# amcpherson/defuse

Hardware: AMD Instinct MI355X
Metric: split-read DP aligns/sec (higher is better)
Workload: dtype int16

## Files before the change

### defuse_amd/csrc/dsa_api.hip

```cpp
#include <hip/hip_runtime.h>
#include <fcntl.h>
#include <sys/file.h>
#include <unistd.h>
#include <hipcub/hipcub.hpp>

#include <algorithm>
#include <atomic>
#include <condition_variable>
#include <memory>
#include <mutex>
#include <thread>
#include <cstdio>
#include <cstdlib>
#include <cstring>
#include <string>
#include <chrono>
#include <vector>

#include "dsa_kernels.hpp"
#include "dsa_long.hpp"
#include "dsa_diag_host.hpp"
#include "hip_host.hpp"

using namespace dsa;

namespace {

template <typename T>
using DevBuf = hiphost::DeviceBuffer<T, hiphost::GrowSize>;
using hiphost::elapsed;
using hiphost::grid_of;

struct HostResult {
    Counters ctr;
    int64_t n_rec;
    PlanGlobals plan;
};

struct PipeLane {
    hipStream_t stream = nullptr;
    hipEvent_t ev[7] = {};
    hipStream_t aux = nullptr;
    hipEvent_t ev_fork = nullptr, ev_join = nullptr;
    HostResult* host = nullptr;
    int slice = -1;
    int64_t resident_upload = -1;
    int resident_slice = -1;
    bool emit_pending = false;
    bool emit_early = false;
    uint64_t emit_cap = 0;
    int emit_from = 5;
    uint64_t last_gtasks = 0;
    bool phase1_end_recorded = false;
    unsigned tier_hint = 0xFu;
    unsigned tiers_launched = 0;
    DevBuf<uint8_t> d_wg_tier;
    DevBuf<uint32_t> d_rowcodes, d_rowbytes, d_bnd, d_cmax, d_rmax, d_tmask;
    DevBuf<PairState> d_state;
    DevBuf<KeptRow> d_kept;
    DevBuf<int64_t> d_rec_count, d_rec_offset;
    DevBuf<ReplayTask> d_tasks;
    DevBuf<uint64_t> d_masks;
    DevBuf<uint2> d_gtasks;
    DevBuf<Counters> d_ctr;
    DevBuf<uint8_t> d_scan_tmp;
    DevBuf<int32_t> d_tstop;
#ifdef DSA_PRUNE_STATS
    DevBuf<unsigned long long> d_stats;
#endif
    void release()
    {
        d_wg_tier.release(); d_rowcodes.release(); d_rowbytes.release();
        d_bnd.release(); d_cmax.release(); d_rmax.release(); d_tmask.release(); d_state.release(); d_kept.release();
        d_rec_count.release(); d_rec_offset.release(); d_tasks.release(); d_masks.release(); d_gtasks.release();
        d_ctr.release(); d_scan_tmp.release(); d_tstop.release();
    }
};

struct LaneSet {
    int device = -1;
    hipStream_t own[2] = {};
    PipeLane lane[2];
    ~LaneSet()
    {
        if (device >= 0) (void)hipSetDevice(device);
        (void)hipDeviceSynchronize();
        for (PipeLane& L : lane) {
            L.release();
            for (auto& e : L.ev)
                if (e) (void)hipEventDestroy(e);
            if (L.ev_fork) (void)hipEventDestroy(L.ev_fork);
            if (L.ev_join) (void)hipEventDestroy(L.ev_join);
            if (L.aux) (void)hipStreamDestroy(L.aux);
            if (L.host) (void)hipHostFree(L.host);
        }
        for (hipStream_t st : own)
            if (st) (void)hipStreamDestroy(st);
    }
};

std::atomic<int64_t> g_upload_serial{0};

struct Slice {
    int64_t pair_begin = 0, pair_end = 0;
    Geom g{};
};

}

struct dsa_ctx {
    int device = -1;
    hipStream_t main_stream() const;
    hipStream_t user_stream = nullptr;
    std::string err;
    size_t scratch_budget = (size_t)16 << 30;
    unsigned plan_flags = 0;

    int64_t n_pairs = 0, ref_bytes_len = 0, read_bytes_len = 0;
    int32_t n_fusions = 0;
    DevBuf<uint8_t> d_ref, d_reads;
    DevBuf<dsa_fusion> d_fusions;
    int64_t upload_serial = 0;
    int nch_all = 1;
    DevBuf<uint32_t> d_refcodes;
    hipEvent_t ev_pack[2] = {};
    DevBuf<int32_t> d_orig;
    DevBuf<dsa_pair> d_pairs_in;
    DevBuf<dsa_pair> d_pairs;
    DevBuf<int32_t> d_min_score;
    DevBuf<PlanRun> plan_runs;
    DevBuf<uint32_t> plan_key, plan_key_sorted;
    DevBuf<int32_t> plan_fidx, plan_order, plan_bsum, plan_start, plan_rank;
    DevBuf<uint16_t> plan_bound;
    DevBuf<uint8_t> plan_flip, plan_sort_tmp;
    DevBuf<PlanGlobals> plan_glob;
    PlanParams plan_prm{};
    hipEvent_t ev_plan[2] = {};
    bool plan_timed = false;
    std::vector<Slice> slices;
    float last_plan_ms = 0.f;
    std::vector<int32_t> h_min_score;
    std::vector<LongDesc> h_long;
    std::vector<int32_t> h_long_fusions;
    std::vector<LongState> h_long_state;
    DevBuf<LongDesc> d_long;
    DevBuf<int32_t> d_long_fusions, d_long_work, d_long_rows;
    DevBuf<LongState> d_long_state;
    DevBuf<uint32_t> d_long_bits;
    int64_t long_cells = 0;
    int64_t long_blank_cells = 0;

    std::shared_ptr<LaneSet> lanes;
    DevBuf<dsa_record> d_records;
    int64_t n_records = 0;
    bool have_results = false;

    dsa_timing timing{};
    dsa_kernel_counts kcounts{};
};

hipStream_t dsa_ctx::main_stream() const { return lanes->lane[0].stream; }

namespace {

template <class... Args>
int fail(dsa_ctx* c, int code, const char* fmt, Args... args)
{
    std::string nowhere;
    return hiphost::fail(c ? c->err : nowhere, code, fmt, args...);
}

#define HIPC(call) HIPHOST_TRY(ctx->err, call)

int min_score_for(int lq)
{
    float f = (float)lq * (float)DSA_MATCH;
    return (int)((double)f * 0.90);
}

size_t slice_scratch_bytes(int64_t n_waves, int lq1, int nch)
{
    size_t rows = (size_t)n_waves * lq1 * WAVE * 4;
    return 3 * rows + rows / 4 + 2 * rows * (size_t)nch;
}

void make_slices(dsa_ctx* ctx, int64_t n_pairs, int lqmax)
{
    ctx->slices.clear();
    const int lq1 = (lqmax + 1 + 3) & ~3;
    const size_t per_wg = slice_scratch_bytes(WG_WAVES, lq1, ctx->nch_all);
    int64_t chunk = (int64_t)std::min<size_t>((size_t)1 << 40, ctx->scratch_budget / std::max<size_t>(per_wg, 1)) * WG_LANES;
    if (const char* e = getenv("DEFUSE_DSA_SPLIT_LARGE"))
        if (atoi(e) != 0 && chunk >= n_pairs && n_pairs >= ((int64_t)1 << 19)) chunk = ((n_pairs + 1) / 2 + WG_LANES - 1) / WG_LANES * WG_LANES;
    if (const char* e = getenv("DEFUSE_DSA_SLICE_PAIRS")) chunk = std::min<int64_t>(chunk, std::max<int64_t>(WG_LANES, atoll(e) / WG_LANES * WG_LANES));
    chunk = std::max<int64_t>(chunk, WG_LANES);
    for (int64_t b = 0; b < n_pairs; b += chunk) {
        Slice cur;
        cur.pair_begin = b;
        cur.pair_end = std::min(n_pairs, b + chunk);
        const int64_t n = cur.pair_end - cur.pair_begin;
        cur.g.n_waves = (int32_t)((n + WAVE - 1) / WAVE);
        cur.g.n_wgs = (int32_t)((n + WG_LANES - 1) / WG_LANES);
        cur.g.lq1 = lq1;
        cur.g.nch = ctx->nch_all;
        cur.g.lrp = ctx->nch_all * W;
        cur.g.n_fusions = ctx->n_fusions;
        cur.g.n_pairs = n;
        cur.g.orig = nullptr;
        ctx->slices.push_back(cur);
    }
}

int enqueue_plan(dsa_ctx* ctx)
{
    const int nf = ctx->n_fusions;
    const int64_t n_pairs = ctx->n_pairs;
    if (n_pairs == 0 || nf == 0 || ctx->slices.empty()) return DSA_OK;
    hipStream_t st = ctx->main_stream();
    const bool no_reorder = ctx->plan_flags & DSA_PLAN_NO_REORDER, no_rank = ctx->plan_flags & DSA_PLAN_NO_RANK,
               no_tighten = ctx->plan_flags & DSA_PLAN_NO_TIGHTEN, no_lpt = ctx->plan_flags & DSA_PLAN_NO_LPT;
    int64_t max_chunk = 0;
    for (const Slice& sl : ctx->slices) max_chunk = std::max(max_chunk, sl.pair_end - sl.pair_begin);
    const int nb = (nf + PLACE_BLOCK - 1) / PLACE_BLOCK;
    HIPC(ctx->plan_runs.reserve((size_t)nf));
    HIPC(ctx->plan_key.reserve((size_t)nf));
    HIPC(ctx->plan_key_sorted.reserve((size_t)nf));
    HIPC(ctx->plan_fidx.reserve((size_t)nf));
    HIPC(ctx->plan_order.reserve((size_t)nf));
    HIPC(ctx->plan_bsum.reserve((size_t)nb));
    HIPC(ctx->plan_start.reserve((size_t)nf));
    HIPC(ctx->plan_flip.reserve((size_t)nf));
    HIPC(ctx->plan_rank.reserve((size_t)max_chunk));
    HIPC(ctx->plan_bound.reserve((size_t)max_chunk));
    HIPC(ctx->plan_glob.reserve(ctx->slices.size()));
    HIPC(ctx->d_orig.reserve((size_t)n_pairs));
    HIPC(ctx->d_pairs.reserve((size_t)n_pairs + 1));
    size_t sort_tmp = 0;
    HIPC(hipcub::DeviceRadixSort::SortPairs(nullptr, sort_tmp, ctx->plan_key.p, ctx->plan_key_sorted.p, ctx->plan_fidx.p, ctx->plan_order.p, nf, 0, PLAN_KEY_BITS, st));
    HIPC(ctx->plan_sort_tmp.reserve(sort_tmp));
    const PlanParams prm = ctx->plan_prm;
    const size_t lds = plan_lds_bytes(prm.wc, prm.slots);
    HIPC(hipEventRecord(ctx->ev_plan[0], st));
    HIPC(hipMemsetAsync(ctx->plan_glob.p, 0, ctx->slices.size() * sizeof(PlanGlobals), st));
    for (size_t k = 0; k < ctx->slices.size(); ++k) {
        Slice& sl = ctx->slices[k];
        const int64_t n = sl.pair_end - sl.pair_begin;
        const dsa_pair* in = ctx->d_pairs_in.p + sl.pair_begin;
        sl.g.orig = ctx->d_orig.p + sl.pair_begin;
        PlanGlobals* glob = ctx->plan_glob.p + k;
        if (!no_reorder) {
            HIPC(hipMemsetAsync(ctx->plan_runs.p, 0, (size_t)nf * sizeof(PlanRun), st));
            hipLaunchKernelGGL(k_plan_runs, dim3(grid_of(n)), dim3(256), 0, st, in, n, ctx->plan_runs.p);
            PlanParams pp = prm;
            pp.use_rank = no_rank ? 0 : 1;
            pp.use_bound = no_tighten ? 0 : 1;
            pp.use_lpt = no_lpt ? 0 : 1;
            hipLaunchKernelGGL(k_plan_fusion, dim3((unsigned)nf), dim3(PLAN_THREADS), lds, st, ctx->d_ref.p, ctx->d_fusions.p, ctx->d_reads.p, in,
                               ctx->plan_runs.p, ctx->plan_key.p, ctx->plan_fidx.p, ctx->plan_rank.p, ctx->plan_bound.p, glob, pp);
            size_t tmp = ctx->plan_sort_tmp.cap;
            HIPC(hipcub::DeviceRadixSort::SortPairs(ctx->plan_sort_tmp.p, tmp, ctx->plan_key.p, ctx->plan_key_sorted.p, ctx->plan_fidx.p,
                                                    ctx->plan_order.p, nf, 0, PLAN_KEY_BITS, st));
            hipLaunchKernelGGL(k_plan_place_a, dim3((unsigned)nb), dim3(PLACE_BLOCK), 0, st, ctx->plan_order.p, ctx->plan_runs.p, nf, ctx->plan_bsum.p);
            hipLaunchKernelGGL(k_plan_place_b, dim3((unsigned)nb), dim3(PLACE_BLOCK), 0, st, ctx->plan_order.p, ctx->plan_runs.p, nf, ctx->plan_bsum.p,
                               ctx->plan_start.p, ctx->plan_flip.p);
        }
        hipLaunchKernelGGL(k_plan_permute, dim3(grid_of(n)), dim3(256), 0, st, in, n, ctx->d_fusions.p, ctx->plan_runs.p, ctx->plan_start.p,
                           ctx->plan_flip.p, ctx->plan_rank.p, ctx->plan_bound.p, glob, no_reorder ? 1 : 0, ctx->d_pairs.p + sl.pair_begin,
                           ctx->d_orig.p + sl.pair_begin);
    }
    HIPC(hipEventRecord(ctx->ev_plan[1], st));
    HIPC(hipGetLastError());
    ctx->plan_timed = true;
    for (PipeLane& L : ctx->lanes->lane) L.resident_upload = -1;
    return DSA_OK;
}

int exclusive_scan(dsa_ctx* ctx, PipeLane& L, const int64_t* in, int64_t* out, int64_t n)
{
    HIPC(hiphost::cub_run(L.d_scan_tmp, [&](void* t, size_t& tmp) {
        return hipcub::DeviceScan::ExclusiveSum(t, tmp, in, out, (int)n, L.stream);
    }));
    return DSA_OK;
}

int grow_records(dsa_ctx* ctx, size_t need)
{
    if (need <= ctx->d_records.cap) return DSA_OK;
    DevBuf<dsa_record> bigger;
    HIPC(bigger.reserve(need + need / 2 + 1024));
    HIPC(hipDeviceSynchronize());
    if (ctx->n_records)
        HIPC(hipMemcpy(bigger.p, ctx->d_records.p, ctx->n_records * sizeof(dsa_record), hipMemcpyDeviceToDevice));
    ctx->d_records.release();
    ctx->d_records.swap(bigger);
    return DSA_OK;
}

FinishBufs finish_bufs(PipeLane& L)
{
    FinishBufs fb;
    fb.state = L.d_state.p;
    fb.kept = L.d_kept.p;
    fb.tasks = L.d_tasks.p;
    fb.masks = L.d_masks.p;
    fb.gtasks = L.d_gtasks.p;
    fb.ctr = L.d_ctr.p;
    fb.kept_cap = L.d_kept.cap;
    fb.task_cap = L.d_tasks.cap;
    fb.mask_cap = L.d_masks.cap / 2;
    fb.gtask_cap = L.d_gtasks.cap;
    fb.tstop = L.d_tstop.p;
    fb.rec_count = L.d_rec_count.p;
    return fb;
}

unsigned listed_grid(const PipeLane& L, int64_t n_pairs)
{
    const uint64_t expect = L.last_gtasks ? L.last_gtasks : (uint64_t)n_pairs / 10 + 1;
    const uint64_t blocks = (expect + expect / 64 + EMIT_BLOCK - 1) / EMIT_BLOCK + 1;
    return (unsigned)std::min<uint64_t>(std::max<uint64_t>(blocks, 16), 16384);
}
void launch_emit(dsa_ctx* ctx, PipeLane& L, const Slice& s, size_t cap_left, bool record_start = true)
{
    const int64_t np = s.g.n_pairs;
    Geom g = s.g;
    g.tiers_launched = L.tiers_launched;
    const dsa_pair* pairs = ctx->d_pairs.p + s.pair_begin;
    dsa_record* out = ctx->d_records.p + ctx->n_records;
    L.emit_from = record_start ? 5 : 2;
    if (record_start) (void)hipEventRecord(L.ev[5], L.stream);
    (void)hipEventRecord(L.ev_fork, L.stream);
    (void)hipStreamWaitEvent(L.aux, L.ev_fork, 0);
    hipLaunchKernelGGL(k_emit_listed<true>, dim3(listed_grid(L, np)), dim3(EMIT_BLOCK), 0, L.aux, L.d_gtasks.p, (uint64_t)L.d_gtasks.cap, L.d_ctr.p,
                       pairs, ctx->d_fusions.p, L.d_state.p, L.d_kept.p, L.d_tasks.p, (uint64_t)L.d_tasks.cap, L.d_masks.p,
                       (uint64_t)(L.d_masks.cap / 2), (uint64_t)L.d_kept.cap, L.d_rec_count.p, (const int64_t*)L.d_rec_offset.p, out,
                       (uint64_t)cap_left, (int64_t)s.pair_begin, g);
    (void)hipEventRecord(L.ev_join, L.aux);
    hipLaunchKernelGGL(k_emit_counted, dim3((unsigned)((np + EMIT_BLOCK - 1) / EMIT_BLOCK)), dim3(EMIT_BLOCK), 0, L.stream, pairs, ctx->d_fusions.p,
                       L.d_state.p, L.d_kept.p, L.d_tasks.p, L.d_masks.p, (const int64_t*)L.d_rec_offset.p, out, (uint64_t)cap_left,
                       (int64_t)s.pair_begin, L.d_ctr.p, (uint64_t)L.d_kept.cap, (uint64_t)L.d_tasks.cap, (uint64_t)(L.d_masks.cap / 2),
                       (uint64_t)L.d_gtasks.cap, g);
    if (!ctx->h_long.empty())
        hipLaunchKernelGGL(k_long_emit<true>, dim3((unsigned)((ctx->h_long.size() + 63) / 64)), dim3(64), 0, L.stream, ctx->d_long.p, ctx->d_long_state.p,
                           (int)ctx->h_long.size(), ctx->d_long_work.p, ctx->d_long_bits.p, (int64_t)s.pair_begin, (int64_t)s.pair_end, L.d_rec_count.p,
                           (const int64_t*)L.d_rec_offset.p, out, (uint64_t)cap_left);
    (void)hipStreamWaitEvent(L.stream, L.ev_join, 0);
    (void)hipEventRecord(L.ev[6], L.stream);
}

int launch_compute(dsa_ctx* ctx, PipeLane& L, const Slice& s)
{
    Geom g = s.g;
#ifdef DSA_PRUNE_STATS
    HIPC(L.d_stats.reserve(16));
    HIPC(hipMemsetAsync(L.d_stats.p, 0, 16 * sizeof(unsigned long long), L.stream));
    g.stats = L.d_stats.p;
#endif
    hipStream_t st = L.stream;
    const int64_t np = g.n_pairs;
    const dsa_pair* pairs = ctx->d_pairs.p + s.pair_begin;
    const FinishBufs fb = finish_bufs(L);
    hipLaunchKernelGGL(k_reset_finish, dim3(1), dim3(64), 0, st, L.d_ctr.p, L.d_rec_count.p + np);
    HIPC(hipEventRecord(L.ev[1], st));
    const unsigned mask = L.tier_hint | 1u;
    L.tiers_launched = mask;
    g.tiers_launched = mask;
#define DSA_LAUNCH_FILL(TIER, WIDE)                                                                                                              \
    hipLaunchKernelGGL((k_fill_fast<TIER, WIDE>), dim3((unsigned)g.n_wgs), dim3(WG_LANES), 0, st, pairs, L.d_wg_tier.p, ctx->d_refcodes.p, \
                       ctx->d_reads.p, L.d_rowcodes.p, L.d_rowbytes.p, ctx->d_min_score.p, ctx->d_fusions.p, L.d_bnd.p, L.d_cmax.p, L.d_rmax.p, L.d_tmask.p, fb, g)
    const bool wide = g.nch > 8 && g.nch <= 16;
    if (wide) DSA_LAUNCH_FILL(0, true); else DSA_LAUNCH_FILL(0, false);
    if (mask & 2u) { if (wide) DSA_LAUNCH_FILL(1, true); else DSA_LAUNCH_FILL(1, false); }
    if (mask & 4u) { if (wide) DSA_LAUNCH_FILL(2, true); else DSA_LAUNCH_FILL(2, false); }
#undef DSA_LAUNCH_FILL
    if (mask & 8u)
        hipLaunchKernelGGL(k_fill_generic, dim3((unsigned)g.n_wgs), dim3(WG_LANES), 0, st, pairs, ctx->d_fusions.p, L.d_wg_tier.p, ctx->d_refcodes.p,
                           ctx->d_reads.p, L.d_rowcodes.p, ctx->d_min_score.p, L.d_bnd.p, L.d_cmax.p, L.d_rmax.p, L.d_tmask.p, fb, g);
    HIPC(hipEventRecord(L.ev[2], st));
    hipLaunchKernelGGL(k_replay, dim3(2048), dim3(REPLAY_BLOCK), 0, st, L.d_tasks.p, (uint64_t)L.d_tasks.cap, L.d_gtasks.p,
                       (uint64_t)L.d_gtasks.cap, L.d_ctr.p, L.d_state.p, L.d_kept.p, (uint64_t)L.d_kept.cap, pairs, ctx->d_fusions.p,
                       ctx->d_refcodes.p, L.d_rowcodes.p, L.d_bnd.p, L.d_tstop.p, L.d_masks.p, (uint64_t)(L.d_masks.cap / 2), g);
    hipLaunchKernelGGL(k_emit_listed<false>, dim3(listed_grid(L, np)), dim3(EMIT_BLOCK), 0, st, L.d_gtasks.p, (uint64_t)L.d_gtasks.cap, L.d_ctr.p,
                       pairs, ctx->d_fusions.p, L.d_state.p, L.d_kept.p, L.d_tasks.p, (uint64_t)L.d_tasks.cap, L.d_masks.p,
                       (uint64_t)(L.d_masks.cap / 2), (uint64_t)L.d_kept.cap, L.d_rec_count.p, (const int64_t*)nullptr, (dsa_record*)nullptr,
                       (uint64_t)0, (int64_t)s.pair_begin, g);
    if (!ctx->h_long.empty())
        hipLaunchKernelGGL(k_long_emit<false>, dim3((unsigned)((ctx->h_long.size() + 63) / 64)), dim3(64), 0, st, ctx->d_long.p, ctx->d_long_state.p,
                           (int)ctx->h_long.size(), ctx->d_long_work.p, ctx->d_long_bits.p, (int64_t)s.pair_begin, (int64_t)s.pair_end, L.d_rec_count.p,
                           (const int64_t*)nullptr, (dsa_record*)nullptr, (uint64_t)0);
    if (int rc = exclusive_scan(ctx, L, L.d_rec_count.p, L.d_rec_offset.p, np + 1)) return rc;
    hipLaunchKernelGGL(k_publish, dim3(1), dim3(64), 0, st, L.d_ctr.p, L.d_rec_offset.p + np, reinterpret_cast<const unsigned long long*>(ctx->plan_glob.p + (&s - ctx->slices.data())),
                       &L.host->ctr, &L.host->n_rec, reinterpret_cast<unsigned long long*>(&L.host->plan));
    L.emit_cap = 0;
    L.emit_early = false;
    L.phase1_end_recorded = false;
    if (ctx->n_records == 0 && &s == &ctx->slices.front() && ctx->d_records.cap > 0) {
        L.emit_cap = ctx->d_records.cap;
        L.emit_early = true;
        launch_emit(ctx, L, s, L.emit_cap, false);
    } else {
        HIPC(hipEventRecord(L.ev[3], st));
        L.phase1_end_recorded = true;
    }
    HIPC(hipGetLastError());
    return DSA_OK;
}

int phase1(dsa_ctx* ctx, PipeLane& L, int slice_idx)
{
    const Slice& s = ctx->slices[slice_idx];
    Geom g = s.g;
    hipStream_t st = L.stream;
    const int64_t np = g.n_pairs;
    if (g.lq1 > ((FAST_MAX_READ + 1 + 3) & ~3)) return fail(ctx, DSA_E_LIMIT, "internal: a long read reached the 16-bit kernels");
    const size_t n_rows = (size_t)g.n_waves * g.lq1 * WAVE;
    HIPC(L.d_wg_tier.reserve((size_t)g.n_wgs));
    HIPC(L.d_rowcodes.reserve(n_rows));
    HIPC(L.d_rowbytes.reserve(n_rows / 4));
    HIPC(L.d_bnd.reserve(n_rows * g.nch));
    HIPC(L.d_cmax.reserve(n_rows * g.nch));
    HIPC(L.d_rmax.reserve(n_rows));
    HIPC(L.d_tmask.reserve(n_rows));
    HIPC(L.d_tstop.reserve((size_t)g.n_waves * g.nch));
    HIPC(L.d_state.reserve(np));
    HIPC(L.d_rec_count.reserve(np + 1));
    HIPC(L.d_rec_offset.reserve(np + 1));
    HIPC(L.d_ctr.reserve(1));
    HIPC(L.d_kept.reserve((size_t)np * 2 + 1024));
    HIPC(L.d_tasks.reserve((size_t)np * 4 + 1024));
    HIPC(L.d_masks.reserve((size_t)np * 8 + 1024));
    HIPC(L.d_gtasks.reserve((size_t)np * 2 + 1024));
    if (int rc = launch_compute(ctx, L, s)) return rc;
    L.slice = slice_idx;
    return DSA_OK;
}

void account_emit(dsa_ctx* ctx, PipeLane& L)
{
    if (!L.emit_pending) return;
    (void)hipEventSynchronize(L.ev[6]);
    ctx->timing.finish_ms += elapsed(L.ev[L.emit_from], L.ev[6]);
    L.emit_pending = false;
}

int phase2(dsa_ctx* ctx, PipeLane& L)
{
    const Slice& s = ctx->slices[L.slice];
    account_emit(ctx, L);
    for (int attempt = 0;; ++attempt) {
        HIPC(hipStreamSynchronize(L.stream));
        HIPC(hipGetLastError());
        const Counters c = L.host->ctr;
        const bool tiers_ok = (c.need_tiers & ~L.tiers_launched) == 0;
        L.tier_hint = tiers_ok ? c.need_tiers : 0xFu;
        if (!tiers_ok) ctx->kcounts.slices_rerun += 1;
        if (tiers_ok && c.n_kept <= L.d_kept.cap && c.n_tasks <= L.d_tasks.cap && c.n_masks <= L.d_masks.cap / 2 && c.n_gtasks <= L.d_gtasks.cap) break;
        if (attempt >= 3) return fail(ctx, DSA_E_DEVICE, "finish stage did not converge");
        HIPC(L.d_kept.reserve(c.n_kept + 1024));
        HIPC(L.d_tasks.reserve(c.n_tasks + 1024));
        HIPC(L.d_masks.reserve(2 * c.n_masks + 1024));
// ... 113 lines not shown
    if (hiphost::check_device(device) || hipSetDevice(device) != hipSuccess) return DSA_E_DEVICE;
    dsa_ctx* ctx = new dsa_ctx();
    ctx->device = device;
    bool ok = true;
    for (const auto& sw : {std::pair<const char*, unsigned>{"DEFUSE_DSA_NO_REORDER", DSA_PLAN_NO_REORDER}, {"DEFUSE_DSA_NO_RANK", DSA_PLAN_NO_RANK},
                           {"DEFUSE_DSA_NO_TIGHTEN", DSA_PLAN_NO_TIGHTEN}, {"DEFUSE_DSA_NO_LPT", DSA_PLAN_NO_LPT}}) {
        const char* e = getenv(sw.first);
        if (e && atoi(e) != 0) ctx->plan_flags |= sw.second;
    }
    if (share) {
        ctx->lanes = share->lanes;
        ctx->scratch_budget = share->scratch_budget;
    } else {
        ctx->lanes = std::make_shared<LaneSet>();
        ctx->lanes->device = device;
        for (int l = 0; l < 2; ++l) {
            PipeLane& L = ctx->lanes->lane[l];
            ok = ok && hipStreamCreate(&ctx->lanes->own[l]) == hipSuccess;
            L.stream = ctx->lanes->own[l];
            for (auto& e : L.ev) ok = ok && hipEventCreate(&e) == hipSuccess;
            ok = ok && hipStreamCreateWithFlags(&L.aux, hipStreamNonBlocking) == hipSuccess;
            ok = ok && hipEventCreateWithFlags(&L.ev_fork, hipEventDisableTiming) == hipSuccess;
            ok = ok && hipEventCreateWithFlags(&L.ev_join, hipEventDisableTiming) == hipSuccess;
            ok = ok && hipHostMalloc((void**)&L.host, sizeof(HostResult)) == hipSuccess;
        }
    }
    for (auto& e : ctx->ev_pack) ok = ok && hipEventCreate(&e) == hipSuccess;
    for (auto& e : ctx->ev_plan) ok = ok && hipEventCreate(&e) == hipSuccess;
    if (!ok) {
        dsa_destroy(ctx);
        return DSA_E_DEVICE;
    }
    if (!share)
        if (const char* mb = getenv("DEFUSE_DSA_SCRATCH_MB")) {
            long v = atol(mb);
            if (v > 0) ctx->scratch_budget = (size_t)v << 20;
        }
    *out = ctx;
    return DSA_OK;
}

int dsa_create(dsa_ctx** out, int device) { return create_ctx(out, device, nullptr); }

void dsa_destroy(dsa_ctx* ctx)
{
    if (!ctx) return;
    (void)hipSetDevice(ctx->device);
    (void)hipDeviceSynchronize();
    ctx->d_ref.release(); ctx->d_reads.release(); ctx->d_fusions.release(); ctx->d_pairs.release(); ctx->d_orig.release(); ctx->d_pairs_in.release();
    ctx->d_min_score.release(); ctx->d_records.release(); ctx->d_refcodes.release();
    ctx->plan_runs.release(); ctx->plan_key.release(); ctx->plan_key_sorted.release(); ctx->plan_fidx.release(); ctx->plan_order.release();
    ctx->plan_bsum.release(); ctx->plan_start.release(); ctx->plan_rank.release(); ctx->plan_bound.release(); ctx->plan_flip.release();
    ctx->plan_sort_tmp.release(); ctx->plan_glob.release();
    ctx->d_long.release(); ctx->d_long_fusions.release(); ctx->d_long_work.release(); ctx->d_long_rows.release(); ctx->d_long_state.release();
    ctx->d_long_bits.release();
    for (auto& e : ctx->ev_pack)
        if (e) (void)hipEventDestroy(e);
    for (auto& e : ctx->ev_plan)
        if (e) (void)hipEventDestroy(e);
    ctx->lanes.reset();
    delete ctx;
}

int dsa_share_scratch(dsa_ctx* ctx, dsa_ctx* donor)
{
    if (!ctx || !donor || ctx == donor) return DSA_E_ARG;
    if (ctx->device != donor->device) return fail(ctx, DSA_E_ARG, "dsa_share_scratch: contexts on different devices");
    HIPC(hipSetDevice(ctx->device));
    HIPC(hipDeviceSynchronize());
    ctx->lanes = donor->lanes;
    ctx->scratch_budget = donor->scratch_budget;
    return DSA_OK;
}

int dsa_get_limits(const dsa_ctx*, dsa_limits* out)
{
    if (!out) return DSA_E_ARG;
    out->max_read_len = LONG_MAX_READ;
    out->max_ref_len = LONG_MAX_REF;
    out->tile_cols = W;
    return DSA_OK;
}

const char* dsa_last_error(const dsa_ctx* ctx) { return ctx ? ctx->err.c_str() : "no context"; }

int dsa_set_stream(dsa_ctx* ctx, void* hip_stream)
{
    if (!ctx) return DSA_E_ARG;
    ctx->user_stream = (hipStream_t)hip_stream;
    ctx->lanes->lane[0].stream = hip_stream ? (hipStream_t)hip_stream : ctx->lanes->own[0];
    return DSA_OK;
}

int dsa_synchronize(dsa_ctx* ctx)
{
    if (!ctx) return DSA_E_ARG;
    HIPC(hipStreamSynchronize(ctx->main_stream()));
    return DSA_OK;
}

}

namespace {

int upload_enqueue(dsa_ctx* ctx, hipStream_t st, const uint8_t* ref_bytes, int64_t ref_bytes_len, const dsa_fusion* fusions,
               int32_t n_fusions, const uint8_t* read_bytes, int64_t read_bytes_len, const dsa_pair* pairs,
               int64_t n_pairs)
{
    if (!ctx) return DSA_E_ARG;
    if (n_fusions < 0 || n_pairs < 0 || ref_bytes_len < 0 || read_bytes_len < 0)
        return fail(ctx, DSA_E_ARG, "negative size");
    if (n_pairs >= ((int64_t)1 << 31)) return fail(ctx, DSA_E_LIMIT, "more than 2^31-1 pairs in one batch");
    if ((n_fusions && !fusions) || (n_pairs && !pairs) || (ref_bytes_len && !ref_bytes) || (read_bytes_len && !read_bytes))
        return fail(ctx, DSA_E_ARG, "null pointer with non-zero size");
    ctx->h_long.clear();
    ctx->h_long_fusions.clear();
    ctx->long_cells = 0;
    ctx->long_blank_cells = 0;
    int nch_all = 1, maxwin = 0;
    for (int32_t f = 0; f < n_fusions; ++f) {
        const dsa_fusion& fu = fusions[f];
        if (fu.ref0_len < 0 || fu.ref1_len < 0 || fu.ref0_off < 0 || fu.ref1_off < 0 ||
            (int64_t)fu.ref0_off + fu.ref0_len > ref_bytes_len || (int64_t)fu.ref1_off + fu.ref1_len > ref_bytes_len)
            return fail(ctx, DSA_E_ARG, "fusion %d: reference window outside ref_bytes", f);
        if (fu.ref0_len > LONG_MAX_REF || fu.ref1_len > LONG_MAX_REF)
            return fail(ctx, DSA_E_LIMIT, "fusion %d: reference window longer than %d", f, LONG_MAX_REF);
        if (fu.ref0_len > FAST_MAX_REF || fu.ref1_len > FAST_MAX_REF) {
            ctx->h_long_fusions.push_back(f);
            continue;
        }
        nch_all = std::max<int>(nch_all, std::max(grid_of(fu.ref0_len, W), grid_of(fu.ref1_len, W)));
        maxwin = std::max(maxwin, std::max(fu.ref0_len, fu.ref1_len));
    }
    const bool any_long_fusion = !ctx->h_long_fusions.empty();
    int lqmax = 0;
    for (int64_t p = 0; p < n_pairs; ++p) {
        const dsa_pair& pr = pairs[p];
        if (pr.fusion_idx < 0 || pr.fusion_idx >= n_fusions) return fail(ctx, DSA_E_ARG, "pair %lld: bad fusion_idx", (long long)p);
        if (pr.read_len < 0 || pr.read_off < 0 || (int64_t)pr.read_off + pr.read_len > read_bytes_len)
            return fail(ctx, DSA_E_ARG, "pair %lld: read outside read_bytes", (long long)p);
        if (pr.read_len > LONG_MAX_READ) return fail(ctx, DSA_E_LIMIT, "pair %lld: read longer than %d", (long long)p, LONG_MAX_READ);
        if (pr.read_len > FAST_MAX_READ ||
            (any_long_fusion && (fusions[pr.fusion_idx].ref0_len > FAST_MAX_REF || fusions[pr.fusion_idx].ref1_len > FAST_MAX_REF))) {
            const dsa_fusion& fu = fusions[pr.fusion_idx];
            LongDesc d;
            d.pair_idx = (int32_t)p;
            d.read_off = pr.read_off;
            d.read_len = pr.read_len;
            d.ref0_off = fu.ref0_off;
            d.ref0_len = fu.ref0_len;
            d.ref1_off = fu.ref1_off;
            d.ref1_len = fu.ref1_len;
            d.fusion_id = fu.fusion_id;
            d.frag = pr.frag;
            d.read_end = pr.read_end;
            d.revcomp = pr.revcomp;
            d.min_score = min_score_for(pr.read_len);
            ctx->h_long.push_back(d);
            ctx->long_cells += (int64_t)(fu.ref0_len + 1 + fu.ref1_len + 1) * (pr.read_len + 1);
            ctx->long_blank_cells += (fu.ref0_len > FAST_MAX_REF || fu.ref1_len > FAST_MAX_REF) ? 2 : fu.ref0_len + 1 + fu.ref1_len + 1;
            continue;
        }
        lqmax = std::max(lqmax, (int)pr.read_len);
    }
    HIPC(hipSetDevice(ctx->device));
    ctx->have_results = false;
    ctx->n_records = 0;
    ctx->upload_serial = ++g_upload_serial;
    ctx->n_pairs = n_pairs;
    ctx->n_fusions = n_fusions;
    ctx->ref_bytes_len = ref_bytes_len;
    ctx->read_bytes_len = read_bytes_len;
    HIPC(ctx->d_ref.reserve((size_t)ref_bytes_len + 64));
    HIPC(ctx->d_reads.reserve((size_t)read_bytes_len + 64));
    HIPC(ctx->d_fusions.reserve((size_t)n_fusions + 1));
    HIPC(ctx->d_pairs_in.reserve((size_t)n_pairs + 1));
    ctx->nch_all = nch_all;
    HIPC(ctx->d_refcodes.reserve((size_t)n_fusions * nch_all * W + 1));
    if (ref_bytes_len) HIPC(hipMemcpyAsync(ctx->d_ref.p, ref_bytes, ref_bytes_len, hipMemcpyHostToDevice, st));
    if (read_bytes_len) HIPC(hipMemcpyAsync(ctx->d_reads.p, read_bytes, read_bytes_len, hipMemcpyHostToDevice, st));
    if (n_fusions) HIPC(hipMemcpyAsync(ctx->d_fusions.p, fusions, n_fusions * sizeof(dsa_fusion), hipMemcpyHostToDevice, st));
    if (n_pairs) HIPC(hipMemcpyAsync(ctx->d_pairs_in.p, pairs, n_pairs * sizeof(dsa_pair), hipMemcpyHostToDevice, st));
    if (!ctx->h_long.empty() || !ctx->h_long_fusions.empty()) {
        const int nl = (int)ctx->h_long.size(), nlf = (int)ctx->h_long_fusions.size();
        HIPC(ctx->d_long.reserve((size_t)nl + 1));
        HIPC(ctx->d_long_fusions.reserve((size_t)nlf + 1));
        if (nl) HIPC(hipMemcpyAsync(ctx->d_long.p, ctx->h_long.data(), (size_t)nl * sizeof(LongDesc), hipMemcpyHostToDevice, st));
        if (nlf) HIPC(hipMemcpyAsync(ctx->d_long_fusions.p, ctx->h_long_fusions.data(), (size_t)nlf * sizeof(int32_t), hipMemcpyHostToDevice, st));
        const int n = std::max(nl, nlf);
        hipLaunchKernelGGL(k_long_blank, dim3(grid_of(n)), dim3(256), 0, st, ctx->d_pairs_in.p, ctx->d_long.p, nl, ctx->d_fusions.p,
                           ctx->d_long_fusions.p, nlf);
    }
    std::vector<int32_t>& tab = ctx->h_min_score;
    tab.resize(lqmax + 1);
    for (int l = 0; l <= lqmax; ++l) tab[l] = min_score_for(l);
    HIPC(ctx->d_min_score.reserve(tab.size()));
    HIPC(hipMemcpyAsync(ctx->d_min_score.p, tab.data(), tab.size() * sizeof(int32_t), hipMemcpyHostToDevice, st));
    {
        const int mw = std::min(maxwin, PLAN_MAXWIN - 1);
        int slots = 256;
        while (slots < 2 * mw) slots <<= 1;
        ctx->plan_prm = PlanParams{};
        ctx->plan_prm.n_fusions = n_fusions;
        ctx->plan_prm.slots = slots;
        ctx->plan_prm.wc = (mw + 2 * PLAN_PAD + 47) / 16 + 1;
        ctx->plan_prm.tile_cols = W;
    }
    make_slices(ctx, n_pairs, lqmax);
    HIPC(hipGetLastError());
    return DSA_OK;
}


}

extern "C" {

int dsa_upload(dsa_ctx* ctx, const uint8_t* ref_bytes, int64_t ref_bytes_len, const dsa_fusion* fusions,
               int32_t n_fusions, const uint8_t* read_bytes, int64_t read_bytes_len, const dsa_pair* pairs,
               int64_t n_pairs)
{
    if (!ctx) return DSA_E_ARG;
    if (int rc = upload_enqueue(ctx, ctx->main_stream(), ref_bytes, ref_bytes_len, fusions, n_fusions, read_bytes, read_bytes_len, pairs, n_pairs)) return rc;
    if (int rc = enqueue_plan(ctx)) return rc;
    HIPC(hipStreamSynchronize(ctx->main_stream()));
    HIPC(hipGetLastError());
    return DSA_OK;
}

int dsa_plan(dsa_ctx* ctx)
{
    if (!ctx) return DSA_E_ARG;
    HIPC(hipSetDevice(ctx->device));
    ctx->have_results = false;
    return enqueue_plan(ctx);
}

}

namespace {

void reset_lanes(dsa_ctx* ctx)
{
    for (PipeLane& L : ctx->lanes->lane) {
        (void)hipStreamSynchronize(L.stream);
        (void)hipStreamSynchronize(L.aux);
        L.slice = -1;
        L.emit_pending = false;
        L.emit_early = false;
    }
    (void)hipGetLastError();
}

int run_long(dsa_ctx* ctx)
{
    const int nl = (int)ctx->h_long.size();
    if (nl == 0) return DSA_OK;
    hipStream_t st = ctx->lanes->lane[0].stream;
    std::vector<LongState>& hs = ctx->h_long_state;
    hs.assign((size_t)nl, LongState{});
    for (LongState& x : hs) x.max_score = -1;
    int64_t work = 0, rows_max = 0;
    for (int k = 0; k < nl; ++k) {
        const LongDesc& d = ctx->h_long[(size_t)k];
        hs[(size_t)k].work_off = work;
        work += long_work_words(d.read_len);
        rows_max = std::max(rows_max, long_rows_words(d.ref0_len, d.ref1_len));
    }
    const int grid = (int)std::max<int64_t>(1, std::min<int64_t>(std::min(nl, 512), ((int64_t)1 << 28) / std::max<int64_t>(rows_max, 1)));
    HIPC(ctx->d_long_work.reserve((size_t)work + 1));
    HIPC(ctx->d_long_rows.reserve((size_t)(rows_max * grid) + 1));
    HIPC(ctx->d_long_state.reserve((size_t)nl));
    HIPC(hipMemcpyAsync(ctx->d_long_state.p, hs.data(), (size_t)nl * sizeof(LongState), hipMemcpyHostToDevice, st));
    hipLaunchKernelGGL(k_long_rows, dim3((unsigned)grid), dim3(LONG_THREADS), 0, st, ctx->d_long.p, ctx->d_long_state.p, nl, ctx->d_ref.p, ctx->d_reads.p,
                       ctx->d_long_work.p, ctx->d_long_rows.p, rows_max);
    HIPC(hipMemcpyAsync(hs.data(), ctx->d_long_state.p, (size_t)nl * sizeof(LongState), hipMemcpyDeviceToHost, st));
    HIPC(hipStreamSynchronize(st));
    HIPC(hipGetLastError());
    int64_t bits = 0;
    for (int k = 0; k < nl; ++k) {
        const LongDesc& d = ctx->h_long[(size_t)k];
        ctx->kcounts.long_pairs += hs[(size_t)k].max_score >= 0 ? 1 : 0;
        hs[(size_t)k].bits_off = bits;
        bits += (int64_t)hs[(size_t)k].n_kept * (long_bitmap_words(d.ref0_len) + long_bitmap_words(d.ref1_len));
    }
    HIPC(ctx->d_long_bits.reserve((size_t)bits + 1));
    HIPC(hipMemcpyAsync(ctx->d_long_state.p, hs.data(), (size_t)nl * sizeof(LongState), hipMemcpyHostToDevice, st));
    hipLaunchKernelGGL(k_long_cols, dim3((unsigned)grid), dim3(LONG_THREADS), 0, st, ctx->d_long.p, ctx->d_long_state.p, nl, ctx->d_ref.p, ctx->d_reads.p,
                       ctx->d_long_work.p, ctx->d_long_rows.p, rows_max, ctx->d_long_bits.p);
// ... 368 lines not shown
```

### defuse_amd/csrc/dsa_diag.hpp

```cpp
#pragma once
#include <hip/hip_runtime.h>

namespace dsa {

#ifdef DSA_NO_PRUNE
constexpr bool DIAG_PRUNE = false;
#else
constexpr bool DIAG_PRUNE = true;
#endif
#ifdef DSA_NO_GAP_SKIP
constexpr bool DIAG_GAP_SKIP = false;
#else
constexpr bool DIAG_GAP_SKIP = true;
#endif
#ifdef DSA_NARROW
constexpr bool DIAG_NARROW = true;
#else
constexpr bool DIAG_NARROW = false;
#endif
#ifdef DSA_ABLATE_TAIL
constexpr bool DIAG_TAIL = false;
#else
constexpr bool DIAG_TAIL = true;
#endif
#ifdef DSA_ABLATE_REPLAY
constexpr bool DIAG_REPLAY = false;
#else
constexpr bool DIAG_REPLAY = true;
#endif

enum DiagSlot {
    DS_GROUPS_SKIPPED = 0, DS_GROUPS = 1, DS_UNUSED2 = 2, DS_WAVE_CYCLES = 3, DS_BARRIER = 4, DS_TABLES = 5, DS_TAIL = 6, DS_ROWMAX = 7,
    DS_COMBINE = 8, DS_REPLAY = 9, DS_GREPLAY_SETUP = 10, DS_GREPLAY_SWEEP = 11, DS_GREPLAY_WAVES = 12, DS_GREPLAY_STEPS = 13,
    DS_GAP_GROUPS = 14, DS_SLOWEST_LISTED = 15
};

#ifdef DSA_PRUNE_STATS
struct DiagClock {
    unsigned long long t;
    __device__ DiagClock() : t(__builtin_readcyclecounter()) {}
    __device__ unsigned long long lap()
    {
        const unsigned long long n = __builtin_readcyclecounter(), d = n - t;
        t = n;
        return d;
    }
};
#define DSA_STAT_ADD(g, slot, v) atomicAdd(&(g).stats[slot], (unsigned long long)(v))
#define DSA_STAT_MAX(g, slot, v) atomicMax(&(g).stats[slot], (unsigned long long)(v))
#else
struct DiagClock {
    __device__ unsigned long long lap() { return 0; }
};
#define DSA_STAT_ADD(g, slot, v) ((void)0)
#define DSA_STAT_MAX(g, slot, v) ((void)0)
#endif

}
```

### defuse_amd/csrc/dsa_diag_host.hpp

```cpp
#pragma once
#ifdef DSA_PRUNE_STATS
#include <cstdio>
#include <vector>

#include "dsa_kernels.hpp"

namespace dsa {

inline void diag_dump_slice(const unsigned long long* d_stats, const uint2* d_gtasks, size_t ng, const ReplayTask* d_tasks, size_t nt)
{
    std::vector<uint2> gt(ng);
    std::vector<ReplayTask> tk(nt);
    if (ng) (void)hipMemcpy(gt.data(), d_gtasks, ng * sizeof(uint2), hipMemcpyDeviceToHost);
    if (nt) (void)hipMemcpy(tk.data(), d_tasks, nt * sizeof(ReplayTask), hipMemcpyDeviceToHost);
    long hist[3][10] = {};
    for (size_t i = 0; i < ng; ++i) {
        const ReplayTask& t = tk[gt[i].x & ~GTASK_OWNER];
        const int kind = t.chunk0 != NO_CHUNK && t.chunk1 != NO_CHUNK ? 2 : t.chunk0 != NO_CHUNK ? 0 : 1;
        hist[kind][std::min(9, (t.last_row & TASK_ROW) / 8)]++;
    }
    for (int k = 0; k < 3; ++k) {
        fprintf(stderr, "[stats] left-over replay tasks, %s, by last row / 8:", k == 0 ? "M1 side only" : k == 1 ? "M2 side only" : "both sides");
        for (int b = 0; b < 10; ++b) fprintf(stderr, " %ld", hist[k][b]);
        fprintf(stderr, "\n");
    }
    unsigned long long h[16];
    (void)hipMemcpy(h, d_stats, sizeof h, hipMemcpyDeviceToHost);
    const double wc = h[DS_WAVE_CYCLES] ? (double)h[DS_WAVE_CYCLES] : 1.0;
    fprintf(stderr,
            "[stats] fill: row groups not swept %llu of %llu (of which skipped between live parts %llu); wave cycles %.4g: tile barriers %.1f %%, "
            "table builds %.1f %%, tail %.1f %% (row maxima %.1f, combine %.1f, replay %.1f), sweeps %.1f %%\n",
            h[DS_GROUPS_SKIPPED], h[DS_GROUPS], h[DS_GAP_GROUPS], wc, 100.0 * h[DS_BARRIER] / wc, 100.0 * h[DS_TABLES] / wc, 100.0 * h[DS_TAIL] / wc,
            100.0 * h[DS_ROWMAX] / wc, 100.0 * h[DS_COMBINE] / wc, 100.0 * h[DS_REPLAY] / wc,
            100.0 * (wc - h[DS_BARRIER] - h[DS_TABLES] - h[DS_TAIL]) / wc);
    fprintf(stderr, "[stats] left-over replay: %llu waves, set-up %llu, sweep %llu cycles, %llu steps (lane 0); slowest lane of the listed count: %llu cycles, "
            "%llu kept rows, %llu tasks\n", h[DS_GREPLAY_WAVES], h[DS_GREPLAY_SETUP], h[DS_GREPLAY_SWEEP], h[DS_GREPLAY_STEPS], h[DS_SLOWEST_LISTED] >> 24,
            (h[DS_SLOWEST_LISTED] >> 8) & 0xFFFF, h[DS_SLOWEST_LISTED] & 0xFF);
}

inline void diag_dump_plan()
{
    unsigned long long h[8] = {}, zero[8] = {};
    (void)hipMemcpyFromSymbol(h, HIP_SYMBOL(g_plan_phase), sizeof h);
    (void)hipMemcpyToSymbol(HIP_SYMBOL(g_plan_phase), zero, sizeof zero);
    double tot = 0;
    for (int k = 0; k < 6; ++k) tot += (double)h[k];
    if (tot == 0) return;
    const char* names[6] = {"prologue + first read", "windows packed", "11-mers hashed", "diagonals + vote", "bounds + keys", "ranks"};
    fprintf(stderr, "[stats] k_plan_fusion wave cycles %.4g:", tot);
    for (int k = 0; k < 6; ++k) fprintf(stderr, " %s %.1f %%", names[k], 100.0 * h[k] / tot);
    fprintf(stderr, "\n");
}

}
#endif
```

### defuse_amd/csrc/dsa_kernels.hpp

```cpp
#pragma once
#include <hip/hip_runtime.h>
#include <stdint.h>

#include "../../include/defuse_dsa.h"
#include "dsa_diag.hpp"

namespace dsa {

constexpr int W = 64;
constexpr int WAVE = 64;
constexpr int WG_WAVES = 4;
constexpr int WG_LANES = WG_WAVES * WAVE;
constexpr uint32_t REF_PAD16 = 0x00AAu;
constexpr uint32_t ROW_PAD16 = 0x0055u;

constexpr int NCLS = 5;
constexpr int NCOMBO = NCLS * NCLS;
constexpr int TROW = W + 4;
#ifndef FILL_PF
#define FILL_PF 2
#endif
constexpr int GMAX = 4;
constexpr int TGROUP = NCOMBO * TROW;
constexpr int GSPLIT = 20;
constexpr int GSPLIT2 = 40;
constexpr int TROW_S = TROW / 2;
constexpr int TGROUP_SPLIT = 2 * NCLS * TROW_S;
static_assert(GSPLIT * TGROUP_SPLIT <= GMAX * TGROUP, "split tables must fit the LDS of the combined ones");
static_assert((TROW_S % 2) == 0, "split table rows are read with ds_read_b64");

__device__ __forceinline__ uint4 split_terms(const uint32_t* tb, uint32_t k1, uint32_t k2, int q)
{
    const uint2 L = reinterpret_cast<const uint2*>(tb + k1 * TROW_S)[q];
    const uint2 H = reinterpret_cast<const uint2*>(tb + (NCLS + k2) * TROW_S)[q];
    return make_uint4(__builtin_amdgcn_perm(H.x, L.x, 0x05040100u), __builtin_amdgcn_perm(H.x, L.x, 0x07060302u),
                      __builtin_amdgcn_perm(H.y, L.y, 0x05040100u), __builtin_amdgcn_perm(H.y, L.y, 0x07060302u));
}
constexpr uint32_t BIAS16 = 0x0400u;
constexpr uint32_t BIAS2 = 0x04000400u;
constexpr uint32_t TWO2 = 0x00020002u;
constexpr uint32_t FOUR2 = 0x00040004u;
constexpr uint32_t SIX2 = 0x00060006u;
__host__ __device__ constexpr uint32_t drift2(int i) { return (uint32_t)(2 * i) * 0x00010001u; }

typedef unsigned short v2u __attribute__((ext_vector_type(2)));
typedef _Float16 v2h __attribute__((ext_vector_type(2)));

__device__ __forceinline__ uint32_t max2(uint32_t a, uint32_t b)
{
    return __builtin_bit_cast(uint32_t, __builtin_elementwise_maximum(__builtin_bit_cast(v2h, a), __builtin_bit_cast(v2h, b)));
}
__device__ __forceinline__ uint32_t pk_max_u16(uint32_t a, uint32_t b)
{
    return __builtin_bit_cast(uint32_t, __builtin_elementwise_max(__builtin_bit_cast(v2u, a), __builtin_bit_cast(v2u, b)));
}
__device__ __forceinline__ uint32_t max3(uint32_t a, uint32_t b, uint32_t c)
{
    return __builtin_bit_cast(uint32_t,
                              __builtin_elementwise_maximum(
                                  __builtin_elementwise_maximum(__builtin_bit_cast(v2h, a), __builtin_bit_cast(v2h, b)),
                                  __builtin_bit_cast(v2h, c)));
}
__device__ __forceinline__ uint32_t min3u(uint32_t x)
{
    const v2u three = {3, 3};
    return __builtin_bit_cast(uint32_t, __builtin_elementwise_min(__builtin_bit_cast(v2u, x), three));
}

__device__ __forceinline__ int pair_bound(const dsa_pair& pr) { return (int)pr.pad_[0] | ((int)pr.pad_[1] << 8); }

struct WaveInfo {
    int32_t lq_max;
    int32_t nch_max;
};

constexpr uint8_t TIER_GENERIC = 3;

struct WgGroupsLds {
    int32_t wave_starts[WG_WAVES];
    int32_t group_f[GSPLIT2];
};
struct WgView {
    int32_t n_groups;
    int32_t f4[GMAX];
    const int32_t* list;
};
__device__ __forceinline__ int group_fusion(const WgView& v, int k)
{
    if (v.n_groups > GMAX) return v.list[k];
    int f = v.f4[0];
#pragma unroll
    for (int j = 1; j < GMAX; ++j)
        if (k == j) f = v.f4[j];
    return f;
}
__device__ __forceinline__ WgView wg_groups(WgGroupsLds* gl, int f, int f_prev_of_wave_lane0, int& my_group)
{
    const int tid = threadIdx.x, lane = tid & 63, wv = tid >> 6;
    int fprev = __shfl_up(f, 1, 64);
    if (lane == 0) fprev = f_prev_of_wave_lane0;
    const bool start = tid == 0 || f != fprev;
    const unsigned long long m = __builtin_amdgcn_ballot_w64(start);
    if (lane == 0) gl->wave_starts[wv] = __builtin_popcountll(m);
    __syncthreads();
    int base = 0, total = 0;
#pragma unroll
    for (int k = 0; k < WG_WAVES; ++k) {
        const int c = gl->wave_starts[k];
        if (k < wv) base += c;
        total += c;
    }
    my_group = base + __builtin_popcountll(m & ((2ull << lane) - 1ull)) - 1;
    if (start && my_group < GSPLIT2) gl->group_f[my_group] = f;
    __syncthreads();
    WgView v;
    v.n_groups = total <= GSPLIT2 ? total : 0;
    v.list = gl->group_f;
#pragma unroll
    for (int k = 0; k < GMAX; ++k) v.f4[k] = k < total ? gl->group_f[k] : 0;
    return v;
}

struct Geom {
    int32_t n_waves;
    int32_t n_wgs;
    int32_t lq1;
    int32_t nch;
    int32_t lrp;
    int32_t n_fusions;
    int64_t n_pairs;
    const int32_t* orig;
    uint32_t tiers_launched;
#ifdef DSA_PRUNE_STATS
    unsigned long long* stats;
#endif
};

struct KeptRow {
    int16_t a;
    int16_t m1, m2;
    int16_t pad_;
};

constexpr uint8_t NO_CHUNK = 0xFF;
struct ReplayTask {
    uint32_t pair;
    uint32_t mask_begin;
    uint16_t last_row;
    uint8_t  chunk0;
    uint8_t  chunk1;
    int32_t fusion;
};
constexpr uint32_t GTASK_OWNER = 0x80000000u;
constexpr uint16_t TASK_FAST = 0x8000u;
constexpr uint16_t TASK_ONLY = 0x4000u;
constexpr uint16_t TASK_ROW = 0x3FFFu;

struct alignas(8) PairState {
    uint32_t mask_begin;
    uint32_t kept_begin;
    uint32_t task_begin;
    uint16_t n_kept;
    uint8_t n_tasks;
    uint8_t flags;
    uint16_t tiles0, tiles1;
    uint8_t first0, first1;
    uint16_t pad_;
};
__device__ __forceinline__ int task_of_tile(uint32_t tiles, int first, int c)
{
    if (c == first) return 0;
    const uint32_t rest = first < 16 ? tiles & ~(1u << first) : tiles;
    return 1 + __builtin_popcount(rest & ((1u << c) - 1u));
}
static_assert(sizeof(PairState) == 24, "three 8-byte loads");
constexpr uint8_t STATE_COUNTED = 1;
constexpr uint8_t STATE_TILES = 2;

struct Counters {
    unsigned long long n_kept, n_tasks, n_masks, n_gtasks;
    unsigned need_tiers;
    unsigned pad_;
    unsigned fill_wgs[8];
};
constexpr int FILL_WGS_FAST = 0;
constexpr int FILL_WGS_GENERIC = 6;

__device__ __forceinline__ int cdiv_dev(int a, int b) { return (a + b - 1) / b; }

__host__ __device__ __forceinline__ int64_t rowidx(int j, int lane) { return ((int64_t)(j >> 2) * WAVE + lane) * 4 + (j & 3); }
constexpr uint32_t CODE_MASK = 0xFF00FF00u;
__device__ __forceinline__ int half_of(uint32_t v, int h) { return (int)((v >> (16 * h)) & 0xFFFFu) - (int)BIAS16; }

__global__ void k_pack_refs(const uint8_t* __restrict__ ref_bytes, const dsa_fusion* __restrict__ fusions,
                            uint32_t* __restrict__ refcodes, Geom g)
{
    int64_t t = (int64_t)blockIdx.x * blockDim.x + threadIdx.x;
    int64_t total = (int64_t)g.n_fusions * g.lrp;
    if (t >= total) return;
    const int i = (int)(t % g.lrp);
    const dsa_fusion f = fusions[t / g.lrp];
    uint32_t lo = REF_PAD16, hi = REF_PAD16;
    if (i < f.ref0_len) lo = (uint32_t)ref_bytes[(int64_t)f.ref0_off + i] << 8;
    if (i < f.ref1_len) hi = (uint32_t)ref_bytes[(int64_t)f.ref1_off + (f.ref1_len - 1 - i)] << 8;
    refcodes[t] = lo | (hi << 16);
}

__device__ __forceinline__ bool is_fast_base(uint32_t b)
{
    return b == 'A' || b == 'C' || b == 'G' || b == 'T' || b == 'N';
}

__device__ __forceinline__ uint32_t base_class(uint32_t byte)
{
    uint32_t k = (byte >> 1) & 7u;
    return k > 4u ? 4u : k;
}
__device__ __forceinline__ uint32_t table_row(uint32_t k1, uint32_t k2)
{
    if (k1 < 4u && k2 < 4u) return 4u * k1 + k2;
    return k1 == 4u ? 16u + k2 : 21u + k1;
}
__device__ __forceinline__ void table_row_classes(int t, int& k1, int& k2)
{
    if (t < 16) { k1 = t >> 2; k2 = t & 3; }
    else if (t < 21) { k1 = 4; k2 = t - 16; }
    else { k1 = t - 21; k2 = 4; }
}

template <bool SPLIT, class CodeFn>
__device__ __forceinline__ void build_tables(uint32_t* __restrict__ T, int n_groups, CodeFn&& code_of)
{
    for (int e = threadIdx.x; e < n_groups * W; e += WG_LANES) {
        const int i = e & (W - 1), gi = e >> 6;
        uint32_t q0, q1;
        code_of(gi, i, q0, q1);
        const uint32_t cls_byte[NCLS] = {'A', 'C', 'T', 'G', 'N'};
        uint32_t lo[NCLS], hi[NCLS];
#pragma unroll
        for (int k = 0; k < NCLS; ++k) {
            lo[k] = q0 == REF_PAD16 ? 0u : ((q0 >> 8) == cls_byte[k] ? 4u : 1u);
            hi[k] = (q1 == REF_PAD16 ? 0u : ((q1 >> 8) == cls_byte[k] ? 4u : 1u)) << 16;
        }
        const uint32_t drift = i > 0 ? TWO2 : 0u;
        if (SPLIT) {
            unsigned short* col = reinterpret_cast<unsigned short*>(T + gi * TGROUP_SPLIT) + i;
#pragma unroll
            for (int k = 0; k < NCLS; ++k) {
                col[k * TROW] = (unsigned short)(lo[k] + (drift & 0xFFFFu));
                col[(NCLS + k) * TROW] = (unsigned short)((hi[k] + (drift & 0xFFFF0000u)) >> 16);
            }
        } else {
            uint32_t* col = T + gi * TGROUP + i;
#pragma unroll
            for (int t = 0; t < NCOMBO; ++t) {
                int k1, k2;
                table_row_classes(t, k1, k2);
                col[t * TROW] = (lo[k1] | hi[k2]) + drift;
            }
        }
    }
}

template <int BYTE_KIND>
__device__ __forceinline__ bool pack_rows_wave(const uint8_t* __restrict__ read_bytes, const dsa_pair* __restrict__ pairs,
                                               uint32_t* __restrict__ rowcodes, uint32_t* __restrict__ row_bytes, const Geom& g, int w,
                                               int lane, int lq_wave)
{
    const int64_t p = (int64_t)w * WAVE + lane;
    const bool valid = p < g.n_pairs;
    dsa_pair pr{};
    if (valid) pr = pairs[p];
    uint4* out = reinterpret_cast<uint4*>(rowcodes + (int64_t)w * g.lq1 * WAVE) + lane;
    uint32_t* out1 = BYTE_KIND ? row_bytes + (int64_t)w * (g.lq1 >> 2) * WAVE + lane : nullptr;
    bool exotic = false;
    for (int gq = 0; gq <= (lq_wave >> 2); ++gq) {
        uint32_t code[4];
        uint32_t bytes = 0;
#pragma unroll
        for (int sidx = 0; sidx < 4; ++sidx) {
            const int j = 4 * gq + sidx;
            code[sidx] = ROW_PAD16 | (ROW_PAD16 << 16);
            if (valid && j >= 1 && j <= pr.read_len) {
                const uint32_t b0 = read_bytes[(int64_t)pr.read_off + (j - 1)];
                const uint32_t b1 = read_bytes[(int64_t)pr.read_off + (pr.read_len - j)];
                exotic |= !is_fast_base(b0);
                const uint32_t k1 = base_class(b0), k2 = base_class(b1);
                code[sidx] = (b0 << 8) | (b1 << 24) | table_row(k1, k2) | ((k1 | (k2 << 4)) << 16);
                if (BYTE_KIND) bytes |= (BYTE_KIND == 1 ? table_row(k1, k2) : (k1 | (k2 << 4))) << (8 * sidx);
            }
        }
        out[(int64_t)gq * WAVE] = make_uint4(code[0], code[1], code[2], code[3]);
        if (BYTE_KIND) out1[(int64_t)gq * WAVE] = bytes;
    }
    return exotic;
}

__device__ __forceinline__ void row_step(uint32_t (&X)[W], const uint32_t (&r)[W], uint32_t cj, uint32_t bprev,
                                         uint32_t bcur)
{
    cj &= CODE_MASK;
    constexpr int BLK = 16;
    uint32_t a = (bprev + FOUR2) - min3u(cj ^ r[0]);
    uint32_t up = bcur - TWO2;
#pragma unroll
    for (int b = 0; b < W; b += BLK) {
        uint32_t d[BLK];
#pragma unroll
        for (int k = 0; k < BLK; ++k)
            d[k] = b + k + 1 < W ? SIX2 - min3u(cj ^ r[b + k + 1]) : 0u;
#pragma unroll
        for (int k = 0; k < BLK; ++k) {
            const int i = b + k;
            const uint32_t a_next = X[i] + d[k];
            X[i] = max3(a, X[i], up);
            up = X[i];
            a = a_next;
        }
    }
}

template <bool MASKED>
__device__ __forceinline__ uint32_t tile_row_max(const uint32_t (&X)[W], int nv0, int nv1)
{
    uint32_t acc0 = BIAS2, acc1 = BIAS2;
#pragma unroll
    for (int i = 0; i < W; i += 4) {
        uint32_t x[4];
#pragma unroll
        for (int k = 0; k < 4; ++k) {
            x[k] = X[i + k] - drift2(i + k);
            if (MASKED) {
                if (i + k >= nv0) x[k] = (x[k] & 0xFFFF0000u) | BIAS16;
                if (i + k >= nv1) x[k] = (x[k] & 0x0000FFFFu) | (BIAS16 << 16);
            }
        }
        acc0 = max3(acc0, x[0], x[1]);
        acc1 = max3(acc1, x[2], x[3]);
    }
    return max2(acc0, acc1);
}

__device__ __forceinline__ unsigned long long wave_alloc(unsigned long long* counter, unsigned n)
{
    unsigned incl = n;
#pragma unroll
    for (int d = 1; d < 64; d <<= 1) {
        unsigned y = __shfl_up(incl, d, 64);
        if ((int)(threadIdx.x & 63) >= d) incl += y;
    }
    const unsigned total = __shfl(incl, 63, 64);
    unsigned long long base = 0;
    if ((threadIdx.x & 63) == 63 && total) base = atomicAdd(counter, (unsigned long long)total);
    base = __shfl(base, 63, 64);
    return base + (incl - n);
}

__device__ __forceinline__ int nth_set_bit(uint64_t m, int n)
{
    for (int k = 0; k < n && m; ++k) m &= m - 1;
    return m ? __builtin_ctzll(m) : -1;
}

constexpr int TMASK_TILES = 16;

struct FinishBufs {
    PairState* state;
    KeptRow* kept;
    ReplayTask* tasks;
    uint64_t* masks;
    uint2* gtasks;
    Counters* ctr;
    uint64_t kept_cap, task_cap, mask_cap, gtask_cap;
    int32_t* tstop;
    int64_t* rec_count;
};

__device__ __forceinline__ int load_tstop(const int32_t* p) { return __hip_atomic_load(p, __ATOMIC_RELAXED, __HIP_MEMORY_SCOPE_AGENT); }

struct LaneInfo {
    uint32_t kept_begin, mask_begin;
    uint16_t n_kept;
    uint16_t last_row;
    uint8_t  c0, c1;
    uint16_t key_group;
    uint16_t lq;
    uint8_t  nv0, nv1;
};
constexpr int KCACHE = 3;
struct FinishLds {
    int tile[GSPLIT2];
    int hist[258];
    unsigned short order[WG_LANES];
    LaneInfo info[WG_LANES];
    uint64_t kc[KCACHE * WG_LANES];
};

__device__ __forceinline__ void wave_alloc4(Counters* ctr, const unsigned (&n)[4], unsigned long long (&base)[4])
{
    unsigned incl[4] = {n[0], n[1], n[2], n[3]};
#pragma unroll
    for (int d = 1; d < 64; d <<= 1) {
#pragma unroll
        for (int q = 0; q < 4; ++q) {
            const unsigned y = __shfl_up(incl[q], d, 64);
            if ((int)(threadIdx.x & 63) >= d) incl[q] += y;
        }
    }
    unsigned long long* const counter[4] = {&ctr->n_kept, &ctr->n_tasks, &ctr->n_masks, &ctr->n_gtasks};
    unsigned long long b[4] = {0, 0, 0, 0};
    if ((threadIdx.x & 63) == 63) {
#pragma unroll
        for (int q = 0; q < 4; ++q)
            if (incl[q]) b[q] = atomicAdd(counter[q], (unsigned long long)incl[q]);
    }
#pragma unroll
    for (int q = 0; q < 4; ++q) base[q] = __shfl(b[q], 63, 64) + (incl[q] - n[q]);
}

template <bool HANDOFF>
__device__ __forceinline__ void combine_wg(
    const dsa_pair* __restrict__ pairs, const dsa_fusion* __restrict__ fusions, const uint32_t* __restrict__ cmax,
    const uint32_t* __restrict__ rmax, const uint32_t* __restrict__ tmask, const int32_t* __restrict__ min_score_tab,
    const WgView& wgi, int my_group, bool fast_wg, FinishLds* fl, const FinishBufs& fb, const Geom& g)
{
    PairState* __restrict__ state = fb.state;
    KeptRow* __restrict__ kept = fb.kept;
    ReplayTask* __restrict__ tasks = fb.tasks;
    uint2* __restrict__ gtasks = fb.gtasks;
    const uint64_t kept_cap = fb.kept_cap, task_cap = fb.task_cap, mask_cap = fb.mask_cap, gtask_cap = fb.gtask_cap;
    const int tid = threadIdx.x;
    const int64_t p = (int64_t)blockIdx.x * WG_LANES + tid;
    const bool active = p < g.n_pairs;
    const int64_t w = p >> 6;
    const int lane = (int)(p & 63);
    if (tid < GSPLIT2) fl->tile[tid] = -1;
    const uint32_t* rm = rmax + w * g.lq1 * WAVE;
    const uint4* rm4 = reinterpret_cast<const uint4*>(rm) + lane;
    const uint4* tm4 = reinterpret_cast<const uint4*>(tmask + w * g.lq1 * WAVE) + lane;
    auto accept = [](uint32_t word, int h, int n_chunks, int row) -> int {
        if (row == 0 || n_chunks == 0) return 0;
        const int v = half_of(word, h) - 2 * row;
        return v >= DSA_MIN_SPLIT ? v : 0;
    };
    auto rowmax = [&](int h, int n_chunks, int row) -> int { return accept(rm[rowidx(row, lane)], h, n_chunks, row); };
    auto pick = [](const uint4& v, int k) -> uint32_t { return k == 0 ? v.x : k == 1 ? v.y : k == 2 ? v.z : v.w; };
    int lq = 0, nc0 = 0, nc1 = 0, max_score = 0, n_kept = 0, fidx = -1, len0 = 0, len1 = 0;
    unsigned n_t0 = 0, n_t1 = 0;
    uint64_t tiles0 = 0, tiles1 = 0;
    bool small = true;
    int first_a = 0, last_a = 0;
    uint64_t kcr[KCACHE] = {};
    int n_cached = 0;
    if (active) {
        const dsa_pair pr = pairs[p];
        const dsa_fusion fu = fusions[pr.fusion_idx];
        fidx = pr.fusion_idx;
        lq = pr.read_len;
        len0 = fu.ref0_len;
        len1 = fu.ref1_len;
        nc0 = cdiv_dev(fu.ref0_len, W);
        nc1 = cdiv_dev(fu.ref1_len, W);
        small = nc0 <= 64 && nc1 <= 64;
        const int min_score = min_score_tab[lq];
        if (g.nch <= TMASK_TILES) {
            struct Step { uint4 x, yh, yl, tx, th, tl; };
            const int ng = lq >> 2;
            auto load = [&](int gq) -> Step {
                gq = gq < ng ? gq : ng;
                const int b_hi = lq - 4 * gq, b_lo = b_hi - 3;
                const int64_t ih = (int64_t)(b_hi >> 2) * WAVE, il = (int64_t)((b_lo > 0 ? b_lo : 0) >> 2) * WAVE;
                Step s;
                s.x = rm4[(int64_t)gq * WAVE];
                s.yh = rm4[ih];
                s.yl = rm4[il];
                s.tx = tm4[(int64_t)gq * WAVE];
                s.th = tm4[ih];
                s.tl = tm4[il];
                return s;
            };
            Step s0 = load(0), s1 = load(1);
            for (int gq = 0; gq <= ng; ++gq) {
                const Step cur = s0;
                s0 = s1;
                s1 = load(gq + 2);
                const int b_hi = lq - 4 * gq;
#pragma unroll
                for (int sidx = 0; sidx < 4; ++sidx) {
                    const int a = 4 * gq + sidx, b = lq - a;
                    if (b < 0) continue;
                    const bool in_hi = (b >> 2) == (b_hi >> 2);
                    const uint32_t yw = in_hi ? pick(cur.yh, b & 3) : pick(cur.yl, b & 3);
                    const int m1 = accept(pick(cur.x, sidx), 0, nc0, a), m2 = accept(yw, 1, nc1, b);
                    const int sc = m1 + m2;
                    if (sc < min_score || sc < max_score) continue;
                    if (sc > max_score) {
                        max_score = sc;
                        n_kept = 0;
                        tiles0 = tiles1 = 0;
                    }
                    if (m1 == 0 || m2 == 0) continue;
                    if (n_kept == 0) first_a = a;
                    last_a = a;
                    KeptRow kr;
                    kr.a = (int16_t)a;
                    kr.m1 = (int16_t)m1;
                    kr.m2 = (int16_t)m2;
                    kr.pad_ = 0;
#pragma unroll
                    for (int k = 0; k < KCACHE; ++k)
                        if (n_kept == k) kcr[k] = __builtin_bit_cast(uint64_t, kr);
                    ++n_kept;
                    tiles0 |= pick(cur.tx, sidx) & 0xFFFFu;
                    tiles1 |= (in_hi ? pick(cur.th, b & 3) : pick(cur.tl, b & 3)) >> 16;
                }
            }
            n_cached = n_kept < KCACHE ? n_kept : KCACHE;
        } else {
            auto for_each_split = [&](auto&& fn) {
                for (int gq = 0; 4 * gq <= lq; ++gq) {
                    const int b_hi = lq - 4 * gq, b_lo = b_hi - 3;
                    const uint4 x1 = rm4[(int64_t)gq * WAVE];
                    const uint4 y_hi = rm4[(int64_t)(b_hi >> 2) * WAVE];
                    const uint4 y_lo = rm4[(int64_t)((b_lo > 0 ? b_lo : 0) >> 2) * WAVE];
#pragma unroll
                    for (int sidx = 0; sidx < 4; ++sidx) {
                        const int a = 4 * gq + sidx, b = lq - a;
                        if (b >= 0) {
                            const uint32_t yw = (b >> 2) == (b_hi >> 2) ? pick(y_hi, b & 3) : pick(y_lo, b & 3);
                            fn(a, b, accept(pick(x1, sidx), 0, nc0, a), accept(yw, 1, nc1, b));
                        }
                    }
                }
            };
            for_each_split([&](int, int, int m1, int m2) {
                const int sc = m1 + m2;
                if (sc >= min_score && sc > max_score) max_score = sc;
            });
            if (max_score != 0) {
                first_a = lq;
                for_each_split([&](int a, int b, int m1, int m2) {
                    if (m1 + m2 != max_score || m1 == 0 || m2 == 0) return;
                    if (n_kept == 0) first_a = a;
                    last_a = a;
                    ++n_kept;
// ... 11 lines not shown
        }
        if (n_kept > 0) {
            n_t0 = small ? (unsigned)__builtin_popcountll(tiles0) : (unsigned)nc0;
            n_t1 = small ? (unsigned)__builtin_popcountll(tiles1) : (unsigned)nc1;
        }
    }
    unsigned n_tasks = n_t0 > n_t1 ? n_t0 : n_t1;
    const int gsel = my_group;
    int f0 = small ? nth_set_bit(tiles0, 0) : (n_t0 > 0 ? 0 : -1), f1 = small ? nth_set_bit(tiles1, 0) : (n_t1 > 0 ? 0 : -1);
    const bool eligible = n_tasks > 0 && small && fast_wg && gsel >= 0 && f0 >= 0 && f1 >= 0;
    const int key = eligible ? ((f0 << 8) | f1) : -1;
    constexpr int VOTE_TILES = 8;
    static_assert(GMAX * 2 * VOTE_TILES <= 2 * 258, "votes must fit the histogram words");
    const bool vote = g.nch <= VOTE_TILES && wgi.n_groups <= GMAX;
    if (vote)
        for (int e = tid; e < 258; e += WG_LANES) fl->hist[e] = 0;
    __syncthreads();
    if (eligible) {
        if (vote) {
            for (uint64_t r = tiles0; r; r &= r - 1) {
                const int slot = (gsel * 2 + 0) * VOTE_TILES + __builtin_ctzll(r);
                atomicAdd(&fl->hist[slot >> 1], 1 << (16 * (slot & 1)));
            }
            for (uint64_t r = tiles1; r; r &= r - 1) {
                const int slot = (gsel * 2 + 1) * VOTE_TILES + __builtin_ctzll(r);
                atomicAdd(&fl->hist[slot >> 1], 1 << (16 * (slot & 1)));
            }
        } else
            atomicCAS(&fl->tile[gsel], -1, key);
    }
    __syncthreads();
    if (vote && tid < GMAX) {
        int win[2] = {-1, -1};
        for (int h = 0; h < 2; ++h) {
            int best = 0;
            for (int c = 0; c < VOTE_TILES; ++c) {
                const int slot = (tid * 2 + h) * VOTE_TILES + c;
                const int n = (fl->hist[slot >> 1] >> (16 * (slot & 1))) & 0xFFFF;
                if (n > best) { best = n; win[h] = c; }
            }
        }
        if (win[0] >= 0 && win[1] >= 0) fl->tile[tid] = (win[0] << 8) | win[1];
    }
    if (vote) __syncthreads();
    bool fast = false;
    if (eligible) {
        const int agreed = fl->tile[gsel];
        if (vote) {
            const bool h0 = agreed >= 0 && ((tiles0 >> (agreed >> 8)) & 1ull), h1 = agreed >= 0 && ((tiles1 >> (agreed & 0xFF)) & 1ull);
            fast = h0 || h1;
            if (fast) {
                f0 = h0 ? agreed >> 8 : -1;
                f1 = h1 ? agreed & 0xFF : -1;
                const unsigned s0 = n_t0 + (h0 ? 0u : 1u), s1 = n_t1 + (h1 ? 0u : 1u);
                n_tasks = s0 > s1 ? s0 : s1;
            }
        } else
            fast = agreed == key;
    }
    const unsigned n_gen = n_tasks - (fast ? 1u : 0u);

    const int fold_a = first_a < lq - first_a ? first_a : lq - first_a;
    const unsigned want[4] = {(unsigned)n_kept, n_tasks, n_tasks * (unsigned)n_kept, n_gen};
    unsigned long long base[4];
    wave_alloc4(fb.ctr, want, base);
    const unsigned long long kb = base[0], tb = base[1], mb = base[2], gb = base[3];
    bool ok = active && n_kept > 0;
    if (ok && (kb + n_kept > kept_cap || tb + n_tasks > task_cap || mb + (unsigned long long)n_tasks * n_kept > mask_cap ||
               gb + n_gen > gtask_cap))
        ok = false;
    if (HANDOFF) {
        LaneInfo li;
        li.kept_begin = (uint32_t)kb;
        li.mask_begin = (uint32_t)mb;
        li.n_kept = (uint16_t)(ok ? n_kept : 0);
        const int c0 = f0 >= 0 ? f0 : (int)NO_CHUNK, c1 = f1 >= 0 ? f1 : (int)NO_CHUNK;
        const bool here = ok && fast;
        const int r0 = c0 != NO_CHUNK ? last_a : 0, r1 = c1 != NO_CHUNK ? lq - first_a : 0;
        li.last_row = here ? (uint16_t)((r0 > r1 ? r0 : r1) | TASK_FAST | (n_tasks == 1 ? TASK_ONLY : 0)) : (uint16_t)0;
        li.c0 = here ? (uint8_t)c0 : NO_CHUNK;
        li.c1 = here ? (uint8_t)c1 : NO_CHUNK;
        li.key_group = (uint16_t)((fold_a < 255 ? fold_a : 255) | ((gsel >= 0 ? gsel : 0) << 8));
        li.lq = (uint16_t)lq;
        const int v0 = len0 - c0 * W, v1 = len1 - c1 * W;
        li.nv0 = (uint8_t)(here && c0 != NO_CHUNK ? (v0 < W ? (v0 > 0 ? v0 : 0) : W) : 0);
        li.nv1 = (uint8_t)(here && c1 != NO_CHUNK ? (v1 < W ? (v1 > 0 ? v1 : 0) : W) : 0);
        fl->info[tid] = li;
    }
    if (!active) return;
    PairState st;
    st.mask_begin = (uint32_t)mb;
    st.kept_begin = (uint32_t)kb;
    st.task_begin = (uint32_t)tb;
    st.n_kept = (uint16_t)(ok ? n_kept : 0);
    st.n_tasks = (uint8_t)(n_tasks < 255u ? n_tasks : 255u);
    const bool tiles_fit = small && g.nch <= 16;
    st.flags = (uint8_t)(((!ok || (HANDOFF && fast && n_tasks == 1)) ? STATE_COUNTED : 0) | (tiles_fit ? STATE_TILES : 0));
    st.tiles0 = (uint16_t)(tiles_fit ? tiles0 : 0);
    st.tiles1 = (uint16_t)(tiles_fit ? tiles1 : 0);
    st.first0 = f0 >= 0 ? (uint8_t)f0 : NO_CHUNK;
    st.first1 = f1 >= 0 ? (uint8_t)f1 : NO_CHUNK;
    st.pad_ = 0;
    state[p] = st;
    if (!ok) {
        fb.rec_count[g.orig ? g.orig[p] : p] = 0;
        return;
    }
    int k = 0, a_next = first_a;
    for (; k < n_cached; ++k) {
        const KeptRow kr = __builtin_bit_cast(KeptRow, k == 0 ? kcr[0] : k == 1 ? kcr[1] : kcr[KCACHE - 1]);
        kept[kb + k] = kr;
        if (HANDOFF) fl->kc[k * WG_LANES + tid] = __builtin_bit_cast(uint64_t, kr);
        a_next = kr.a + 1;
    }
    for (int a = a_next; k < n_kept && a <= last_a; ++a) {
        const int m1 = rowmax(0, nc0, a), m2 = rowmax(1, nc1, lq - a);
        if (m1 + m2 != max_score || m1 == 0 || m2 == 0) continue;
        KeptRow kr;
        kr.a = (int16_t)a;
        kr.m1 = (int16_t)m1;
        kr.m2 = (int16_t)m2;
        kr.pad_ = 0;
        kept[kb + k] = kr;
        if (HANDOFF && k < KCACHE) fl->kc[k * WG_LANES + tid] = __builtin_bit_cast(uint64_t, kr);
        ++k;
    }
    unsigned gi = 0;
    const uint64_t rest0 = f0 >= 0 && small ? tiles0 & ~(1ull << f0) : tiles0, rest1 = f1 >= 0 && small ? tiles1 & ~(1ull << f1) : tiles1;
    for (unsigned t = 0; t < n_tasks; ++t) {
        const int c0 = small ? (t == 0 ? f0 : nth_set_bit(rest0, (int)t - 1)) : (t < n_t0 ? (int)t : -1);
        const int c1 = small ? (t == 0 ? f1 : nth_set_bit(rest1, (int)t - 1)) : (t < n_t1 ? (int)t : -1);
        ReplayTask rt;
        rt.pair = (uint32_t)p;
        rt.mask_begin = (uint32_t)(mb + (unsigned long long)t * n_kept);
        const int r0 = c0 >= 0 ? last_a : 0, r1 = c1 >= 0 ? lq - first_a : 0;
        rt.last_row = (uint16_t)(r0 > r1 ? r0 : r1);
        rt.chunk0 = c0 >= 0 ? (uint8_t)c0 : NO_CHUNK;
        rt.chunk1 = c1 >= 0 ? (uint8_t)c1 : NO_CHUNK;
        rt.fusion = fidx;
        if (t == 0 && fast)
            rt.last_row |= TASK_FAST;
        else {
            gtasks[gb + gi] = make_uint2((uint32_t)(tb + t) | (gi == 0 ? GTASK_OWNER : 0u), (uint32_t)p);
            ++gi;
        }
        tasks[tb + t] = rt;
    }
}

struct HitCursor {
    int k0, k1;
    int row0, row1;
    uint32_t t0, t1;
    uint64_t valid0, valid1;
};
__device__ __forceinline__ KeptRow kept_row(const KeptRow* __restrict__ kr, const uint64_t* kc, int k)
{
    if (kc != nullptr && k < KCACHE) return __builtin_bit_cast(KeptRow, kc[k * WG_LANES]);
    return kr[k];
}
__device__ __forceinline__ void cursor_next0(HitCursor& hc, const KeptRow* __restrict__ kr, const uint64_t* kc, int n_kept, bool has0)
{
    hc.row0 = -1;
    if (has0 && hc.k0 < n_kept) {
        const KeptRow r = kept_row(kr, kc, hc.k0);
        hc.row0 = r.a;
        hc.t0 = (uint32_t)(r.m1 + 2 * r.a) + BIAS16;
    }
}
__device__ __forceinline__ void cursor_next1(HitCursor& hc, const KeptRow* __restrict__ kr, const uint64_t* kc, int lq, bool has1)
{
    hc.row1 = -1;
    if (has1 && hc.k1 >= 0) {
        const KeptRow r = kept_row(kr, kc, hc.k1);
        hc.row1 = lq - r.a;
        hc.t1 = (uint32_t)(r.m2 + 2 * (lq - r.a)) + BIAS16;
    }
}
__device__ __forceinline__ HitCursor cursor_init(const KeptRow* __restrict__ kr, const uint64_t* kc, int n_kept, int lq,
                                                 bool has0, bool has1, int nv0, int nv1)
{
    HitCursor hc;
    hc.k0 = 0;
    hc.k1 = n_kept - 1;
    hc.t0 = hc.t1 = 0;
    hc.valid0 = nv0 >= W ? ~0ull : ((1ull << (nv0 > 0 ? nv0 : 0)) - 1ull);
    hc.valid1 = nv1 >= W ? ~0ull : ((1ull << (nv1 > 0 ? nv1 : 0)) - 1ull);
    cursor_next0(hc, kr, kc, n_kept, has0);
    cursor_next1(hc, kr, kc, lq, has1);
    return hc;
}

constexpr uint32_t NO_TARGET16 = 0x7F00u;
__device__ __forceinline__ void equal_columns(const uint32_t (&X)[W], uint32_t target2, uint64_t& m0, uint64_t& m1)
{
    uint32_t hit[W / 16];
    const uint32_t below = target2 - 0x00010001u;
#pragma unroll
    for (int q = 0; q < W / 16; ++q) {
        uint32_t acc = 0;
#pragma unroll
        for (int k = 15; k >= 0; --k) {
            const int i = 16 * q + k;
            const uint32_t c = below + drift2(i);
            typedef unsigned short us2 __attribute__((ext_vector_type(2)));
            const uint32_t y = __builtin_bit_cast(uint32_t, __builtin_elementwise_sub_sat(__builtin_bit_cast(us2, X[i]), __builtin_bit_cast(us2, c)));
            asm("v_lshl_or_b32 %0, %0, 1, %1" : "+v"(acc) : "v"(y));
        }
        hit[q] = acc;
    }
    const uint32_t lo_a = (hit[0] & 0xFFFFu) | (hit[1] << 16), lo_b = (hit[2] & 0xFFFFu) | (hit[3] << 16);
    const uint32_t hi_a = (hit[0] >> 16) | (hit[1] & 0xFFFF0000u), hi_b = (hit[2] >> 16) | (hit[3] & 0xFFFF0000u);
    m0 = (uint64_t)lo_a | ((uint64_t)lo_b << 32);
    m1 = (uint64_t)hi_a | ((uint64_t)hi_b << 32);
}

__device__ __forceinline__ void record_hits(const uint32_t (&X)[W], int j, int lq, const KeptRow* __restrict__ kr,
                                            const uint64_t* kc, int n_kept, bool has0, bool has1, HitCursor& hc,
                                            uint64_t* __restrict__ masks, uint32_t mask_begin)
{
    const bool hit0 = hc.row0 == j, hit1 = hc.row1 == j;
    if (!(hit0 || hit1)) return;
    uint64_t m0, m1;
    equal_columns(X, (hit0 ? hc.t0 : NO_TARGET16) | ((hit1 ? hc.t1 : NO_TARGET16) << 16), m0, m1);
    if (hit0) {
        masks[((uint64_t)mask_begin + hc.k0) * 2] = m0 & hc.valid0;
        ++hc.k0;
        cursor_next0(hc, kr, kc, n_kept, has0);
    }
    if (hit1) {
        masks[((uint64_t)mask_begin + hc.k1) * 2 + 1] = m1 & hc.valid1;
        --hc.k1;
        cursor_next1(hc, kr, kc, lq, has1);
    }
}

__device__ __forceinline__ int64_t count_one_tile_pair(const uint64_t* mk, int n_kept)
{
    int64_t n = 0;
    for (int k = 0; k < n_kept; ++k) {
        const uint64_t m0 = mk[2 * k], m1 = mk[2 * k + 1];
        if (k == 0) {
            n += (int64_t)__builtin_popcountll(m0) * __builtin_popcountll(m1);
            continue;
        }
        for (uint64_t r0 = m0; r0; r0 &= r0 - 1)
            for (uint64_t r1 = m1; r1; r1 &= r1 - 1) {
                const int i1 = __builtin_ctzll(r0), i2 = __builtin_ctzll(r1);
                bool dup = false;
                for (int k2 = 0; k2 < k && !dup; ++k2) dup = ((mk[2 * k2] >> i1) & 1ull) && ((mk[2 * k2 + 1] >> i2) & 1ull);
                n += dup ? 0 : 1;
            }
    }
    return n;
}

template <bool SPLIT>
__device__ __forceinline__ void replay_fast_wg(uint32_t* T, FinishLds* fl, const WgView& wgi, const FinishBufs& fb,
                                               const uint32_t* __restrict__ refcodes, const uint32_t* __restrict__ rowcodes,
                                               const uint32_t* __restrict__ bnd, const Geom& g)
{
    const KeptRow* __restrict__ kept = fb.kept;
    uint64_t* __restrict__ masks = fb.masks;
    bool any = false;
    for (int k = 0; k < wgi.n_groups; ++k) any |= fl->tile[k] >= 0;
    if (!any) return;
    build_tables<SPLIT>(T, wgi.n_groups, [&](int gi, int i, uint32_t& q0, uint32_t& q1) {
        const int key = fl->tile[gi];
        q0 = q1 = REF_PAD16;
        if (key >= 0) {
            const int c0 = key >> 8, c1 = key & 0xFF;
            const uint32_t* rc = refcodes + (int64_t)group_fusion(wgi, gi) * g.lrp;
            if (c0 != NO_CHUNK) q0 = rc[c0 * W + i] & 0xFFFFu;
            if (c1 != NO_CHUNK) q1 = rc[c1 * W + i] >> 16;
        }
    });
    for (int e = threadIdx.x; e < 258; e += WG_LANES) fl->hist[e] = 0;
    __syncthreads();
    int my_key = 256, my_rank = 0;
    {
        const LaneInfo mine = fl->info[threadIdx.x];
        if (mine.last_row & TASK_FAST) my_key = mine.key_group & 0xFF;
        my_rank = atomicAdd(&fl->hist[my_key], 1);
    }
    __syncthreads();
    if (threadIdx.x == 0) {
        int run = 0;
        for (int e = 0; e < 257; ++e) {
            const int n = fl->hist[e];
            fl->hist[e] = run;
            run += n;
        }
    }
    __syncthreads();
    fl->order[fl->hist[my_key] + my_rank] = (unsigned short)threadIdx.x;
    __syncthreads();

    const int src = fl->order[threadIdx.x];
    const LaneInfo li = fl->info[src];
    const int64_t p = (int64_t)blockIdx.x * WG_LANES + src;
    const int lane = (int)(p & 63);
    const int64_t w = p >> 6;
    const bool has = (li.last_row & TASK_FAST) != 0;
    const int R = has ? (li.last_row & TASK_ROW) : 0;
    int Rw = R;
#pragma unroll
    for (int d = 32; d >= 1; d >>= 1) Rw = max(Rw, __shfl_xor(Rw, d, 64));
    if (Rw == 0) return;
    const bool has0 = has && li.c0 != NO_CHUNK, has1 = has && li.c1 != NO_CHUNK;
    const int c0 = has0 ? li.c0 : 0, c1 = has1 ? li.c1 : 0;
    const uint32_t* tb = T + (li.key_group >> 8) * (SPLIT ? TGROUP_SPLIT : TGROUP);
    const int64_t wr = w < g.n_waves ? w : (int64_t)blockIdx.x * WG_WAVES;
    const uint4* rows4 = reinterpret_cast<const uint4*>(rowcodes + wr * g.lq1 * WAVE) + lane;
    const uint4* bi0 = reinterpret_cast<const uint4*>(bnd + (wr * g.nch + (c0 - 1)) * g.lq1 * WAVE) + lane;
    const uint4* bi1 = reinterpret_cast<const uint4*>(bnd + (wr * g.nch + (c1 - 1)) * g.lq1 * WAVE) + lane;
    const KeptRow* kr = kept + li.kept_begin;
    const uint64_t* kc = fl->kc + src;
    const int lq = li.lq;
    const int n_kept = has ? li.n_kept : 0;
    HitCursor hc = cursor_init(kr, kc, n_kept, lq, has0, has1, li.nv0, li.nv1);
    const int stop0 = c0 > 0 ? load_tstop(fb.tstop + wr * g.nch + (c0 - 1)) : 0;
    const int stop1 = c1 > 0 ? load_tstop(fb.tstop + wr * g.nch + (c1 - 1)) : 0;

    uint32_t X[W];
#pragma unroll
    for (int i = 0; i < W; ++i) X[i] = BIAS2 + drift2(i);
    const uint4 bias4 = make_uint4(BIAS2, BIAS2, BIAS2, BIAS2);
    uint32_t bprev = BIAS2;
    const int ngq = (Rw >> 2) + 1;
    auto boundary = [&](int gq) -> uint4 {
        const uint4 x0 = gq < stop0 ? bi0[(int64_t)gq * WAVE] : bias4;
        const uint4 x1 = gq < stop1 ? bi1[(int64_t)gq * WAVE] : bias4;
        return make_uint4((x0.x & 0xFFFFu) | (x1.x & 0xFFFF0000u), (x0.y & 0xFFFFu) | (x1.y & 0xFFFF0000u),
                          (x0.z & 0xFFFFu) | (x1.z & 0xFFFF0000u), (x0.w & 0xFFFFu) | (x1.w & 0xFFFF0000u));
    };
    uint4 rc_n = rows4[0];
    uint4 b_n = boundary(0);
    for (int gq = 0; gq < ngq; ++gq) {
        const uint4 rc = rc_n, b = b_n;
        const int gn = gq + 1 < ngq ? gq + 1 : gq;
        rc_n = rows4[(int64_t)gn * WAVE];
        b_n = boundary(gn);
        const uint32_t rcv[4] = {rc.x, rc.y, rc.z, rc.w}, bv[4] = {b.x, b.y, b.z, b.w};
#pragma unroll
        for (int sidx = 0; sidx < 4; ++sidx) {
            const int j = 4 * gq + sidx;
            const uint32_t bcur = bv[sidx];
            if (j >= 1 && j <= Rw) {
                const uint4* trow = reinterpret_cast<const uint4*>(tb + (rcv[sidx] & 0xFFu) * TROW);
                auto table4 = [&](int q) -> uint4 {
                    if (SPLIT) return split_terms(tb, (rcv[sidx] >> 16) & 0xFu, (rcv[sidx] >> 20) & 0xFu, q);
                    return trow[q];
                };
                uint4 v = table4(0);
                uint32_t a = bprev + v.x;
                uint32_t up = bcur - TWO2;
#pragma unroll
                for (int q = 0; q < W / 4; ++q) {
                    uint4 vn = v;
                    if (q + 1 < W / 4) vn = table4(q + 1);
                    uint32_t an;
                    an = X[4 * q + 0] + v.y;
                    X[4 * q + 0] = max3(a, X[4 * q + 0], up);
                    a = an;
                    an = X[4 * q + 1] + v.z;
                    X[4 * q + 1] = max3(a, X[4 * q + 1], X[4 * q + 0]);
                    a = an;
                    an = X[4 * q + 2] + v.w;
                    X[4 * q + 2] = max3(a, X[4 * q + 2], X[4 * q + 1]);
                    a = an;
                    an = X[4 * q + 3] + vn.x;
                    X[4 * q + 3] = max3(a, X[4 * q + 3], X[4 * q + 2]);
                    a = an;
                    up = X[4 * q + 3];
                    v = vn;
                }
                record_hits(X, j, lq, kr, kc, n_kept, has0, has1, hc, masks, li.mask_begin);
            }
            bprev = bcur;
        }
    }
    if (has && !has0)
        for (int k = 0; k < n_kept; ++k) masks[((uint64_t)li.mask_begin + k) * 2] = 0;
    if (has && !has1)
        for (int k = 0; k < n_kept; ++k) masks[((uint64_t)li.mask_begin + k) * 2 + 1] = 0;
    if (has && (li.last_row & TASK_ONLY) && p < g.n_pairs)
        fb.rec_count[g.orig ? g.orig[p] : p] = count_one_tile_pair(masks + (uint64_t)li.mask_begin * 2, n_kept);
}

template <bool MASKED>
__device__ __forceinline__ int sweep_tile_generic(const uint32_t (&r)[W], const uint4* __restrict__ rows4,
                                                  const uint4* __restrict__ bi4, uint4* __restrict__ cm4,
                                                  uint4* __restrict__ bo4, int lq, bool first, int nv0, int nv1,
                                                  int lq_lane, int slack, int l_in, int stop_prev, int& last_bnd)
{
    uint32_t X[W];
#pragma unroll
    for (int i = 0; i < W; ++i) X[i] = BIAS2 + drift2(i);
    const uint4 bias4 = make_uint4(BIAS2, BIAS2, BIAS2, BIAS2);
    uint32_t bprev = BIAS2;
    const int ngq = (lq >> 2) + 1;
    uint4 rc_n = rows4[0];
    uint4 b_n = first ? bias4 : bi4[0];
    last_bnd = 0;
    int gq = 0;
    for (; gq < ngq; ++gq) {
        const uint4 rc = rc_n, b = b_n;
        const int gn = gq + 1 < ngq ? gq + 1 : gq;
        rc_n = rows4[(int64_t)gn * WAVE];
        b_n = (!first && gn < stop_prev) ? bi4[(int64_t)gn * WAVE] : bias4;
        const uint32_t rcv[4] = {rc.x, rc.y, rc.z, rc.w}, bv[4] = {b.x, b.y, b.z, b.w};
        uint32_t cmv[4] = {BIAS2, BIAS2, BIAS2, BIAS2}, bov[4] = {BIAS2, BIAS2, BIAS2, BIAS2};
        bool alive = false;
#pragma unroll
        for (int sidx = 0; sidx < 4; ++sidx) {
            const int j = 4 * gq + sidx;
            if (j >= 1 && j <= lq) {
                row_step(X, r, rcv[sidx], bprev, bv[sidx]);
                cmv[sidx] = tile_row_max<MASKED>(X, nv0, nv1);
                bov[sidx] = X[W - 1] - drift2(W - 1);
                const int thr = 4 * j - slack + (int)BIAS16;
                const bool in_read = j <= lq_lane;
                alive |= in_read && ((int)(cmv[sidx] & 0xFFFFu) >= thr || (int)(cmv[sidx] >> 16) >= thr);
                if (in_read && ((int)(bov[sidx] & 0xFFFFu) >= thr || (int)(bov[sidx] >> 16) >= thr)) last_bnd = j;
            }
            bprev = bv[sidx];
        }
        cm4[(int64_t)gq * WAVE] = make_uint4(cmv[0], cmv[1], cmv[2], cmv[3]);
        bo4[(int64_t)gq * WAVE] = make_uint4(bov[0], bov[1], bov[2], bov[3]);
        if (DIAG_PRUNE && 4 * gq + 3 > l_in && __builtin_amdgcn_ballot_w64(alive) == 0) { ++gq; break; }
    }
    return gq;
}

__device__ __forceinline__ uint32_t eq_bits(uint32_t v, uint32_t m, int c)
{
    uint32_t differs;
    const uint32_t one2 = 0x00010001u;
    asm("v_pk_min_u16 %0, %1, %2" : "=v"(differs) : "v"(v ^ m), "v"(one2));
    return (differs ^ one2) << c;
}
struct TileStops { int v[8]; };
template <bool WIDE>
__device__ __forceinline__ void reduce_row_max(const uint32_t* __restrict__ cmax, uint32_t* __restrict__ rmax,
                                               uint32_t* __restrict__ tmask, const int32_t* tstop, const TileStops& stops,
                                               const Geom& g, int w, int lane, int nch_wave, int lq)
{
    const int ngq = (lq >> 2) + 1;
    const uint4 dead4 = make_uint4(BIAS2, BIAS2, BIAS2, BIAS2);
    uint4* out = reinterpret_cast<uint4*>(rmax + (int64_t)w * g.lq1 * WAVE) + lane;
    uint4* tout = reinterpret_cast<uint4*>(tmask + (int64_t)w * g.lq1 * WAVE) + lane;
    const uint4* src = reinterpret_cast<const uint4*>(cmax + (int64_t)w * g.nch * g.lq1 * WAVE) + lane;
    const int64_t cstride = (int64_t)(g.lq1 >> 2) * WAVE;
    constexpr int NC = 8;
    if (nch_wave <= NC) {
        for (int gq = 0; gq < ngq; ++gq) {
            uint4 v[NC];
#pragma unroll
            for (int c = 0; c < NC; ++c)
                v[c] = c < nch_wave ? (gq < stops.v[c] ? src[c * cstride + (int64_t)gq * WAVE] : dead4) : make_uint4(0, 0, 0, 0);
            uint4 m = make_uint4(BIAS2, BIAS2, BIAS2, BIAS2);
#pragma unroll
            for (int c = 0; c < NC; ++c)
                if (c < nch_wave) {
                    m.x = max2(m.x, v[c].x);
                    m.y = max2(m.y, v[c].y);
                    m.z = max2(m.z, v[c].z);
                    m.w = max2(m.w, v[c].w);
                }
            uint4 t = make_uint4(0, 0, 0, 0);
#pragma unroll
            for (int c = 0; c < NC; ++c)
                if (c < nch_wave) {
                    t.x |= eq_bits(v[c].x, m.x, c);
                    t.y |= eq_bits(v[c].y, m.y, c);
                    t.z |= eq_bits(v[c].z, m.z, c);
                    t.w |= eq_bits(v[c].w, m.w, c);
                }
            out[(int64_t)gq * WAVE] = m;
            tout[(int64_t)gq * WAVE] = t;
        }
        return;
    }
    if (WIDE && nch_wave <= 2 * NC) {
        int stop_hi[NC];
#pragma unroll
        for (int c = 0; c < NC; ++c) stop_hi[c] = NC + c < nch_wave ? load_tstop(tstop + (int64_t)w * g.nch + NC + c) : 0;
        for (int gq = 0; gq < ngq; ++gq) {
            uint4 v[NC], u[NC];
#pragma unroll
            for (int c = 0; c < NC; ++c) {
                v[c] = gq < stops.v[c] ? src[c * cstride + (int64_t)gq * WAVE] : dead4;
                u[c] = NC + c < nch_wave ? (gq < stop_hi[c] ? src[(NC + c) * cstride + (int64_t)gq * WAVE] : dead4) : make_uint4(0, 0, 0, 0);
            }
            uint4 m = make_uint4(BIAS2, BIAS2, BIAS2, BIAS2);
#pragma unroll
            for (int c = 0; c < NC; ++c) {
                m.x = max2(m.x, v[c].x); m.y = max2(m.y, v[c].y); m.z = max2(m.z, v[c].z); m.w = max2(m.w, v[c].w);
                if (NC + c < nch_wave) { m.x = max2(m.x, u[c].x); m.y = max2(m.y, u[c].y); m.z = max2(m.z, u[c].z); m.w = max2(m.w, u[c].w); }
            }
            uint4 t = make_uint4(0, 0, 0, 0);
#pragma unroll
            for (int c = 0; c < NC; ++c) {
                t.x |= eq_bits(v[c].x, m.x, c); t.y |= eq_bits(v[c].y, m.y, c); t.z |= eq_bits(v[c].z, m.z, c); t.w |= eq_bits(v[c].w, m.w, c);
                if (NC + c < nch_wave) {
                    t.x |= eq_bits(u[c].x, m.x, NC + c); t.y |= eq_bits(u[c].y, m.y, NC + c); t.z |= eq_bits(u[c].z, m.z, NC + c); t.w |= eq_bits(u[c].w, m.w, NC + c);
                }
            }
            out[(int64_t)gq * WAVE] = m;
            tout[(int64_t)gq * WAVE] = t;
        }
        return;
    }
    for (int gq = 0; gq < ngq; ++gq) {
        uint4 m = make_uint4(BIAS2, BIAS2, BIAS2, BIAS2);
        for (int c = 0; c < nch_wave; ++c) {
            const uint4 v = gq < load_tstop(tstop + (int64_t)w * g.nch + c) ? src[c * cstride + (int64_t)gq * WAVE] : dead4;
            m.x = max2(m.x, v.x);
            m.y = max2(m.y, v.y);
            m.z = max2(m.z, v.z);
            m.w = max2(m.w, v.w);
        }
        out[(int64_t)gq * WAVE] = m;
        if (nch_wave <= TMASK_TILES) {
            uint4 t = make_uint4(0, 0, 0, 0);
            for (int c = 0; c < nch_wave; ++c) {
                const uint4 v = gq < load_tstop(tstop + (int64_t)w * g.nch + c) ? src[c * cstride + (int64_t)gq * WAVE] : dead4;
                t.x |= eq_bits(v.x, m.x, c);
                t.y |= eq_bits(v.y, m.y, c);
                t.z |= eq_bits(v.z, m.z, c);
                t.w |= eq_bits(v.w, m.w, c);
            }
            tout[(int64_t)gq * WAVE] = t;
        }
    }
}

__global__ __launch_bounds__(WG_LANES) void k_fill_generic(const dsa_pair* __restrict__ pairs,
                                                           const dsa_fusion* __restrict__ fusions,
                                                           const uint8_t* __restrict__ wg_tier,
                                                           const uint32_t* __restrict__ refcodes,
                                                           const uint8_t* __restrict__ read_bytes,
                                                           uint32_t* __restrict__ rowcodes,
                                                           const int32_t* __restrict__ min_score_tab,
                                                           uint32_t* __restrict__ bnd, uint32_t* __restrict__ cmax,
                                                           uint32_t* __restrict__ rmax, uint32_t* __restrict__ tmask,
                                                           FinishBufs fb, Geom g)
{
    __shared__ FinishLds fl;
    if (wg_tier[blockIdx.x] != TIER_GENERIC) return;
    if (threadIdx.x == 0) atomicAdd(&fb.ctr->fill_wgs[FILL_WGS_GENERIC], 1u);
    const int w = __builtin_amdgcn_readfirstlane((int)(blockIdx.x * WG_WAVES + (threadIdx.x >> 6)));
    if (w < g.n_waves) {
        const int lane = threadIdx.x & 63;
        const int64_t p = min((int64_t)w * WAVE + lane, g.n_pairs - 1);
        const bool in_batch = (int64_t)w * WAVE + lane < g.n_pairs;
        const int f = pairs[p].fusion_idx;
        const dsa_fusion fu = fusions[f];
        auto wave_max = [](int v) {
#pragma unroll
            for (int d = 32; d >= 1; d >>= 1) v = max(v, __shfl_xor(v, d, 64));
            return v;
        };
        WaveInfo wi;
        wi.lq_max = wave_max(in_batch ? (int)pairs[p].read_len : 0);
        wi.nch_max = wave_max(in_batch ? max(cdiv_dev(fu.ref0_len, W), cdiv_dev(fu.ref1_len, W)) : 0);
        (void)pack_rows_wave<0>(read_bytes, pairs, rowcodes, nullptr, g, w, lane, wi.lq_max);
        const uint32_t* rc = refcodes + (int64_t)f * g.lrp;
        const uint4* rows4 = reinterpret_cast<const uint4*>(rowcodes + (int64_t)w * g.lq1 * WAVE) + lane;
        int lq_lane = 0, slack = 0;
        if (in_batch) {
            lq_lane = pairs[p].read_len;
            slack = 2 * lq_lane - max(min_score_tab[lq_lane], pair_bound(pairs[p]));
        }
        int l_in = wave_max(lq_lane > 0 ? min(slack >> 2, lq_lane) : 0);
        int stop_prev = 0;
        TileStops stops = {};

        for (int c = 0; c < wi.nch_max; ++c) {
            uint32_t r[W];
#pragma unroll
            for (int i = 0; i < W; ++i) r[i] = rc[c * W + i];
            const int nv0 = fu.ref0_len - c * W, nv1 = fu.ref1_len - c * W;
            uint4* cm4 = reinterpret_cast<uint4*>(cmax + ((int64_t)w * g.nch + c) * g.lq1 * WAVE) + lane;
            uint4* bo4 = reinterpret_cast<uint4*>(bnd + ((int64_t)w * g.nch + c) * g.lq1 * WAVE) + lane;
            const uint4* bi4 = reinterpret_cast<const uint4*>(bnd + ((int64_t)w * g.nch + (c - 1)) * g.lq1 * WAVE) + lane;
            int last_bnd, stop;
            if (__builtin_amdgcn_ballot_w64(nv0 < W || nv1 < W) == 0)
                stop = sweep_tile_generic<false>(r, rows4, bi4, cm4, bo4, wi.lq_max, c == 0, nv0, nv1, lq_lane, slack, l_in, stop_prev, last_bnd);
            else
                stop = sweep_tile_generic<true>(r, rows4, bi4, cm4, bo4, wi.lq_max, c == 0, nv0, nv1, lq_lane, slack, l_in, stop_prev, last_bnd);
            if (lane == 0) fb.tstop[(int64_t)w * g.nch + c] = stop;
            stop_prev = stop;
#pragma unroll
            for (int k = 0; k < 8; ++k)
                if (k == c) stops.v[k] = stop;
            l_in = wave_max(last_bnd);
        }
        __builtin_amdgcn_fence(__ATOMIC_RELEASE, "workgroup");
        reduce_row_max<false>(cmax, rmax, tmask, fb.tstop, stops, g, w, lane, wi.nch_max, wi.lq_max);
    }
    WgView wgi = {};
    wgi.list = nullptr;
    combine_wg<false>(pairs, fusions, cmax, rmax, tmask, min_score_tab, wgi, 0, false, &fl, fb, g);
}

template <int NW, bool SPLIT, bool LAST>
__device__ __forceinline__ int sweep_tile_fast(const uint32_t* __restrict__ tb, const uint32_t* __restrict__ rows1, const uint4* __restrict__ bi4,
                                               uint4* __restrict__ cm4, uint4* __restrict__ bo4, bool first_tile, int lq_max, int lq_lane,
                                               int slack, int l_in, int stop_prev, int& last_bnd, const Geom& g)
{
    static_assert(NW % 4 == 0 && NW / 4 > FILL_PF, "table reads in flight");
    (void)g;
    uint32_t X[NW];
#pragma unroll
    for (int i = 0; i < NW; ++i) X[i] = BIAS2 + drift2(i);
    const uint4 bias4 = make_uint4(BIAS2, BIAS2, BIAS2, BIAS2);
    uint32_t bprev = BIAS2;
    const int ngq = (lq_max >> 2) + 1;
    uint32_t rc_n = rows1[0];
    uint4 b_n = first_tile ? bias4 : bi4[0];
    last_bnd = 0;
    int gq = 0;
    int n_gap_groups = 0;
    for (; gq < ngq; ++gq) {
        const uint32_t rc = rc_n;
        const uint4 b = b_n;
        const int gn = gq + 1 < ngq ? gq + 1 : gq;
        rc_n = rows1[(int64_t)gn * WAVE];
        b_n = gn < stop_prev ? bi4[(int64_t)gn * WAVE] : bias4;
        const uint32_t bv[4] = {b.x, b.y, b.z, b.w};
        uint32_t cmv[4] = {BIAS2, BIAS2, BIAS2, BIAS2}, bov[4] = {BIAS2, BIAS2, BIAS2, BIAS2};
        uint32_t alive_bits = 0;
#pragma unroll
        for (int sidx = 0; sidx < 4; ++sidx) {
            const int j = 4 * gq + sidx;
            const uint32_t bcur = bv[sidx];
            if (j >= 1 && j <= lq_max) {
                if constexpr (SPLIT) {
                    const uint32_t k1 = (rc >> (8 * sidx)) & 0xFu, k2 = (rc >> (8 * sidx + 4)) & 0xFu;
                    uint4 v = split_terms(tb, k1, k2, 0);
                    uint32_t a = bprev + v.x;
                    uint32_t up = bcur - TWO2;
#pragma unroll
                    for (int q = 0; q < NW / 4; ++q) {
                        uint4 vn = v;
                        if (q + 1 < NW / 4) vn = split_terms(tb, k1, k2, q + 1);
                        uint32_t an;
                        an = X[4 * q + 0] + v.y;
                        X[4 * q + 0] = max3(a, X[4 * q + 0], up);
                        a = an;
                        an = X[4 * q + 1] + v.z;
                        X[4 * q + 1] = max3(a, X[4 * q + 1], X[4 * q + 0]);
                        a = an;
                        an = X[4 * q + 2] + v.w;
                        X[4 * q + 2] = max3(a, X[4 * q + 2], X[4 * q + 1]);
                        a = an;
                        an = X[4 * q + 3] + vn.x;
                        X[4 * q + 3] = max3(a, X[4 * q + 3], X[4 * q + 2]);
                        a = an;
                        up = X[4 * q + 3];
                        v = vn;
                    }
                } else {
                    const uint4* trow = reinterpret_cast<const uint4*>(tb + ((rc >> (8 * sidx)) & 0xFFu) * TROW);
                    uint4 vq[FILL_PF + 1];
#pragma unroll
                    for (int k = 0; k <= FILL_PF; ++k) vq[k] = trow[k];
                    uint32_t a = bprev + vq[0].x;
                    uint32_t up = bcur - TWO2;
#pragma unroll
                    for (int q = 0; q < NW / 4; ++q) {
                        const uint4 v = vq[0];
#pragma unroll
                        for (int k = 0; k < FILL_PF; ++k) vq[k] = vq[k + 1];
                        if (q + 1 + FILL_PF < NW / 4) vq[FILL_PF] = trow[q + 1 + FILL_PF];
                        const uint4 vn = vq[0];
                        uint32_t an;
                        an = X[4 * q + 0] + v.y;
                        X[4 * q + 0] = max3(a, X[4 * q + 0], up);
                        a = an;
                        an = X[4 * q + 1] + v.z;
                        X[4 * q + 1] = max3(a, X[4 * q + 1], X[4 * q + 0]);
                        a = an;
                        an = X[4 * q + 2] + v.w;
                        X[4 * q + 2] = max3(a, X[4 * q + 2], X[4 * q + 1]);
                        a = an;
                        an = X[4 * q + 3] + vn.x;
                        X[4 * q + 3] = max3(a, X[4 * q + 3], X[4 * q + 2]);
                        a = an;
                        up = X[4 * q + 3];
                    }
                }
                {
                    uint32_t acc0 = BIAS2, acc1 = BIAS2;
#pragma unroll
                    for (int i = 0; i < NW; i += 4) {
                        acc0 = max3(acc0, X[i] - drift2(i), X[i + 1] - drift2(i + 1));
                        acc1 = max3(acc1, X[i + 2] - drift2(i + 2), X[i + 3] - drift2(i + 3));
                    }
                    cmv[sidx] = max2(acc0, acc1);
                }
                const int t1 = max(4 * j - slack + (int)BIAS16 - 1, 0);
                const uint32_t tm2 = j <= lq_lane ? (uint32_t)t1 * 0x00010001u : 0xFFFFFFFFu;
                alive_bits |= pk_max_u16(cmv[sidx], tm2) ^ tm2;
                if (!LAST) {
                    bov[sidx] = X[NW - 1] - drift2(NW - 1);
                    if ((pk_max_u16(bov[sidx], tm2) ^ tm2) != 0u) last_bnd = j;
                }
            }
            bprev = bcur;
        }
        const bool alive = alive_bits != 0u;
        cm4[(int64_t)gq * WAVE] = make_uint4(cmv[0], cmv[1], cmv[2], cmv[3]);
        if (!LAST) bo4[(int64_t)gq * WAVE] = make_uint4(bov[0], bov[1], bov[2], bov[3]);
        if (DIAG_PRUNE && __builtin_amdgcn_ballot_w64(alive) == 0) {
            if (4 * gq + 3 > l_in) { ++gq; break; }
            if (DIAG_GAP_SKIP) {
                int g2 = gq + 1;
                bool resume = false;
                uint4 bb = b_n;
                uint32_t in_prev = bv[3];
                for (; g2 < ngq; ++g2) {
                    if (g2 > gq + 1) bb = g2 < stop_prev ? bi4[(int64_t)g2 * WAVE] : bias4;
                    const uint32_t bbv[5] = {in_prev, bb.x, bb.y, bb.z, bb.w};
                    uint32_t in_bits = 0;
#pragma unroll
                    for (int sidx = 0; sidx < 5; ++sidx) {
                        const int j = 4 * g2 + sidx - 1;
                        const int t1 = max(4 * j - slack + (int)BIAS16 - 1, 0);
                        const uint32_t tm2 = j <= lq_lane ? (uint32_t)t1 * 0x00010001u : 0xFFFFFFFFu;
                        in_bits |= pk_max_u16(bbv[sidx], tm2) ^ tm2;
                    }
                    if (__builtin_amdgcn_ballot_w64(in_bits != 0u) != 0) { resume = true; break; }
                    cm4[(int64_t)g2 * WAVE] = bias4;
                    if (!LAST) bo4[(int64_t)g2 * WAVE] = bias4;
                    in_prev = bb.w;
                    if (4 * g2 + 3 > l_in) { ++g2; break; }
                }
                n_gap_groups += g2 - (gq + 1);
                if (!resume) { gq = g2; break; }
#pragma unroll
                for (int i = 0; i < NW; ++i) X[i] = BIAS2 + drift2(i);
                bprev = in_prev;
                b_n = bb;
                rc_n = rows1[(int64_t)g2 * WAVE];
                gq = g2 - 1;
            }
        }
    }
    if ((threadIdx.x & 63) == 0) {
        DSA_STAT_ADD(g, DS_GAP_GROUPS, n_gap_groups);
        DSA_STAT_ADD(g, DS_GROUPS_SKIPPED, ngq - gq);
        DSA_STAT_ADD(g, DS_GROUPS, ngq);
    }
    return gq;
}

__host__ __device__ constexpr int tier_of(int n_groups) { return n_groups <= GMAX ? 0 : n_groups <= GSPLIT ? 1 : 2; }
#ifndef DSA_FAST_WGS
#define DSA_FAST_WGS 4
#endif
template <int TIER, bool WIDE = false>
__global__ __launch_bounds__(WG_LANES, TIER == 2 ? 2 : DSA_FAST_WGS) void k_fill_fast(const dsa_pair* __restrict__ pairs,
                                                           uint8_t* __restrict__ wg_tier,
                                                           const uint32_t* __restrict__ refcodes,
                                                           const uint8_t* __restrict__ read_bytes,
                                                           uint32_t* __restrict__ rowcodes, uint32_t* __restrict__ row_bytes,
                                                           const int32_t* __restrict__ min_score_tab,
                                                           const dsa_fusion* __restrict__ fusions,
                                                           uint32_t* __restrict__ bnd, uint32_t* __restrict__ cmax,
                                                           uint32_t* __restrict__ rmax, uint32_t* __restrict__ tmask,
                                                           FinishBufs fb, Geom g)
{
    constexpr bool SPLIT = TIER > 0;
    __shared__ __attribute__((aligned(16))) uint32_t T[TIER == 2 ? GSPLIT2 * TGROUP_SPLIT : GMAX * TGROUP];
    __shared__ int s_nch, s_exotic;
    __shared__ FinishLds fl;
    __shared__ WgGroupsLds gl;
    if (TIER != 0 && wg_tier[blockIdx.x] != TIER) return;
    const int w = __builtin_amdgcn_readfirstlane((int)(blockIdx.x * WG_WAVES + (threadIdx.x >> 6)));
    const bool live = w < g.n_waves;
    const int lane = threadIdx.x & 63;
    const int64_t p = (int64_t)w * WAVE + lane;
    const bool in_batch = p < g.n_pairs;
    const dsa_pair pr = pairs[min(p, g.n_pairs - 1)];
    const int f = pr.fusion_idx;
    int my_group;
    const WgView wgi = wg_groups(&gl, f, (lane == 0 && threadIdx.x != 0) ? pairs[min(p - 1, g.n_pairs - 1)].fusion_idx : -1, my_group);
    if (TIER == 0) {
        const int tier = wgi.n_groups == 0 ? (int)TIER_GENERIC : tier_of(wgi.n_groups);
        if (threadIdx.x == 0) {
            wg_tier[blockIdx.x] = (uint8_t)tier;
            if (tier != 0) atomicOr(&fb.ctr->need_tiers, 1u << tier);
        }
        if (tier != 0) return;
    }
    int lq_lane = 0, slack = 0, tiles_lane = 0, tail_cols_lane = 0;
    if (in_batch) {
        const dsa_fusion fu = fusions[f];
        lq_lane = pr.read_len;
        slack = 2 * lq_lane - max(min_score_tab[lq_lane], pair_bound(pr));
        tiles_lane = max(cdiv_dev(fu.ref0_len, W), cdiv_dev(fu.ref1_len, W));
        tail_cols_lane = max(fu.ref0_len, fu.ref1_len) - (tiles_lane - 1) * W;
    }
    auto wave_max = [](int v) {
#pragma unroll
        for (int d = 32; d >= 1; d >>= 1) v = max(v, __shfl_xor(v, d, 64));
        return v;
    };
    WaveInfo wi;
    wi.lq_max = wave_max(lq_lane);
    wi.nch_max = wave_max(tiles_lane);
    int l_in = wave_max(lq_lane > 0 ? min(slack >> 2, lq_lane) : 0);
    const bool exotic = live && pack_rows_wave<SPLIT ? 2 : 1>(read_bytes, pairs, rowcodes, row_bytes, g, w, lane, wi.lq_max);
    if (threadIdx.x == 0) { s_nch = 0; s_exotic = 0; }
    __syncthreads();
    if (lane == 0 && live) atomicMax(&s_nch, wi.nch_max);
    if (__builtin_amdgcn_ballot_w64(exotic) != 0 && lane == 0) atomicOr(&s_exotic, 1);
    __syncthreads();
    if (s_exotic != 0) {
        if (threadIdx.x == 0) {
            wg_tier[blockIdx.x] = TIER_GENERIC;
            atomicOr(&fb.ctr->need_tiers, 1u << TIER_GENERIC);
        }
        return;
    }
    if (threadIdx.x == 0) atomicAdd(&fb.ctr->fill_wgs[FILL_WGS_FAST + 2 * TIER + (WIDE ? 1 : 0)], 1u);
    const int nch_wg = s_nch;

    const uint32_t* tb = T + my_group * (SPLIT ? TGROUP_SPLIT : TGROUP);
    const uint32_t* rows1 = row_bytes + (int64_t)w * (g.lq1 >> 2) * WAVE + lane;
    int stop_prev = 0;
    TileStops stops = {};

    const int tail_cols = wave_max(in_batch && tiles_lane == wi.nch_max ? tail_cols_lane : 0);
    DiagClock clk_all, clk;
    unsigned long long t_bar = 0, t_tab = 0;
    for (int c = 0; c < nch_wg; ++c) {
        clk.lap();
        __syncthreads();
        t_bar += clk.lap();
        build_tables<SPLIT>(T, wgi.n_groups, [&](int gi, int i, uint32_t& q0, uint32_t& q1) {
            const uint32_t code = refcodes[(int64_t)group_fusion(wgi, gi) * g.lrp + c * W + i];
            q0 = code & 0xFFFFu;
            q1 = code >> 16;
        });
        t_tab += clk.lap();
        __syncthreads();
        t_bar += clk.lap();
        if (!live || c >= wi.nch_max) continue;

        uint4* cm4 = reinterpret_cast<uint4*>(cmax + ((int64_t)w * g.nch + c) * g.lq1 * WAVE) + lane;
        uint4* bo4 = reinterpret_cast<uint4*>(bnd + ((int64_t)w * g.nch + c) * g.lq1 * WAVE) + lane;
        const uint4* bi4 = reinterpret_cast<const uint4*>(bnd + ((int64_t)w * g.nch + (c - 1)) * g.lq1 * WAVE) + lane;
        int last_bnd = 0, gq;
        if (c + 1 < wi.nch_max)
            gq = sweep_tile_fast<W, SPLIT, false>(tb, rows1, bi4, cm4, bo4, c == 0, wi.lq_max, lq_lane, slack, l_in, stop_prev, last_bnd, g);
        else if (!DIAG_NARROW || tail_cols > 16)
            gq = sweep_tile_fast<W, SPLIT, true>(tb, rows1, bi4, cm4, bo4, c == 0, wi.lq_max, lq_lane, slack, l_in, stop_prev, last_bnd, g);
        else
            gq = sweep_tile_fast<16, SPLIT, true>(tb, rows1, bi4, cm4, bo4, c == 0, wi.lq_max, lq_lane, slack, l_in, stop_prev, last_bnd, g);
        if (lane == 0) fb.tstop[(int64_t)w * g.nch + c] = gq;
        stop_prev = gq;
#pragma unroll
        for (int k = 0; k < 8; ++k)
            if (k == c) stops.v[k] = gq;
        l_in = wave_max(last_bnd);
    }
    clk.lap();
    unsigned long long t_rowmax = 0, t_combine = 0, t_replay = 0;
    if (DIAG_TAIL) {
        if (live) {
            __builtin_amdgcn_fence(__ATOMIC_RELEASE, "workgroup");
            reduce_row_max<WIDE>(cmax, rmax, tmask, fb.tstop, stops, g, w, lane, wi.nch_max, wi.lq_max);
        }
        t_rowmax = clk.lap();
        combine_wg<true>(pairs, fusions, cmax, rmax, tmask, min_score_tab, wgi, my_group, true, &fl, fb, g);
        t_combine = clk.lap();
        if (DIAG_REPLAY) replay_fast_wg<SPLIT>(T, &fl, wgi, fb, refcodes, rowcodes, bnd, g);
        t_replay = clk.lap();
    }
    if (lane == 0 && live) {
        DSA_STAT_ADD(g, DS_WAVE_CYCLES, clk_all.lap());
        DSA_STAT_ADD(g, DS_BARRIER, t_bar);
        DSA_STAT_ADD(g, DS_TABLES, t_tab);
        DSA_STAT_ADD(g, DS_TAIL, t_rowmax + t_combine + t_replay);
        DSA_STAT_ADD(g, DS_ROWMAX, t_rowmax);
        DSA_STAT_ADD(g, DS_COMBINE, t_combine);
        DSA_STAT_ADD(g, DS_REPLAY, t_replay);
    }
    (void)t_bar; (void)t_tab; (void)t_rowmax; (void)t_combine; (void)t_replay;
}

constexpr int REPLAY_BLOCK = 256;
constexpr int RQ = 4;
constexpr int RW = W / RQ;
constexpr int REPLAY_TASKS = REPLAY_BLOCK / RQ;

__device__ __forceinline__ void row_step_quarter(uint32_t (&X)[RW], const uint32_t (&r)[RW], uint32_t cj, uint32_t bprev, uint32_t bcur)
{
    cj &= CODE_MASK;
    uint32_t d[RW];
#pragma unroll
    for (int k = 0; k < RW; ++k) d[k] = k + 1 < RW ? SIX2 - min3u(cj ^ r[k + 1]) : 0u;
    uint32_t a = (bprev + FOUR2) - min3u(cj ^ r[0]);
    uint32_t up = bcur - TWO2;
#pragma unroll
    for (int i = 0; i < RW; ++i) {
        const uint32_t a_next = X[i] + d[i];
        X[i] = max3(a, X[i], up);
        up = X[i];
        a = a_next;
    }
}

__device__ __forceinline__ uint32_t equal_columns_quarter(const uint32_t (&X)[RW], uint32_t target2)
{
    static_assert(RW == 16, "one accumulator word");
    const uint32_t below = target2 - 0x00010001u;
    uint32_t acc = 0;
#pragma unroll
    for (int k = RW - 1; k >= 0; --k) {
        typedef unsigned short us2 __attribute__((ext_vector_type(2)));
        const uint32_t c = below + drift2(k);
        const uint32_t y = __builtin_bit_cast(uint32_t, __builtin_elementwise_sub_sat(__builtin_bit_cast(us2, X[k]), __builtin_bit_cast(us2, c)));
        asm("v_lshl_or_b32 %0, %0, 1, %1" : "+v"(acc) : "v"(y));
    }
    return acc;
}

__global__ __launch_bounds__(REPLAY_BLOCK, 5) void k_replay(const ReplayTask* __restrict__ tasks, uint64_t task_cap,
                                                   const uint2* __restrict__ gtasks, uint64_t gtask_cap,
                                                   const Counters* __restrict__ ctr,
                                                   const PairState* __restrict__ state,
                                                   const KeptRow* __restrict__ kept, uint64_t kept_cap,
                                                   const dsa_pair* __restrict__ pairs,
                                                   const dsa_fusion* __restrict__ fusions,
                                                   const uint32_t* __restrict__ refcodes,
                                                   const uint32_t* __restrict__ rowcodes,
                                                   const uint32_t* __restrict__ bnd, const int32_t* __restrict__ tstop,
                                                   uint64_t* __restrict__ masks, uint64_t mask_cap, Geom g)
{
    __shared__ int s_hist[258];
    __shared__ unsigned short s_order[REPLAY_TASKS];
    __shared__ ReplayTask s_task[REPLAY_TASKS];
    __shared__ uint64_t s_kc[KCACHE * REPLAY_BLOCK];
    static_assert(REPLAY_BLOCK == WG_LANES, "kept_row() strides the cache by WG_LANES");
    const unsigned long long n_g = ctr->n_gtasks;
    if (ctr->n_tasks > task_cap || ctr->n_masks > mask_cap || ctr->n_kept > kept_cap || n_g > gtask_cap) return;
    if (ctr->need_tiers & ~g.tiers_launched) return;
    const int q = threadIdx.x & (RQ - 1);
    const int slot = threadIdx.x / RQ;
    for (unsigned long long base = (unsigned long long)blockIdx.x * REPLAY_TASKS; base < n_g;
         base += (unsigned long long)gridDim.x * REPLAY_TASKS) {
        __syncthreads();
        for (int e = threadIdx.x; e < 258; e += REPLAY_BLOCK) s_hist[e] = 0;
        __syncthreads();
        int my_key = 256, my_rank = 0;
        if (threadIdx.x < REPLAY_TASKS) {
            if (base + threadIdx.x < n_g) {
                const ReplayTask mine = tasks[gtasks[base + threadIdx.x].x & ~GTASK_OWNER];
                s_task[threadIdx.x] = mine;
                my_key = min((int)(mine.last_row & TASK_ROW), 255);
            }
            my_rank = atomicAdd(&s_hist[my_key], 1);
        }
        __syncthreads();
        if (threadIdx.x == 0) {
            int run = 0;
            for (int e = 0; e < 257; ++e) {
                const int n = s_hist[e];
                s_hist[e] = run;
                run += n;
            }
        }
        __syncthreads();
        if (threadIdx.x < REPLAY_TASKS) s_order[s_hist[my_key] + my_rank] = (unsigned short)threadIdx.x;
        __syncthreads();
        const int src = s_order[slot];
        const bool valid = base + src < n_g;
        if (__builtin_amdgcn_ballot_w64(valid) == 0) continue;
        ReplayTask rt = s_task[valid ? src : s_order[0]];
        if (!valid) { rt.last_row = 0; rt.chunk0 = rt.chunk1 = NO_CHUNK; }
        DiagClock clk;
        const int64_t p = rt.pair;
        const int64_t w = p >> 6;
        const int lane = (int)(p & 63);
        const bool has0 = rt.chunk0 != NO_CHUNK, has1 = rt.chunk1 != NO_CHUNK;
        const int c0 = has0 ? rt.chunk0 : 0, c1 = has1 ? rt.chunk1 : 0;
        const uint32_t* rc = refcodes + (int64_t)rt.fusion * g.lrp;
        const dsa_fusion fu = fusions[rt.fusion];
        PairState st = state[p];
        if (!valid) st.n_kept = 0;
        const int lq = pairs[p].read_len;
        const uint32_t* rows = rowcodes + w * g.lq1 * WAVE;
        const uint32_t* bi0 = bnd + (w * g.nch + (c0 - 1)) * g.lq1 * WAVE;
        const uint32_t* bi1 = bnd + (w * g.nch + (c1 - 1)) * g.lq1 * WAVE;
        const KeptRow* kr = kept + st.kept_begin;

        uint32_t r[RW];
#pragma unroll
        for (int i = 0; i < RW; ++i) {
            const uint32_t lo = has0 ? (rc[c0 * W + q * RW + i] & 0xFFFFu) : REF_PAD16;
            const uint32_t hi = has1 ? (rc[c1 * W + q * RW + i] & 0xFFFF0000u) : (REF_PAD16 << 16);
            r[i] = lo | hi;
        }
        uint32_t X[RW];
#pragma unroll
        for (int i = 0; i < RW; ++i) X[i] = BIAS2 + drift2(i);
        const int R = rt.last_row & TASK_ROW;
        const int nv0 = has0 ? min(W, fu.ref0_len - c0 * W) : 0;
        const int nv1 = has1 ? min(W, fu.ref1_len - c1 * W) : 0;
        {
            const uint2* kr2 = reinterpret_cast<const uint2*>(kr);
            uint2 first[KCACHE];
#pragma unroll
            for (int k = 0; k < KCACHE; ++k) first[k] = kr2[k < (int)st.n_kept ? k : (st.n_kept ? (int)st.n_kept - 1 : 0)];
#pragma unroll
            for (int k = 0; k < KCACHE; ++k) s_kc[k * REPLAY_BLOCK + threadIdx.x] = ((uint64_t)first[k].y << 32) | first[k].x;
        }
        const uint64_t* kc = s_kc + threadIdx.x;
        HitCursor hc = cursor_init(kr, kc, st.n_kept, lq, has0, has1, nv0, nv1);
        const uint32_t my_valid0 = (uint32_t)(hc.valid0 >> (q * RW)) & 0xFFFFu, my_valid1 = (uint32_t)(hc.valid1 >> (q * RW)) & 0xFFFFu;
        const int stop0 = c0 > 0 ? tstop[w * g.nch + (c0 - 1)] : 0;
        const int stop1 = c1 > 0 ? tstop[w * g.nch + (c1 - 1)] : 0;
        auto plane_at = [&](int j) -> int64_t { return ((int64_t)(j >> 2) * WAVE + lane) * 4 + (j & 3); };
        auto row_code = [&](int j) -> uint32_t { return rows[plane_at(j < 0 ? 0 : j > R ? R : j)]; };
        auto boundary = [&](int j) -> uint32_t {
            const int jj = j < 0 ? 0 : j > R ? R : j;
            const uint32_t x0 = (jj >> 2) < stop0 ? bi0[plane_at(jj)] : BIAS2;
            const uint32_t x1 = (jj >> 2) < stop1 ? bi1[plane_at(jj)] : BIAS2;
            return (x0 & 0xFFFFu) | (x1 & 0xFFFF0000u);
        };
        int Rw = R;
#pragma unroll
        for (int d = 32; d >= 1; d >>= 1) Rw = max(Rw, __shfl_xor(Rw, d, 64));
        uint32_t rc_n = row_code(1 - q), rc_nn = row_code(2 - q);
        uint32_t b_n = q == 0 ? boundary(1) : BIAS2, b_nn = q == 0 ? boundary(2) : BIAS2;
        uint32_t bprev = BIAS2;
        uint32_t xlast = BIAS2;
        const unsigned long long t_setup = clk.lap();
        for (int t = 1; t <= Rw + RQ - 1; ++t) {
            const int j = t - q;
            const uint32_t cj = rc_n;
            const uint32_t from_left = __shfl_up(xlast, 1, RQ);
            const uint32_t bcur = q == 0 ? b_n : from_left;
            rc_n = rc_nn;
            b_n = b_nn;
            rc_nn = row_code(j + 2);
            if (q == 0) b_nn = boundary(j + 2);
            if (j >= 1 && j <= R) {
                row_step_quarter(X, r, cj, bprev, bcur);
                const bool hit0 = hc.row0 == j, hit1 = hc.row1 == j;
                if (hit0 || hit1) {
                    const uint32_t bits = equal_columns_quarter(X, (hit0 ? hc.t0 : NO_TARGET16) | ((hit1 ? hc.t1 : NO_TARGET16) << 16));
                    if (hit0) {
                        reinterpret_cast<unsigned short*>(masks + ((uint64_t)rt.mask_begin + hc.k0) * 2)[q] = (unsigned short)(bits & my_valid0);
                        ++hc.k0;
                        cursor_next0(hc, kr, kc, st.n_kept, has0);
                    }
                    if (hit1) {
                        reinterpret_cast<unsigned short*>(masks + ((uint64_t)rt.mask_begin + hc.k1) * 2 + 1)[q] = (unsigned short)((bits >> 16) & my_valid1);
                        --hc.k1;
                        cursor_next1(hc, kr, kc, lq, has1);
                    }
                }
                bprev = bcur;
                xlast = X[RW - 1] - drift2(RW - 1);
            }
        }
        if (valid && q == 0 && !has0)
            for (int k = 0; k < st.n_kept; ++k) masks[((uint64_t)rt.mask_begin + k) * 2] = 0;
        if (valid && q == 0 && !has1)
            for (int k = 0; k < st.n_kept; ++k) masks[((uint64_t)rt.mask_begin + k) * 2 + 1] = 0;
        if ((threadIdx.x & 63) == 0) {
            DSA_STAT_ADD(g, DS_GREPLAY_SETUP, t_setup);
            DSA_STAT_ADD(g, DS_GREPLAY_SWEEP, clk.lap());
            DSA_STAT_ADD(g, DS_GREPLAY_WAVES, 1);
            DSA_STAT_ADD(g, DS_GREPLAY_STEPS, Rw + RQ - 1);
        }
        (void)t_setup;
    }
}

__global__ void k_reset_finish(Counters* ctr, int64_t* rec_count_end)
{
    if (threadIdx.x == 0) {
        ctr->n_kept = ctr->n_tasks = ctr->n_masks = ctr->n_gtasks = 0;
        ctr->need_tiers = 0;
        for (int k = 0; k < 8; ++k) ctr->fill_wgs[k] = 0;
        *rec_count_end = 0;
    }
}

struct PlanGlobals;
__global__ void k_publish(const Counters* __restrict__ ctr, const int64_t* __restrict__ n_rec, const unsigned long long* __restrict__ plan,
                          Counters* host_ctr, int64_t* host_n_rec, unsigned long long* host_plan)
{
    if (threadIdx.x == 0) {
        *host_ctr = *ctr;
        *host_n_rec = *n_rec;
        host_plan[0] = plan[0];
        host_plan[1] = plan[1];
        __threadfence_system();
    }
}

__device__ __forceinline__ bool col_in(const ReplayTask* tasks, const uint64_t* masks, uint32_t tb, uint32_t te,
                                       int k, int h, int col )
{
    const int c = (col - 1) / W, bit = (col - 1) % W;
    for (uint32_t q = tb; q < te; ++q)
        if ((h ? tasks[q].chunk1 : tasks[q].chunk0) == c)
            return (masks[((uint64_t)tasks[q].mask_begin + k) * 2 + h] >> bit) & 1ull;
    return false;
}

constexpr int EMIT_BLOCK = 128;
constexpr int EMIT_SLOTS_COUNTED = 1, EMIT_SLOTS_LISTED = 16;
constexpr int EMIT_REG_ROWS = 4;
template <int SLOTS>
struct EmitLds {
    uint4 mask[SLOTS][EMIT_BLOCK];
    uint2 kept[SLOTS][EMIT_BLOCK];
};

template <bool WRITE, int SLOTS>
__device__ __forceinline__ int64_t emit_pair(EmitLds<SLOTS>* lds, int64_t p, int64_t o, const PairState& st, const dsa_pair* __restrict__ pairs,
                                             const dsa_fusion* __restrict__ fusions, const KeptRow* __restrict__ kept,
                                             const ReplayTask* __restrict__ tasks, const uint64_t* __restrict__ masks,
                                             const int64_t* __restrict__ rec_offset, dsa_record* __restrict__ out, uint64_t out_cap,
                                             int64_t pair_base)
{
    const int tid = threadIdx.x;
    int64_t n = 0;
    int64_t wr = 0;
    dsa_record rec = {};
    int ref1_len = 0;
    if (WRITE) {
        const dsa_pair pr = pairs[p];
        wr = rec_offset[o];
        const int64_t wr_end = rec_offset[o + 1];
        const dsa_fusion fu = fusions[pr.fusion_idx];
        if ((uint64_t)wr_end > out_cap) return 0;
        rec.fusion_id = fu.fusion_id;
        rec.frag = pr.frag;
        rec.read_end = pr.read_end;
        rec.revcomp = pr.revcomp;
        rec.read_second = pr.read_len;
        rec.pair_idx = (int32_t)(pair_base + o);
        ref1_len = fu.ref1_len;
    }
    auto put = [&](int i1, int i2, const KeptRow& kr) {
        if (WRITE) {
            dsa_record r = rec;
            r.ref_first = i1;
            r.ref_second = ref1_len - i2 - 1;
            r.read_first = kr.a;
            r.read_second = rec.read_second - kr.a;
            r.score = kr.m1 < kr.m2 ? kr.m1 : kr.m2;
            uint2* dst = reinterpret_cast<uint2*>(out + wr);
            const uint2* src = reinterpret_cast<const uint2*>(&r);
#pragma unroll
            for (int q = 0; q < 5; ++q) dst[q] = src[q];
        }
        ++wr;
        ++n;
    };
    const int K = st.n_kept, T = (int)st.n_tasks;
    const bool tiles = (st.flags & STATE_TILES) != 0;
    if (tiles && T == 1 && K <= EMIT_REG_ROWS) {
        const uint4* masks4 = reinterpret_cast<const uint4*>(masks) + st.mask_begin;
        const uint2* kept2 = reinterpret_cast<const uint2*>(kept) + st.kept_begin;
        uint4 m[EMIT_REG_ROWS];
        uint2 kr2[EMIT_REG_ROWS];
#pragma unroll
        for (int e = 0; e < 2; ++e) {
            m[e] = masks4[e < K ? e : K - 1];
            kr2[e] = kept2[e < K ? e : K - 1];
        }
#pragma unroll
        for (int e = 2; e < EMIT_REG_ROWS; ++e) {
            m[e] = m[1];
            kr2[e] = kr2[1];
        }
        if (K > 2) {
#pragma unroll
            for (int e = 2; e < EMIT_REG_ROWS; ++e) {
                m[e] = masks4[e < K ? e : K - 1];
                kr2[e] = kept2[e < K ? e : K - 1];
            }
        }
        const bool both = st.tiles0 != 0 && st.tiles1 != 0;
        const int base1 = __builtin_ctz(st.tiles0 | 0x10000u) * W + 1, base2 = __builtin_ctz(st.tiles1 | 0x10000u) * W + 1;
        auto lo64 = [](const uint4& v) -> uint64_t { return ((uint64_t)v.y << 32) | v.x; };
        auto hi64 = [](const uint4& v) -> uint64_t { return ((uint64_t)v.w << 32) | v.z; };
#pragma unroll
        for (int k = 0; k < EMIT_REG_ROWS; ++k) {
            if (both && k < K) {
                const KeptRow kr = __builtin_bit_cast(KeptRow, kr2[k]);
                for (uint64_t r1 = lo64(m[k]); r1; r1 &= r1 - 1) {
                    const int b1 = __builtin_ctzll(r1);
                    for (uint64_t r2 = hi64(m[k]); r2; r2 &= r2 - 1) {
                        const int b2 = __builtin_ctzll(r2);
                        bool dup = false;
#pragma unroll
                        for (int k2 = 0; k2 < k; ++k2) dup = dup || (((lo64(m[k2]) >> b1) & 1ull) && ((hi64(m[k2]) >> b2) & 1ull));
                        if (!dup) put(base1 + b1, base2 + b2, kr);
                    }
                }
            }
        }
    } else if (tiles) {
        const uint4* masks4 = reinterpret_cast<const uint4*>(masks) + st.mask_begin;
        const uint2* kept2 = reinterpret_cast<const uint2*>(kept) + st.kept_begin;
        const int slots = K * T;
        const bool staged = slots <= SLOTS;
        if (staged) {
#pragma unroll
            for (int e0 = 0, e1 = 2; e0 < SLOTS; e0 = e1, e1 *= 2) {
                if (e0 == 0 || slots > e0) {
#pragma unroll
                    for (int e = e0; e < e1 && e < SLOTS; ++e) {
                        lds->mask[e][tid] = masks4[e < slots ? e : slots - 1];
                        lds->kept[e][tid] = kept2[e < K ? e : K - 1];
                    }
                }
            }
        }
        auto mask_of = [&](int k, int t, int h) -> uint64_t {
            const uint4 v = staged ? lds->mask[t * K + k][tid] : masks4[t * K + k];
            return h ? ((uint64_t)v.w << 32) | v.z : ((uint64_t)v.y << 32) | v.x;
        };
        for (int k = 0; k < K; ++k) {
            const KeptRow kr = __builtin_bit_cast(KeptRow, staged ? lds->kept[k][tid] : kept2[k]);
            for (uint32_t w0 = st.tiles0; w0; w0 &= w0 - 1) {
                const int c0 = __builtin_ctz(w0), t1 = task_of_tile(st.tiles0, st.first0, c0);
                for (uint64_t r1 = mask_of(k, t1, 0); r1; r1 &= r1 - 1) {
                    const int b1 = __builtin_ctzll(r1);
                    for (uint32_t w1 = st.tiles1; w1; w1 &= w1 - 1) {
                        const int c1 = __builtin_ctz(w1), t2 = task_of_tile(st.tiles1, st.first1, c1);
                        for (uint64_t r2 = mask_of(k, t2, 1); r2; r2 &= r2 - 1) {
                            const int b2 = __builtin_ctzll(r2);
                            bool dup = false;
                            for (int k2 = 0; k2 < k && !dup; ++k2) dup = ((mask_of(k2, t1, 0) >> b1) & 1ull) && ((mask_of(k2, t2, 1) >> b2) & 1ull);
                            if (!dup) put(c0 * W + b1 + 1, c1 * W + b2 + 1, kr);
                        }
                    }
                }
            }
        }
    } else {
        const uint32_t tb = st.task_begin, te = tb + st.n_tasks;
        for (int k = 0; k < K; ++k) {
            const KeptRow kr = kept[st.kept_begin + k];
            for (uint32_t q1 = tb; q1 < te; ++q1) {
                if (tasks[q1].chunk0 == NO_CHUNK) continue;
                uint64_t m1 = masks[((uint64_t)tasks[q1].mask_begin + k) * 2];
                while (m1) {
                    const int i1 = tasks[q1].chunk0 * W + __builtin_ctzll(m1) + 1;
                    m1 &= m1 - 1;
                    for (uint32_t q2 = tb; q2 < te; ++q2) {
                        if (tasks[q2].chunk1 == NO_CHUNK) continue;
                        uint64_t m2 = masks[((uint64_t)tasks[q2].mask_begin + k) * 2 + 1];
                        while (m2) {
                            const int i2 = tasks[q2].chunk1 * W + __builtin_ctzll(m2) + 1;
                            m2 &= m2 - 1;
                            bool dup = false;
                            for (int k2 = 0; k2 < k && !dup; ++k2)
                                dup = col_in(tasks, masks, tb, te, k2, 0, i1) && col_in(tasks, masks, tb, te, k2, 1, i2);
                            if (!dup) put(i1, i2, kr);
                        }
                    }
                }
            }
        }
    }
    return n;
}

template <bool WRITE, int SLOTS>
__device__ __forceinline__ int64_t emit_pair_wave(EmitLds<SLOTS>* lds, int64_t p, int64_t o, uint32_t mask_begin, uint32_t kept_begin, int K, int T,
                                                  uint32_t tiles0, uint32_t tiles1, int first0, int first1, const dsa_pair* __restrict__ pairs,
                                                  const dsa_fusion* __restrict__ fusions, const KeptRow* __restrict__ kept,
                                                  const uint64_t* __restrict__ masks, const int64_t* __restrict__ rec_offset,
                                                  dsa_record* __restrict__ out, uint64_t out_cap, int64_t pair_base)
{
    const int lane = threadIdx.x & 63, wbase = threadIdx.x & ~63;
    auto slot_m = [&](int e) -> uint4& { return lds->mask[e >> 6][wbase + (e & 63)]; };
    auto slot_k = [&](int e) -> uint2& { return lds->kept[e >> 6][wbase + (e & 63)]; };
    const uint4* masks4 = reinterpret_cast<const uint4*>(masks) + mask_begin;
    const uint2* kept2 = reinterpret_cast<const uint2*>(kept) + kept_begin;
    __builtin_amdgcn_wave_barrier();
    for (int e = lane; e < K * T; e += 64) slot_m(e) = masks4[e];
    for (int e = lane; e < K; e += 64) slot_k(e) = kept2[e];
    __builtin_amdgcn_fence(__ATOMIC_RELEASE, "wavefront");
    __builtin_amdgcn_wave_barrier();
    __builtin_amdgcn_fence(__ATOMIC_ACQUIRE, "wavefront");
    auto mask_of = [&](int k, int t, int h) -> uint64_t {
        const uint4 v = slot_m(t * K + k);
        return h ? ((uint64_t)v.w << 32) | v.z : ((uint64_t)v.y << 32) | v.x;
    };
    int64_t wr = 0;
    dsa_record rec = {};
    int ref1_len = 0;
    if (WRITE) {
        wr = rec_offset[o];
        if ((uint64_t)rec_offset[o + 1] > out_cap) return 0;
        const dsa_pair pr = pairs[p];
        const dsa_fusion fu = fusions[pr.fusion_idx];
        rec.fusion_id = fu.fusion_id;
        rec.frag = pr.frag;
        rec.read_end = pr.read_end;
        rec.revcomp = pr.revcomp;
        rec.read_second = pr.read_len;
        rec.pair_idx = (int32_t)(pair_base + o);
        ref1_len = fu.ref1_len;
    }
    auto row = [&](int k, auto&& fn) {
        for (uint32_t w0 = tiles0; w0; w0 &= w0 - 1) {
            const int c0 = __builtin_ctz(w0), t1 = task_of_tile(tiles0, first0, c0);
            for (uint64_t r1 = mask_of(k, t1, 0); r1; r1 &= r1 - 1) {
                const int b1 = __builtin_ctzll(r1);
                for (uint32_t w1 = tiles1; w1; w1 &= w1 - 1) {
                    const int c1 = __builtin_ctz(w1), t2 = task_of_tile(tiles1, first1, c1);
                    for (uint64_t r2 = mask_of(k, t2, 1); r2; r2 &= r2 - 1) {
                        const int b2 = __builtin_ctzll(r2);
                        bool dup = false;
                        for (int k2 = 0; k2 < k && !dup; ++k2) dup = ((mask_of(k2, t1, 0) >> b1) & 1ull) && ((mask_of(k2, t2, 1) >> b2) & 1ull);
                        if (!dup) fn(c0 * W + b1 + 1, c1 * W + b2 + 1);
                    }
                }
            }
        }
    };
    int64_t total = 0;
    for (int k0 = 0; k0 < K; k0 += 64) {
        const int k = k0 + lane;
        int n_row = 0;
        if (k < K) row(k, [&](int, int) { ++n_row; });
        int incl = n_row;
#pragma unroll
        for (int d = 1; d < 64; d <<= 1) {
            const int y = __shfl_up(incl, d, 64);
            if (lane >= d) incl += y;
        }
        if (WRITE && k < K) {
            const KeptRow kr = __builtin_bit_cast(KeptRow, slot_k(k));
            int64_t at = wr + total + (incl - n_row);
            row(k, [&](int i1, int i2) {
                dsa_record r = rec;
                r.ref_first = i1;
                r.ref_second = ref1_len - i2 - 1;
                r.read_first = kr.a;
                r.read_second = rec.read_second - kr.a;
                r.score = kr.m1 < kr.m2 ? kr.m1 : kr.m2;
                uint2* dst = reinterpret_cast<uint2*>(out + at);
                const uint2* src = reinterpret_cast<const uint2*>(&r);
#pragma unroll
                for (int q = 0; q < 5; ++q) dst[q] = src[q];
                ++at;
            });
        }
        total += __shfl(incl, 63, 64);
    }
    __builtin_amdgcn_wave_barrier();
    return total;
}

template <int SLOTS>
__device__ __forceinline__ bool emit_is_heavy(const PairState& st)
{
    const int slots = (int)st.n_kept * (int)st.n_tasks;
    if (st.n_tasks == 1 && st.n_kept <= EMIT_REG_ROWS) return false;
    return (st.flags & STATE_TILES) != 0 && slots > SLOTS && slots <= 64 * SLOTS;
}

template <bool WRITE, int SLOTS>
__device__ __forceinline__ int64_t emit_heavy_of_wave(EmitLds<SLOTS>* lds, bool heavy, int64_t p, int64_t o, const PairState& st,
                                                      const dsa_pair* __restrict__ pairs, const dsa_fusion* __restrict__ fusions,
                                                      const KeptRow* __restrict__ kept, const uint64_t* __restrict__ masks,
                                                      const int64_t* __restrict__ rec_offset, dsa_record* __restrict__ out, uint64_t out_cap,
                                                      int64_t pair_base)
{
    int64_t mine = 0;
    uint64_t todo = __builtin_amdgcn_ballot_w64(heavy);
    while (todo) {
        const int src = __builtin_ctzll(todo);
        todo &= todo - 1;
        const int64_t sp = __shfl((int)p, src, 64), so = __shfl((int)o, src, 64);
        const uint32_t mb = (uint32_t)__shfl((int)st.mask_begin, src, 64), kb = (uint32_t)__shfl((int)st.kept_begin, src, 64);
        const int packed = __shfl((int)st.n_kept | ((int)st.n_tasks << 16), src, 64);
        const int tl = __shfl((int)st.tiles0 | ((int)st.tiles1 << 16), src, 64);
        const int firsts = __shfl((int)st.first0 | ((int)st.first1 << 8), src, 64);
        const int64_t n = emit_pair_wave<WRITE, SLOTS>(lds, sp, so, mb, kb, packed & 0xFFFF, (packed >> 16) & 0xFF, (uint32_t)tl & 0xFFFFu,
                                                        (uint32_t)tl >> 16, firsts & 0xFF, (firsts >> 8) & 0xFF, pairs, fusions, kept, masks, rec_offset, out, out_cap, pair_base);
        if ((int)(threadIdx.x & 63) == src) mine = n;
    }
    return mine;
}

__global__ __launch_bounds__(EMIT_BLOCK) void k_emit_counted(const dsa_pair* __restrict__ pairs, const dsa_fusion* __restrict__ fusions,
                       const PairState* __restrict__ state, const KeptRow* __restrict__ kept,
                       const ReplayTask* __restrict__ tasks, const uint64_t* __restrict__ masks,
                       const int64_t* __restrict__ rec_offset, dsa_record* __restrict__ out, uint64_t out_cap, int64_t pair_base,
                       const Counters* __restrict__ ctr, uint64_t kept_cap, uint64_t task_cap, uint64_t mask_cap, uint64_t gtask_cap, Geom g)
{
    __shared__ EmitLds<EMIT_SLOTS_COUNTED> lds;
    if (ctr->n_tasks > task_cap || ctr->n_masks > mask_cap || ctr->n_kept > kept_cap || ctr->n_gtasks > gtask_cap) return;
    if (ctr->need_tiers & ~g.tiers_launched) return;
    const int64_t p = (int64_t)blockIdx.x * EMIT_BLOCK + threadIdx.x;
    PairState st = {};
    int64_t o = 0;
    if (p < g.n_pairs) {
        st = state[p];
        o = g.orig ? g.orig[p] : p;
    }
    const bool mine = p < g.n_pairs && (st.flags & STATE_COUNTED) && st.n_kept != 0;
    if (mine) emit_pair<true, EMIT_SLOTS_COUNTED>(&lds, p, o, st, pairs, fusions, kept, tasks, masks, rec_offset, out, out_cap, pair_base);
}

template <bool WRITE>
__global__ __launch_bounds__(EMIT_BLOCK) void k_emit_listed(const uint2* __restrict__ gtasks, uint64_t gtask_cap, const Counters* __restrict__ ctr,
                       const dsa_pair* __restrict__ pairs, const dsa_fusion* __restrict__ fusions,
                       const PairState* __restrict__ state, const KeptRow* __restrict__ kept,
                       const ReplayTask* __restrict__ tasks, uint64_t task_cap, const uint64_t* __restrict__ masks, uint64_t mask_cap,
                       uint64_t kept_cap, int64_t* __restrict__ rec_count, const int64_t* __restrict__ rec_offset,
                       dsa_record* __restrict__ out, uint64_t out_cap, int64_t pair_base, Geom g)
{
    __shared__ EmitLds<EMIT_SLOTS_LISTED> lds;
    const unsigned long long n_g = ctr->n_gtasks;
    if (ctr->n_tasks > task_cap || ctr->n_masks > mask_cap || ctr->n_kept > kept_cap || n_g > gtask_cap) return;
    if (ctr->need_tiers & ~g.tiers_launched) return;
    const unsigned long long stride = (unsigned long long)gridDim.x * EMIT_BLOCK;
    for (unsigned long long e0 = 0; e0 < n_g; e0 += stride) {
        const unsigned long long e = e0 + (unsigned long long)threadIdx.x * gridDim.x + blockIdx.x;
        uint2 entry = make_uint2(0u, 0u);
        if (e < n_g) entry = gtasks[e];
        const bool mine = (entry.x & GTASK_OWNER) != 0;
        const int64_t p = entry.y;
        PairState st = {};
        if (mine) st = state[p];
        const int64_t o = mine ? (g.orig ? g.orig[p] : p) : 0;
        const bool heavy = mine && emit_is_heavy<EMIT_SLOTS_LISTED>(st);
        DiagClock clk;
        int64_t n = 0;
        if (mine && !heavy) n = emit_pair<WRITE, EMIT_SLOTS_LISTED>(&lds, p, o, st, pairs, fusions, kept, tasks, masks, rec_offset, out, out_cap, pair_base);
        const int64_t nh = emit_heavy_of_wave<WRITE, EMIT_SLOTS_LISTED>(&lds, heavy, p, o, st, pairs, fusions, kept, masks, rec_offset, out, out_cap, pair_base);
        if (!WRITE && mine) rec_count[o] = heavy ? nh : n;
        if (!WRITE && mine)
            DSA_STAT_MAX(g, DS_SLOWEST_LISTED, (clk.lap() << 24) | ((unsigned long long)st.n_kept << 8) | st.n_tasks);
    }
}

}

#include "dsa_plan.hpp"
```

### defuse_amd/dsa.py

```python
import ctypes
import os

import numpy as np

_HERE = os.path.dirname(os.path.abspath(__file__))
LIB_PATH = os.environ.get("DEFUSE_DSA_LIB") or os.path.join(_HERE, "libdefuse_dsa.so")

FUSION_DTYPE = np.dtype([("fusion_id", "<i4"), ("ref0_off", "<i4"), ("ref0_len", "<i4"),
                         ("ref1_off", "<i4"), ("ref1_len", "<i4")])
PAIR_DTYPE = np.dtype([("fusion_idx", "<i4"), ("read_off", "<i4"), ("read_len", "<i4"), ("frag", "<i4"),
                       ("read_end", "u1"), ("revcomp", "u1"), ("pad_", "u1", (2,))])
RECORD_DTYPE = np.dtype([(n, "<i4") for n in ("fusion_id", "frag", "read_end", "revcomp", "ref_first",
                                             "ref_second", "read_first", "read_second", "score", "pair_idx")])
assert FUSION_DTYPE.itemsize == 20 and PAIR_DTYPE.itemsize == 20 and RECORD_DTYPE.itemsize == 40

EXPORTS = ["dsa_create", "dsa_destroy", "dsa_get_limits", "dsa_last_error", "dsa_version", "dsa_build_flags", "dsa_device_count", "dsa_pick_device", "dsa_pick_device_among", "dsa_set_plan_options", "dsa_set_scratch_budget", "dsa_share_scratch", "dsa_align_batch",
           "dsa_upload", "dsa_plan", "dsa_run", "dsa_download", "dsa_copy_records_device", "dsa_get_timing", "dsa_get_kernel_counts", "dsa_set_stream", "dsa_synchronize",
           "dsa_stream_create", "dsa_stream_destroy", "dsa_stream_submit", "dsa_stream_collect", "dsa_stream_recollect", "dsa_stream_last_error",
           "dsa_host_alloc", "dsa_host_free", "dsa_host_register", "dsa_host_unregister"]

PLAN_NO_REORDER, PLAN_NO_RANK, PLAN_NO_TIGHTEN, PLAN_NO_LPT = 1, 2, 4, 8
DSA_E_CAPACITY = -1
DSA_E_ARG = -3
DSA_E_BUSY = -5


class Limits(ctypes.Structure):
    _fields_ = [("max_read_len", ctypes.c_int32), ("max_ref_len", ctypes.c_int32), ("tile_cols", ctypes.c_int32)]


class Timing(ctypes.Structure):
    _fields_ = [("pack_ms", ctypes.c_float), ("fill_ms", ctypes.c_float), ("finish_ms", ctypes.c_float),
                ("total_ms", ctypes.c_float), ("fill_launches", ctypes.c_int32), ("n_generic_tasks", ctypes.c_int32),
                ("cells", ctypes.c_int64), ("n_records", ctypes.c_int64), ("n_replay_tasks", ctypes.c_int64),
                ("plan_ms", ctypes.c_float), ("pad_", ctypes.c_float)]


class KernelCounts(ctypes.Structure):
    _fields_ = [("fast_wgs", ctypes.c_int64 * 3), ("fast_wide_wgs", ctypes.c_int64 * 3), ("generic_wgs", ctypes.c_int64),
                ("workgroups", ctypes.c_int64), ("slices", ctypes.c_int64), ("slices_rerun", ctypes.c_int64),
                ("long_pairs", ctypes.c_int64), ("generic_tasks", ctypes.c_int64)]


class DsaError(RuntimeError):
    def __init__(self, code, msg):
        super().__init__("dsa error %d: %s" % (code, msg))
        self.code = code


_lib = None


def load_library():
    global _lib
    if _lib is None:
        if not os.path.exists(LIB_PATH):
            raise RuntimeError("%s missing: run `python -m defuse_amd.build`" % LIB_PATH)
        lib = ctypes.CDLL(LIB_PATH)
        vp, i32, i64 = ctypes.c_void_p, ctypes.c_int32, ctypes.c_int64
        lib.dsa_create.argtypes = [ctypes.POINTER(vp), ctypes.c_int]
        lib.dsa_destroy.argtypes = [vp]
        lib.dsa_destroy.restype = None
        lib.dsa_get_limits.argtypes = [vp, ctypes.POINTER(Limits)]
        lib.dsa_last_error.argtypes = [vp]
        lib.dsa_last_error.restype = ctypes.c_char_p
        lib.dsa_version.restype = ctypes.c_char_p
        lib.dsa_build_flags.restype = ctypes.c_char_p
        batch = [vp, vp, i64, vp, i32, vp, i64, vp, i64]
        lib.dsa_align_batch.argtypes = batch + [vp, i64, ctypes.POINTER(i64)]
        lib.dsa_upload.argtypes = batch
        lib.dsa_plan.argtypes = [vp]
        lib.dsa_run.argtypes = [vp, ctypes.POINTER(i64)]
        lib.dsa_download.argtypes = [vp, vp, i64, ctypes.POINTER(i64)]
        lib.dsa_copy_records_device.argtypes = [vp, vp, i64, ctypes.POINTER(i64)]
        lib.dsa_get_timing.argtypes = [vp, ctypes.POINTER(Timing)]
        lib.dsa_get_kernel_counts.argtypes = [vp, ctypes.POINTER(KernelCounts)]
        lib.dsa_set_stream.argtypes = [vp, vp]
        lib.dsa_synchronize.argtypes = [vp]
        lib.dsa_set_scratch_budget.argtypes = [vp, i64]
        lib.dsa_set_plan_options.argtypes = [vp, ctypes.c_uint]
        lib.dsa_share_scratch.argtypes = [vp, vp]
        lib.dsa_pick_device_among.argtypes = [ctypes.c_int]
        lib.dsa_stream_create.argtypes = [ctypes.POINTER(vp), ctypes.c_int, ctypes.c_int]
        lib.dsa_stream_destroy.argtypes = [vp]
        lib.dsa_stream_destroy.restype = None
        lib.dsa_stream_submit.argtypes = [vp] + batch[1:] + [vp, i64]
        lib.dsa_stream_collect.argtypes = [vp, ctypes.POINTER(i64)]
        lib.dsa_stream_recollect.argtypes = [vp, vp, i64, ctypes.POINTER(i64)]
        lib.dsa_stream_last_error.argtypes = [vp]
        lib.dsa_stream_last_error.restype = ctypes.c_char_p
        lib.dsa_host_alloc.argtypes = [ctypes.c_size_t]
        lib.dsa_host_alloc.restype = vp
        lib.dsa_host_free.argtypes = [vp]
        lib.dsa_host_free.restype = None
        lib.dsa_host_register.argtypes = [vp, ctypes.c_size_t]
        lib.dsa_host_unregister.argtypes = [vp]
        _lib = lib
    return _lib


def _check_arrays(ref_bytes, fusions, read_bytes, pairs):
    ref_bytes = np.ascontiguousarray(ref_bytes, dtype=np.uint8)
    read_bytes = np.ascontiguousarray(read_bytes, dtype=np.uint8)
    fusions = np.ascontiguousarray(fusions, dtype=FUSION_DTYPE)
    pairs = np.ascontiguousarray(pairs, dtype=PAIR_DTYPE)
    return ref_bytes, fusions, read_bytes, pairs


class Context:

    def __init__(self, device=0):
        self.lib = load_library()
        self.h = ctypes.c_void_p()
        self.device = int(device)
        rc = self.lib.dsa_create(ctypes.byref(self.h), int(device))
        if rc != 0:
            raise DsaError(rc, "dsa_create failed (no HIP device %d?)" % device)
        self._keep = None

    def close(self):
        if self.h:
            self.lib.dsa_destroy(self.h)
            self.h = ctypes.c_void_p()

    def __del__(self):
        try:
            self.close()
        except Exception:
            pass

    def _err(self, rc):
        raise DsaError(rc, self.lib.dsa_last_error(self.h).decode())

    def limits(self):
        lim = Limits()
        self.lib.dsa_get_limits(self.h, ctypes.byref(lim))
        return lim

    def set_plan_options(self, flags):
        rc = self.lib.dsa_set_plan_options(self.h, int(flags))
        if rc != 0:
            self._err(rc)

    def set_scratch_budget(self, nbytes):
        rc = self.lib.dsa_set_scratch_budget(self.h, int(nbytes))
        if rc != 0:
            self._err(rc)

    def share_scratch(self, donor):
        rc = self.lib.dsa_share_scratch(self.h, donor.h)
        if rc != 0:
            self._err(rc)

    def set_stream(self, stream_ptr):
        self.lib.dsa_set_stream(self.h, ctypes.c_void_p(stream_ptr))

    def upload(self, ref_bytes, fusions, read_bytes, pairs):
        ref_bytes, fusions, read_bytes, pairs = _check_arrays(ref_bytes, fusions, read_bytes, pairs)
        rc = self.lib.dsa_upload(self.h, ref_bytes.ctypes.data, ref_bytes.size, fusions.ctypes.data, len(fusions),
                                 read_bytes.ctypes.data, read_bytes.size, pairs.ctypes.data, len(pairs))
        if rc != 0:
            self._err(rc)

    def plan(self):
        rc = self.lib.dsa_plan(self.h)
        if rc != 0:
            self._err(rc)

    def run(self):
        n = ctypes.c_int64(0)
        rc = self.lib.dsa_run(self.h, ctypes.byref(n))
        if rc != 0:
            self._err(rc)
        return n.value

    def download(self):
        n = ctypes.c_int64(0)
        rc = self.lib.dsa_download(self.h, None, 0, ctypes.byref(n))
        if rc not in (0, DSA_E_CAPACITY):
            self._err(rc)
        out = np.zeros(n.value, dtype=RECORD_DTYPE)
        if n.value:
            rc = self.lib.dsa_download(self.h, out.ctypes.data, n.value, ctypes.byref(n))
            if rc != 0:
                self._err(rc)
        return out

    def records_to_device(self, device_ptr, capacity):
        n = ctypes.c_int64(0)
        rc = self.lib.dsa_copy_records_device(self.h, ctypes.c_void_p(device_ptr), int(capacity), ctypes.byref(n))
        if rc != 0:
            self._err(rc)
        return n.value

    def timing(self):
        t = Timing()
        self.lib.dsa_get_timing(self.h, ctypes.byref(t))
        return t

    def kernel_counts(self):
        k = KernelCounts()
        rc = self.lib.dsa_get_kernel_counts(self.h, ctypes.byref(k))
        if rc != 0:
            self._err(rc)
        return dict(fast=list(k.fast_wgs), fast_wide=list(k.fast_wide_wgs), generic=k.generic_wgs, workgroups=k.workgroups,
                    slices=k.slices, slices_rerun=k.slices_rerun, long_pairs=k.long_pairs, generic_tasks=k.generic_tasks)

    def align_batch_into(self, ref_bytes, fusions, read_bytes, pairs, out):
        n = ctypes.c_int64(0)
        rc = self.lib.dsa_align_batch(self.h, ref_bytes.ctypes.data, ref_bytes.size, fusions.ctypes.data, len(fusions),
                                      read_bytes.ctypes.data, read_bytes.size, pairs.ctypes.data, len(pairs),
                                      out.ctypes.data, len(out), ctypes.byref(n))
        if rc != 0:
            self._err(rc)
        return n.value

    def align_batch(self, ref_bytes, fusions, read_bytes, pairs):
        ref_bytes, fusions, read_bytes, pairs = _check_arrays(ref_bytes, fusions, read_bytes, pairs)
        cap = max(1024, 2 * len(pairs))
        while True:
# ... 98 lines not shown
```

### include/defuse_dsa.h

```cpp
#ifndef DEFUSE_DSA_H_
#define DEFUSE_DSA_H_

#include <stddef.h>
#include <stdint.h>

#ifdef __cplusplus
extern "C" {
#endif

#define DSA_OK            0
#define DSA_E_CAPACITY  (-1)
#define DSA_E_DEVICE    (-2)
#define DSA_E_ARG       (-3)
#define DSA_E_LIMIT     (-4)
#define DSA_E_BUSY      (-5)

#define DSA_MATCH       2
#define DSA_MISMATCH  (-1)
#define DSA_GAP       (-2)
#define DSA_MIN_SPLIT   8

typedef struct dsa_ctx dsa_ctx;

typedef struct dsa_fusion {
    int32_t fusion_id;
    int32_t ref0_off, ref0_len;
    int32_t ref1_off, ref1_len;
} dsa_fusion;

typedef struct dsa_pair {
    int32_t fusion_idx;
    int32_t read_off, read_len;
    int32_t frag;
    uint8_t read_end;
    uint8_t revcomp;
    uint8_t pad_[2];
} dsa_pair;

typedef struct dsa_record {
    int32_t fusion_id, frag, read_end, revcomp;
    int32_t ref_first, ref_second;
    int32_t read_first, read_second;
    int32_t score;
    int32_t pair_idx;
} dsa_record;

typedef struct dsa_limits {
    int32_t max_read_len;
    int32_t max_ref_len;
    int32_t tile_cols;
} dsa_limits;

typedef struct dsa_timing {
    float   pack_ms;
    float   fill_ms;
    float   finish_ms;
    float   total_ms;
    int32_t fill_launches;
    int32_t n_generic_tasks;
    int64_t cells;
    int64_t n_records;
    int64_t n_replay_tasks;
    float   plan_ms;
    float   pad_;
} dsa_timing;

typedef struct dsa_kernel_counts {
    int64_t fast_wgs[3];
    int64_t fast_wide_wgs[3];
    int64_t generic_wgs;
    int64_t workgroups;
    int64_t slices;
    int64_t slices_rerun;
    int64_t long_pairs;
    int64_t generic_tasks;
} dsa_kernel_counts;

int  dsa_create(dsa_ctx** out, int device);
void dsa_destroy(dsa_ctx* ctx);
int  dsa_get_limits(const dsa_ctx* ctx, dsa_limits* out);
const char* dsa_last_error(const dsa_ctx* ctx);
const char* dsa_version(void);
const char* dsa_build_flags(void);
int dsa_device_count(void);
int dsa_pick_device(void);
int dsa_pick_device_among(int n_devices);
#define DSA_PLAN_NO_REORDER  1u
#define DSA_PLAN_NO_RANK     2u
#define DSA_PLAN_NO_TIGHTEN  4u
#define DSA_PLAN_NO_LPT      8u
int dsa_set_plan_options(dsa_ctx* ctx, unsigned flags);
int dsa_set_scratch_budget(dsa_ctx* ctx, int64_t bytes);
int dsa_share_scratch(dsa_ctx* ctx, dsa_ctx* donor);

int dsa_align_batch(dsa_ctx* ctx,
                    const uint8_t* ref_bytes, int64_t ref_bytes_len,
                    const dsa_fusion* fusions, int32_t n_fusions,
                    const uint8_t* read_bytes, int64_t read_bytes_len,
                    const dsa_pair* pairs, int64_t n_pairs,
                    dsa_record* out, int64_t out_cap, int64_t* out_n);

int dsa_upload(dsa_ctx* ctx,
               const uint8_t* ref_bytes, int64_t ref_bytes_len,
               const dsa_fusion* fusions, int32_t n_fusions,
               const uint8_t* read_bytes, int64_t read_bytes_len,
               const dsa_pair* pairs, int64_t n_pairs);
int dsa_plan(dsa_ctx* ctx);
int dsa_run(dsa_ctx* ctx, int64_t* out_n);
int dsa_download(dsa_ctx* ctx, dsa_record* out, int64_t out_cap, int64_t* out_n);
int dsa_copy_records_device(dsa_ctx* ctx, void* out_device, int64_t out_cap, int64_t* out_n);
int dsa_get_timing(const dsa_ctx* ctx, dsa_timing* out);
int dsa_get_kernel_counts(const dsa_ctx* ctx, dsa_kernel_counts* out);
int dsa_set_stream(dsa_ctx* ctx, void* hip_stream);
int dsa_synchronize(dsa_ctx* ctx);

typedef struct dsa_stream dsa_stream;
int  dsa_stream_create(dsa_stream** out, int device, int depth);
void dsa_stream_destroy(dsa_stream* s);
int  dsa_stream_submit(dsa_stream* s,
                       const uint8_t* ref_bytes, int64_t ref_bytes_len,
                       const dsa_fusion* fusions, int32_t n_fusions,
                       const uint8_t* read_bytes, int64_t read_bytes_len,
                       const dsa_pair* pairs, int64_t n_pairs,
                       dsa_record* out, int64_t out_cap);
int  dsa_stream_collect(dsa_stream* s, int64_t* out_n);
int  dsa_stream_recollect(dsa_stream* s, dsa_record* out, int64_t out_cap, int64_t* out_n);
const char* dsa_stream_last_error(const dsa_stream* s);
void* dsa_host_alloc(size_t bytes);
void  dsa_host_free(void* p);
int   dsa_host_register(void* p, size_t bytes);
int   dsa_host_unregister(void* p);

#ifdef __cplusplus
}
#endif
#endif
```

Baseline: 286.4 million.

## Pick DP tile width per batch to cut padded columns in fill kernels

Templates the fill, replay and combine kernels on tile width (64, 60 or 56 columns) and picks at upload the width that minimises padded reference columns for the longest window, without changing the tile-count class. Refcodes keep a 64-column stride, with the unused columns padded. Narrower tiles shrink the per-lane register row and skip wasted cells when windows land just above a multiple of 64. In exchange there are more kernel instantiations, which grows code size and compile time, and index maths in the emit and pack paths now depends on the width.

```diff
diff --git a/defuse_amd/csrc/dsa_api.hip b/defuse_amd/csrc/dsa_api.hip
--- a/defuse_amd/csrc/dsa_api.hip
+++ b/defuse_amd/csrc/dsa_api.hip
@@ -10,6 +10,8 @@
 #include <memory>
 #include <mutex>
 #include <thread>
+#include <type_traits>
+#include <utility>
 #include <cstdio>
 #include <cstdlib>
 #include <cstring>
@@ -121,6 +123,7 @@
     DevBuf<uint8_t> d_ref, d_reads;
     DevBuf<dsa_fusion> d_fusions;
     int64_t upload_serial = 0;
+    int wt = W;
     int nch_all = 1;
     DevBuf<uint32_t> d_refcodes;
     hipEvent_t ev_pack[2] = {};
@@ -178,6 +181,17 @@
     return (int)((double)f * 0.90);
 }
 
+template <class Fn, int... K>
+void for_each_tile_width_impl(Fn&& fn, std::integer_sequence<int, K...>)
+{
+    (fn(std::integral_constant<int, TILE_WIDTHS[K]>{}), ...);
+}
+template <class Fn>
+void for_each_tile_width(Fn&& fn)
+{
+    for_each_tile_width_impl(fn, std::make_integer_sequence<int, N_TILE_WIDTHS>{});
+}
+
 size_t slice_scratch_bytes(int64_t n_waves, int lq1, int nch)
 {
     size_t rows = (size_t)n_waves * lq1 * WAVE * 4;
@@ -204,6 +218,7 @@
         cur.g.lq1 = lq1;
         cur.g.nch = ctx->nch_all;
         cur.g.lrp = ctx->nch_all * W;
+        cur.g.wt = ctx->wt;
         cur.g.n_fusions = ctx->n_fusions;
         cur.g.n_pairs = n;
         cur.g.orig = nullptr;
@@ -352,8 +367,8 @@
 {
     Geom g = s.g;
 #ifdef DSA_PRUNE_STATS
-    HIPC(L.d_stats.reserve(16));
-    HIPC(hipMemsetAsync(L.d_stats.p, 0, 16 * sizeof(unsigned long long), L.stream));
+    HIPC(L.d_stats.reserve(DS_SLOTS));
+    HIPC(hipMemsetAsync(L.d_stats.p, 0, DS_SLOTS * sizeof(unsigned long long), L.stream));
     g.stats = L.d_stats.p;
 #endif
     hipStream_t st = L.stream;
@@ -365,17 +380,29 @@
     const unsigned mask = L.tier_hint | 1u;
     L.tiers_launched = mask;
     g.tiers_launched = mask;
-#define DSA_LAUNCH_FILL(TIER, WIDE)                                                                                                              \
-    hipLaunchKernelGGL((k_fill_fast<TIER, WIDE>), dim3((unsigned)g.n_wgs), dim3(WG_LANES), 0, st, pairs, L.d_wg_tier.p, ctx->d_refcodes.p, \
+    const bool wide = g.nch > 8 && g.nch <= 16;
+    bool launched = false;
+    auto launch_fills = [&](auto wt_c, auto wide_c) {
+        constexpr int WT = decltype(wt_c)::value;
+        constexpr bool WIDE = decltype(wide_c)::value;
+        if (g.wt != WT || wide != WIDE) return;
+        launched = true;
+#define DSA_LAUNCH_FILL(TIER)                                                                                                                    \
+    hipLaunchKernelGGL((k_fill_fast<TIER, WIDE, WT>), dim3((unsigned)g.n_wgs), dim3(WG_LANES), 0, st, pairs, L.d_wg_tier.p, ctx->d_refcodes.p, \
                        ctx->d_reads.p, L.d_rowcodes.p, L.d_rowbytes.p, ctx->d_min_score.p, ctx->d_fusions.p, L.d_bnd.p, L.d_cmax.p, L.d_rmax.p, L.d_tmask.p, fb, g)
-    const bool wide = g.nch > 8 && g.nch <= 16;
-    if (wide) DSA_LAUNCH_FILL(0, true); else DSA_LAUNCH_FILL(0, false);
-    if (mask & 2u) { if (wide) DSA_LAUNCH_FILL(1, true); else DSA_LAUNCH_FILL(1, false); }
-    if (mask & 4u) { if (wide) DSA_LAUNCH_FILL(2, true); else DSA_LAUNCH_FILL(2, false); }
+        DSA_LAUNCH_FILL(0);
+        if (mask & 2u) DSA_LAUNCH_FILL(1);
+        if (mask & 4u) DSA_LAUNCH_FILL(2);
 #undef DSA_LAUNCH_FILL
-    if (mask & 8u)
-        hipLaunchKernelGGL(k_fill_generic, dim3((unsigned)g.n_wgs), dim3(WG_LANES), 0, st, pairs, ctx->d_fusions.p, L.d_wg_tier.p, ctx->d_refcodes.p,
-                           ctx->d_reads.p, L.d_rowcodes.p, ctx->d_min_score.p, L.d_bnd.p, L.d_cmax.p, L.d_rmax.p, L.d_tmask.p, fb, g);
+        if (mask & 8u)
+            hipLaunchKernelGGL((k_fill_generic<WT>), dim3((unsigned)g.n_wgs), dim3(WG_LANES), 0, st, pairs, ctx->d_fusions.p, L.d_wg_tier.p, ctx->d_refcodes.p,
+                               ctx->d_reads.p, L.d_rowcodes.p, ctx->d_min_score.p, L.d_bnd.p, L.d_cmax.p, L.d_rmax.p, L.d_tmask.p, fb, g);
+    };
+    for_each_tile_width([&](auto wt_c) {
+        launch_fills(wt_c, std::false_type{});
+        launch_fills(wt_c, std::true_type{});
+    });
+    if (!launched) return fail(ctx, DSA_E_DEVICE, "internal: no fill kernel for tile width %d", g.wt);
     HIPC(hipEventRecord(L.ev[2], st));
     hipLaunchKernelGGL(k_replay, dim3(2048), dim3(REPLAY_BLOCK), 0, st, L.d_tasks.p, (uint64_t)L.d_tasks.cap, L.d_gtasks.p,
                        (uint64_t)L.d_gtasks.cap, L.d_ctr.p, L.d_state.p, L.d_kept.p, (uint64_t)L.d_kept.cap, pairs, ctx->d_fusions.p,
@@ -655,6 +682,10 @@
     return DSA_OK;
 }
 
+int dsa_tile_cols_for(int32_t max_window) { return pick_tile_width(max_window); }
+
+int dsa_tile_cols_in_use(const dsa_ctx* ctx) { return ctx ? ctx->wt : 0; }
+
 const char* dsa_last_error(const dsa_ctx* ctx) { return ctx ? ctx->err.c_str() : "no context"; }
 
 int dsa_set_stream(dsa_ctx* ctx, void* hip_stream)
@@ -690,7 +721,7 @@
     ctx->h_long_fusions.clear();
     ctx->long_cells = 0;
     ctx->long_blank_cells = 0;
-    int nch_all = 1, maxwin = 0;
+    int maxwin = 0;
     for (int32_t f = 0; f < n_fusions; ++f) {
         const dsa_fusion& fu = fusions[f];
         if (fu.ref0_len < 0 || fu.ref1_len < 0 || fu.ref0_off < 0 || fu.ref1_off < 0 ||
@@ -702,9 +733,14 @@
             ctx->h_long_fusions.push_back(f);
             continue;
         }
-        nch_all = std::max<int>(nch_all, std::max(grid_of(fu.ref0_len, W), grid_of(fu.ref1_len, W)));
         maxwin = std::max(maxwin, std::max(fu.ref0_len, fu.ref1_len));
     }
+    int wt = pick_tile_width(maxwin);
+    if (const char* e = getenv("DEFUSE_DSA_TILE_COLS")) {
+        if (!is_tile_width(atoi(e))) return fail(ctx, DSA_E_ARG, "DEFUSE_DSA_TILE_COLS=%s is not a built tile width", e);
+        wt = atoi(e);
+    }
+    const int nch_all = std::max(1, tiles_of(maxwin, wt));
     const bool any_long_fusion = !ctx->h_long_fusions.empty();
     int lqmax = 0;
     for (int64_t p = 0; p < n_pairs; ++p) {
@@ -748,6 +784,7 @@
     HIPC(ctx->d_reads.reserve((size_t)read_bytes_len + 64));
     HIPC(ctx->d_fusions.reserve((size_t)n_fusions + 1));
     HIPC(ctx->d_pairs_in.reserve((size_t)n_pairs + 1));
+    ctx->wt = wt;
     ctx->nch_all = nch_all;
     HIPC(ctx->d_refcodes.reserve((size_t)n_fusions * nch_all * W + 1));
     if (ref_bytes_len) HIPC(hipMemcpyAsync(ctx->d_ref.p, ref_bytes, ref_bytes_len, hipMemcpyHostToDevice, st));
@@ -777,7 +814,7 @@
         ctx->plan_prm.n_fusions = n_fusions;
         ctx->plan_prm.slots = slots;
         ctx->plan_prm.wc = (mw + 2 * PLAN_PAD + 47) / 16 + 1;
-        ctx->plan_prm.tile_cols = W;
+        ctx->plan_prm.tile_cols = wt;
     }
     make_slices(ctx, n_pairs, lqmax);
     HIPC(hipGetLastError());
diff --git a/defuse_amd/csrc/dsa_diag.hpp b/defuse_amd/csrc/dsa_diag.hpp
--- a/defuse_amd/csrc/dsa_diag.hpp
+++ b/defuse_amd/csrc/dsa_diag.hpp
@@ -13,11 +13,6 @@
 #else
 constexpr bool DIAG_GAP_SKIP = true;
 #endif
-#ifdef DSA_NARROW
-constexpr bool DIAG_NARROW = true;
-#else
-constexpr bool DIAG_NARROW = false;
-#endif
 #ifdef DSA_ABLATE_TAIL
 constexpr bool DIAG_TAIL = false;
 #else
@@ -32,7 +27,10 @@
 enum DiagSlot {
     DS_GROUPS_SKIPPED = 0, DS_GROUPS = 1, DS_UNUSED2 = 2, DS_WAVE_CYCLES = 3, DS_BARRIER = 4, DS_TABLES = 5, DS_TAIL = 6, DS_ROWMAX = 7,
     DS_COMBINE = 8, DS_REPLAY = 9, DS_GREPLAY_SETUP = 10, DS_GREPLAY_SWEEP = 11, DS_GREPLAY_WAVES = 12, DS_GREPLAY_STEPS = 13,
-    DS_GAP_GROUPS = 14, DS_SLOWEST_LISTED = 15
+    DS_GAP_GROUPS = 14, DS_SLOWEST_LISTED = 15,
+    DS_TILE_GROUPS = 16,
+    DS_TILE_CYCLES = 32,
+    DS_TILE_SLOTS = 16, DS_SLOTS = 48
 };
 
 #ifdef DSA_PRUNE_STATS
diff --git a/defuse_amd/csrc/dsa_diag_host.hpp b/defuse_amd/csrc/dsa_diag_host.hpp
--- a/defuse_amd/csrc/dsa_diag_host.hpp
+++ b/defuse_amd/csrc/dsa_diag_host.hpp
@@ -24,7 +24,7 @@
         for (int b = 0; b < 10; ++b) fprintf(stderr, " %ld", hist[k][b]);
         fprintf(stderr, "\n");
     }
-    unsigned long long h[16];
+    unsigned long long h[DS_SLOTS];
     (void)hipMemcpy(h, d_stats, sizeof h, hipMemcpyDeviceToHost);
     const double wc = h[DS_WAVE_CYCLES] ? (double)h[DS_WAVE_CYCLES] : 1.0;
     fprintf(stderr,
@@ -36,6 +36,13 @@
     fprintf(stderr, "[stats] left-over replay: %llu waves, set-up %llu, sweep %llu cycles, %llu steps (lane 0); slowest lane of the listed count: %llu cycles, "
             "%llu kept rows, %llu tasks\n", h[DS_GREPLAY_WAVES], h[DS_GREPLAY_SETUP], h[DS_GREPLAY_SWEEP], h[DS_GREPLAY_STEPS], h[DS_SLOWEST_LISTED] >> 24,
             (h[DS_SLOWEST_LISTED] >> 8) & 0xFFFF, h[DS_SLOWEST_LISTED] & 0xFF);
+    unsigned long long tg = 0, tc = 0;
+    for (int c = 0; c < DS_TILE_SLOTS; ++c) { tg += h[DS_TILE_GROUPS + c]; tc += h[DS_TILE_CYCLES + c]; }
+    fprintf(stderr, "[stats] fill sweeps by tile, swept row groups %% / sweep cycles %%:");
+    for (int c = 0; c < DS_TILE_SLOTS; ++c)
+        if (h[DS_TILE_GROUPS + c] || h[DS_TILE_CYCLES + c])
+            fprintf(stderr, " t%d %.1f / %.1f", c, 100.0 * h[DS_TILE_GROUPS + c] / (tg ? tg : 1), 100.0 * h[DS_TILE_CYCLES + c] / (tc ? tc : 1));
+    fprintf(stderr, " (swept row groups %llu, sweep cycles %.4g)\n", tg, (double)tc);
 }
 
 inline void diag_dump_plan()
diff --git a/defuse_amd/csrc/dsa_kernels.hpp b/defuse_amd/csrc/dsa_kernels.hpp
--- a/defuse_amd/csrc/dsa_kernels.hpp
+++ b/defuse_amd/csrc/dsa_kernels.hpp
@@ -4,10 +4,11 @@
 
 #include "../../include/defuse_dsa.h"
 #include "dsa_diag.hpp"
+#include "dsa_tile.hpp"
 
 namespace dsa {
 
-constexpr int W = 64;
+constexpr int W = TILE_W;
 constexpr int WAVE = 64;
 constexpr int WG_WAVES = 4;
 constexpr int WG_LANES = WG_WAVES * WAVE;
@@ -127,6 +128,7 @@
     int32_t lq1;
     int32_t nch;
     int32_t lrp;
+    int32_t wt;
     int32_t n_fusions;
     int64_t n_pairs;
     const int32_t* orig;
@@ -198,9 +200,14 @@
     int64_t t = (int64_t)blockIdx.x * blockDim.x + threadIdx.x;
     int64_t total = (int64_t)g.n_fusions * g.lrp;
     if (t >= total) return;
-    const int i = (int)(t % g.lrp);
+    const int s = (int)(t % g.lrp), k = s % W;
+    const int i = (s / W) * g.wt + k;
     const dsa_fusion f = fusions[t / g.lrp];
     uint32_t lo = REF_PAD16, hi = REF_PAD16;
+    if (k >= g.wt) {
+        refcodes[t] = lo | (hi << 16);
+        return;
+    }
     if (i < f.ref0_len) lo = (uint32_t)ref_bytes[(int64_t)f.ref0_off + i] << 8;
     if (i < f.ref1_len) hi = (uint32_t)ref_bytes[(int64_t)f.ref1_off + (f.ref1_len - 1 - i)] << 8;
     refcodes[t] = lo | (hi << 16);
@@ -228,11 +235,11 @@
     else { k1 = t - 21; k2 = 4; }
 }
 
-template <bool SPLIT, class CodeFn>
+template <bool SPLIT, int WT, class CodeFn>
 __device__ __forceinline__ void build_tables(uint32_t* __restrict__ T, int n_groups, CodeFn&& code_of)
 {
-    for (int e = threadIdx.x; e < n_groups * W; e += WG_LANES) {
-        const int i = e & (W - 1), gi = e >> 6;
+    for (int e = threadIdx.x; e < n_groups * WT; e += WG_LANES) {
+        const int i = e % WT, gi = e / WT;
         uint32_t q0, q1;
         code_of(gi, i, q0, q1);
         const uint32_t cls_byte[NCLS] = {'A', 'C', 'T', 'G', 'N'};
@@ -296,7 +303,8 @@
     return exotic;
 }
 
-__device__ __forceinline__ void row_step(uint32_t (&X)[W], const uint32_t (&r)[W], uint32_t cj, uint32_t bprev,
+template <int WT>
+__device__ __forceinline__ void row_step(uint32_t (&X)[WT], const uint32_t (&r)[WT], uint32_t cj, uint32_t bprev,
                                          uint32_t bcur)
 {
     cj &= CODE_MASK;
@@ -304,13 +312,13 @@
     uint32_t a = (bprev + FOUR2) - min3u(cj ^ r[0]);
     uint32_t up = bcur - TWO2;
 #pragma unroll
-    for (int b = 0; b < W; b += BLK) {
+    for (int b = 0; b < WT; b += BLK) {
         uint32_t d[BLK];
 #pragma unroll
         for (int k = 0; k < BLK; ++k)
-            d[k] = b + k + 1 < W ? SIX2 - min3u(cj ^ r[b + k + 1]) : 0u;
-#pragma unroll
-        for (int k = 0; k < BLK; ++k) {
+            d[k] = b + k + 1 < WT ? SIX2 - min3u(cj ^ r[b + k + 1]) : 0u;
+#pragma unroll
+        for (int k = 0; k < BLK && b + k < WT; ++k) {
             const int i = b + k;
             const uint32_t a_next = X[i] + d[k];
             X[i] = max3(a, X[i], up);
@@ -320,12 +328,13 @@
     }
 }
 
-template <bool MASKED>
-__device__ __forceinline__ uint32_t tile_row_max(const uint32_t (&X)[W], int nv0, int nv1)
+template <bool MASKED, int WT>
+__device__ __forceinline__ uint32_t tile_row_max(const uint32_t (&X)[WT], int nv0, int nv1)
 {
     uint32_t acc0 = BIAS2, acc1 = BIAS2;
-#pragma unroll
-    for (int i = 0; i < W; i += 4) {
+    static_assert(WT % 4 == 0, "four columns per step");
+#pragma unroll
+    for (int i = 0; i < WT; i += 4) {
         uint32_t x[4];
 #pragma unroll
         for (int k = 0; k < 4; ++k) {
@@ -418,7 +427,7 @@
     for (int q = 0; q < 4; ++q) base[q] = __shfl(b[q], 63, 64) + (incl[q] - n[q]);
 }
 
-template <bool HANDOFF>
+template <bool HANDOFF, int WT>
 __device__ __forceinline__ void combine_wg(
     const dsa_pair* __restrict__ pairs, const dsa_fusion* __restrict__ fusions, const uint32_t* __restrict__ cmax,
     const uint32_t* __restrict__ rmax, const uint32_t* __restrict__ tmask, const int32_t* __restrict__ min_score_tab,
@@ -459,8 +468,8 @@
         lq = pr.read_len;
         len0 = fu.ref0_len;
         len1 = fu.ref1_len;
-        nc0 = cdiv_dev(fu.ref0_len, W);
-        nc1 = cdiv_dev(fu.ref1_len, W);
+        nc0 = cdiv_dev(fu.ref0_len, WT);
+        nc1 = cdiv_dev(fu.ref1_len, WT);
         small = nc0 <= 64 && nc1 <= 64;
         const int min_score = min_score_tab[lq];
         if (g.nch <= TMASK_TILES) {
@@ -638,9 +647,9 @@
         li.c1 = here ? (uint8_t)c1 : NO_CHUNK;
         li.key_group = (uint16_t)((fold_a < 255 ? fold_a : 255) | ((gsel >= 0 ? gsel : 0) << 8));
         li.lq = (uint16_t)lq;
-        const int v0 = len0 - c0 * W, v1 = len1 - c1 * W;
-        li.nv0 = (uint8_t)(here && c0 != NO_CHUNK ? (v0 < W ? (v0 > 0 ? v0 : 0) : W) : 0);
-        li.nv1 = (uint8_t)(here && c1 != NO_CHUNK ? (v1 < W ? (v1 > 0 ? v1 : 0) : W) : 0);
+        const int v0 = len0 - c0 * WT, v1 = len1 - c1 * WT;
+        li.nv0 = (uint8_t)(here && c0 != NO_CHUNK ? (v0 < WT ? (v0 > 0 ? v0 : 0) : WT) : 0);
+        li.nv1 = (uint8_t)(here && c1 != NO_CHUNK ? (v1 < WT ? (v1 > 0 ? v1 : 0) : WT) : 0);
         fl->info[tid] = li;
     }
     if (!active) return;
@@ -748,7 +757,8 @@
 }
 
 constexpr uint32_t NO_TARGET16 = 0x7F00u;
-__device__ __forceinline__ void equal_columns(const uint32_t (&X)[W], uint32_t target2, uint64_t& m0, uint64_t& m1)
+template <int WT>
+__device__ __forceinline__ void equal_columns(const uint32_t (&X)[WT], uint32_t target2, uint64_t& m0, uint64_t& m1)
 {
     uint32_t hit[W / 16];
     const uint32_t below = target2 - 0x00010001u;
@@ -758,6 +768,7 @@
 #pragma unroll
         for (int k = 15; k >= 0; --k) {
             const int i = 16 * q + k;
+            if (i >= WT) continue;
             const uint32_t c = below + drift2(i);
             typedef unsigned short us2 __attribute__((ext_vector_type(2)));
             const uint32_t y = __builtin_bit_cast(uint32_t, __builtin_elementwise_sub_sat(__builtin_bit_cast(us2, X[i]), __builtin_bit_cast(us2, c)));
@@ -771,7 +782,8 @@
     m1 = (uint64_t)hi_a | ((uint64_t)hi_b << 32);
 }
 
-__device__ __forceinline__ void record_hits(const uint32_t (&X)[W], int j, int lq, const KeptRow* __restrict__ kr,
+template <int WT>
+__device__ __forceinline__ void record_hits(const uint32_t (&X)[WT], int j, int lq, const KeptRow* __restrict__ kr,
                                             const uint64_t* kc, int n_kept, bool has0, bool has1, HitCursor& hc,
                                             uint64_t* __restrict__ masks, uint32_t mask_begin)
 {
@@ -811,7 +823,7 @@
     return n;
 }
 
-template <bool SPLIT>
+template <bool SPLIT, int WT>
 __device__ __forceinline__ void replay_fast_wg(uint32_t* T, FinishLds* fl, const WgView& wgi, const FinishBufs& fb,
                                                const uint32_t* __restrict__ refcodes, const uint32_t* __restrict__ rowcodes,
                                                const uint32_t* __restrict__ bnd, const Geom& g)
@@ -821,7 +833,7 @@
     bool any = false;
     for (int k = 0; k < wgi.n_groups; ++k) any |= fl->tile[k] >= 0;
     if (!any) return;
-    build_tables<SPLIT>(T, wgi.n_groups, [&](int gi, int i, uint32_t& q0, uint32_t& q1) {
+    build_tables<SPLIT, WT>(T, wgi.n_groups, [&](int gi, int i, uint32_t& q0, uint32_t& q1) {
         const int key = fl->tile[gi];
         q0 = q1 = REF_PAD16;
         if (key >= 0) {
@@ -878,9 +890,9 @@
     const int stop0 = c0 > 0 ? load_tstop(fb.tstop + wr * g.nch + (c0 - 1)) : 0;
     const int stop1 = c1 > 0 ? load_tstop(fb.tstop + wr * g.nch + (c1 - 1)) : 0;
 
-    uint32_t X[W];
-#pragma unroll
-    for (int i = 0; i < W; ++i) X[i] = BIAS2 + drift2(i);
+    uint32_t X[WT];
+#pragma unroll
+    for (int i = 0; i < WT; ++i) X[i] = BIAS2 + drift2(i);
     const uint4 bias4 = make_uint4(BIAS2, BIAS2, BIAS2, BIAS2);
     uint32_t bprev = BIAS2;
     const int ngq = (Rw >> 2) + 1;
@@ -912,9 +924,9 @@
                 uint32_t a = bprev + v.x;
                 uint32_t up = bcur - TWO2;
 #pragma unroll
-                for (int q = 0; q < W / 4; ++q) {
+                for (int q = 0; q < WT / 4; ++q) {
                     uint4 vn = v;
-                    if (q + 1 < W / 4) vn = table4(q + 1);
+                    if (q + 1 < WT / 4) vn = table4(q + 1);
                     uint32_t an;
                     an = X[4 * q + 0] + v.y;
                     X[4 * q + 0] = max3(a, X[4 * q + 0], up);
@@ -944,15 +956,15 @@
         fb.rec_count[g.orig ? g.orig[p] : p] = count_one_tile_pair(masks + (uint64_t)li.mask_begin * 2, n_kept);
 }
 
-template <bool MASKED>
-__device__ __forceinline__ int sweep_tile_generic(const uint32_t (&r)[W], const uint4* __restrict__ rows4,
+template <bool MASKED, int WT>
+__device__ __forceinline__ int sweep_tile_generic(const uint32_t (&r)[WT], const uint4* __restrict__ rows4,
                                                   const uint4* __restrict__ bi4, uint4* __restrict__ cm4,
                                                   uint4* __restrict__ bo4, int lq, bool first, int nv0, int nv1,
                                                   int lq_lane, int slack, int l_in, int stop_prev, int& last_bnd)
 {
-    uint32_t X[W];
-#pragma unroll
-    for (int i = 0; i < W; ++i) X[i] = BIAS2 + drift2(i);
+    uint32_t X[WT];
+#pragma unroll
+    for (int i = 0; i < WT; ++i) X[i] = BIAS2 + drift2(i);
     const uint4 bias4 = make_uint4(BIAS2, BIAS2, BIAS2, BIAS2);
     uint32_t bprev = BIAS2;
     const int ngq = (lq >> 2) + 1;
@@ -974,7 +986,7 @@
             if (j >= 1 && j <= lq) {
                 row_step(X, r, rcv[sidx], bprev, bv[sidx]);
                 cmv[sidx] = tile_row_max<MASKED>(X, nv0, nv1);
-                bov[sidx] = X[W - 1] - drift2(W - 1);
+                bov[sidx] = X[WT - 1] - drift2(WT - 1);
                 const int thr = 4 * j - slack + (int)BIAS16;
                 const bool in_read = j <= lq_lane;
                 alive |= in_read && ((int)(cmv[sidx] & 0xFFFFu) >= thr || (int)(cmv[sidx] >> 16) >= thr);
@@ -1092,6 +1104,7 @@
     }
 }
 
+template <int WT>
 __global__ __launch_bounds__(WG_LANES) void k_fill_generic(const dsa_pair* __restrict__ pairs,
                                                            const dsa_fusion* __restrict__ fusions,
                                                            const uint8_t* __restrict__ wg_tier,
@@ -1120,7 +1133,7 @@
         };
         WaveInfo wi;
         wi.lq_max = wave_max(in_batch ? (int)pairs[p].read_len : 0);
-        wi.nch_max = wave_max(in_batch ? max(cdiv_dev(fu.ref0_len, W), cdiv_dev(fu.ref1_len, W)) : 0);
+        wi.nch_max = wave_max(in_batch ? max(cdiv_dev(fu.ref0_len, WT), cdiv_dev(fu.ref1_len, WT)) : 0);
         (void)pack_rows_wave<0>(read_bytes, pairs, rowcodes, nullptr, g, w, lane, wi.lq_max);
         const uint32_t* rc = refcodes + (int64_t)f * g.lrp;
         const uint4* rows4 = reinterpret_cast<const uint4*>(rowcodes + (int64_t)w * g.lq1 * WAVE) + lane;
@@ -1134,18 +1147,18 @@
         TileStops stops = {};
 
         for (int c = 0; c < wi.nch_max; ++c) {
-            uint32_t r[W];
-#pragma unroll
-            for (int i = 0; i < W; ++i) r[i] = rc[c * W + i];
-            const int nv0 = fu.ref0_len - c * W, nv1 = fu.ref1_len - c * W;
+            uint32_t r[WT];
+#pragma unroll
+            for (int i = 0; i < WT; ++i) r[i] = rc[c * W + i];
+            const int nv0 = fu.ref0_len - c * WT, nv1 = fu.ref1_len - c * WT;
             uint4* cm4 = reinterpret_cast<uint4*>(cmax + ((int64_t)w * g.nch + c) * g.lq1 * WAVE) + lane;
             uint4* bo4 = reinterpret_cast<uint4*>(bnd + ((int64_t)w * g.nch + c) * g.lq1 * WAVE) + lane;
             const uint4* bi4 = reinterpret_cast<const uint4*>(bnd + ((int64_t)w * g.nch + (c - 1)) * g.lq1 * WAVE) + lane;
             int last_bnd, stop;
-            if (__builtin_amdgcn_ballot_w64(nv0 < W || nv1 < W) == 0)
-                stop = sweep_tile_generic<false>(r, rows4, bi4, cm4, bo4, wi.lq_max, c == 0, nv0, nv1, lq_lane, slack, l_in, stop_prev, last_bnd);
+            if (__builtin_amdgcn_ballot_w64(nv0 < WT || nv1 < WT) == 0)
+                stop = sweep_tile_generic<false, WT>(r, rows4, bi4, cm4, bo4, wi.lq_max, c == 0, nv0, nv1, lq_lane, slack, l_in, stop_prev, last_bnd);
             else
-                stop = sweep_tile_generic<true>(r, rows4, bi4, cm4, bo4, wi.lq_max, c == 0, nv0, nv1, lq_lane, slack, l_in, stop_prev, last_bnd);
+                stop = sweep_tile_generic<true, WT>(r, rows4, bi4, cm4, bo4, wi.lq_max, c == 0, nv0, nv1, lq_lane, slack, l_in, stop_prev, last_bnd);
             if (lane == 0) fb.tstop[(int64_t)w * g.nch + c] = stop;
             stop_prev = stop;
 #pragma unroll
@@ -1158,16 +1171,16 @@
     }
     WgView wgi = {};
     wgi.list = nullptr;
-    combine_wg<false>(pairs, fusions, cmax, rmax, tmask, min_score_tab, wgi, 0, false, &fl, fb, g);
+    combine_wg<false, WT>(pairs, fusions, cmax, rmax, tmask, min_score_tab, wgi, 0, false, &fl, fb, g);
 }
 
 template <int NW, bool SPLIT, bool LAST>
 __device__ __forceinline__ int sweep_tile_fast(const uint32_t* __restrict__ tb, const uint32_t* __restrict__ rows1, const uint4* __restrict__ bi4,
                                                uint4* __restrict__ cm4, uint4* __restrict__ bo4, bool first_tile, int lq_max, int lq_lane,
-                                               int slack, int l_in, int stop_prev, int& last_bnd, const Geom& g)
-{
-    static_assert(NW % 4 == 0 && NW / 4 > FILL_PF, "table reads in flight");
-    (void)g;
+                                               int slack, int l_in, int stop_prev, int& last_bnd, const Geom& g, int tile)
+{
+    static_assert(NW % 4 == 0 && NW / 4 > FILL_PF && NW <= W, "table reads in flight");
+    (void)g; (void)tile;
     uint32_t X[NW];
 #pragma unroll
     for (int i = 0; i < NW; ++i) X[i] = BIAS2 + drift2(i);
@@ -1309,6 +1322,7 @@
         DSA_STAT_ADD(g, DS_GAP_GROUPS, n_gap_groups);
         DSA_STAT_ADD(g, DS_GROUPS_SKIPPED, ngq - gq);
         DSA_STAT_ADD(g, DS_GROUPS, ngq);
+        DSA_STAT_ADD(g, DS_TILE_GROUPS + (tile < DS_TILE_SLOTS ? tile : DS_TILE_SLOTS - 1), gq - n_gap_groups);
     }
     return gq;
 }
@@ -1317,7 +1331,7 @@
 #ifndef DSA_FAST_WGS
 #define DSA_FAST_WGS 4
 #endif
-template <int TIER, bool WIDE = false>
+template <int TIER, bool WIDE, int WT>
 __global__ __launch_bounds__(WG_LANES, TIER == 2 ? 2 : DSA_FAST_WGS) void k_fill_fast(const dsa_pair* __restrict__ pairs,
                                                            uint8_t* __restrict__ wg_tier,
                                                            const uint32_t* __restrict__ refcodes,
@@ -1352,13 +1366,12 @@
         }
         if (tier != 0) return;
     }
-    int lq_lane = 0, slack = 0, tiles_lane = 0, tail_cols_lane = 0;
+    int lq_lane = 0, slack = 0, tiles_lane = 0;
     if (in_batch) {
         const dsa_fusion fu = fusions[f];
         lq_lane = pr.read_len;
         slack = 2 * lq_lane - max(min_score_tab[lq_lane], pair_bound(pr));
-        tiles_lane = max(cdiv_dev(fu.ref0_len, W), cdiv_dev(fu.ref1_len, W));
-        tail_cols_lane = max(fu.ref0_len, fu.ref1_len) - (tiles_lane - 1) * W;
+        tiles_lane = max(cdiv_dev(fu.ref0_len, WT), cdiv_dev(fu.ref1_len, WT));
     }
     auto wave_max = [](int v) {
 #pragma unroll
@@ -1390,14 +1403,13 @@
     int stop_prev = 0;
     TileStops stops = {};
 
-    const int tail_cols = wave_max(in_batch && tiles_lane == wi.nch_max ? tail_cols_lane : 0);
     DiagClock clk_all, clk;
     unsigned long long t_bar = 0, t_tab = 0;
     for (int c = 0; c < nch_wg; ++c) {
         clk.lap();
         __syncthreads();
         t_bar += clk.lap();
-        build_tables<SPLIT>(T, wgi.n_groups, [&](int gi, int i, uint32_t& q0, uint32_t& q1) {
+        build_tables<SPLIT, WT>(T, wgi.n_groups, [&](int gi, int i, uint32_t& q0, uint32_t& q1) {
             const uint32_t code = refcodes[(int64_t)group_fusion(wgi, gi) * g.lrp + c * W + i];
             q0 = code & 0xFFFFu;
             q1 = code >> 16;
@@ -1412,11 +1424,10 @@
         const uint4* bi4 = reinterpret_cast<const uint4*>(bnd + ((int64_t)w * g.nch + (c - 1)) * g.lq1 * WAVE) + lane;
         int last_bnd = 0, gq;
         if (c + 1 < wi.nch_max)
-            gq = sweep_tile_fast<W, SPLIT, false>(tb, rows1, bi4, cm4, bo4, c == 0, wi.lq_max, lq_lane, slack, l_in, stop_prev, last_bnd, g);
-        else if (!DIAG_NARROW || tail_cols > 16)
-            gq = sweep_tile_fast<W, SPLIT, true>(tb, rows1, bi4, cm4, bo4, c == 0, wi.lq_max, lq_lane, slack, l_in, stop_prev, last_bnd, g);
+            gq = sweep_tile_fast<WT, SPLIT, false>(tb, rows1, bi4, cm4, bo4, c == 0, wi.lq_max, lq_lane, slack, l_in, stop_prev, last_bnd, g, c);
         else
-            gq = sweep_tile_fast<16, SPLIT, true>(tb, rows1, bi4, cm4, bo4, c == 0, wi.lq_max, lq_lane, slack, l_in, stop_prev, last_bnd, g);
+            gq = sweep_tile_fast<WT, SPLIT, true>(tb, rows1, bi4, cm4, bo4, c == 0, wi.lq_max, lq_lane, slack, l_in, stop_prev, last_bnd, g, c);
+        if (lane == 0) DSA_STAT_ADD(g, DS_TILE_CYCLES + (c < DS_TILE_SLOTS ? c : DS_TILE_SLOTS - 1), clk.lap());
         if (lane == 0) fb.tstop[(int64_t)w * g.nch + c] = gq;
         stop_prev = gq;
 #pragma unroll
@@ -1432,9 +1443,9 @@
             reduce_row_max<WIDE>(cmax, rmax, tmask, fb.tstop, stops, g, w, lane, wi.nch_max, wi.lq_max);
         }
         t_rowmax = clk.lap();
-        combine_wg<true>(pairs, fusions, cmax, rmax, tmask, min_score_tab, wgi, my_group, true, &fl, fb, g);
+        combine_wg<true, WT>(pairs, fusions, cmax, rmax, tmask, min_score_tab, wgi, my_group, true, &fl, fb, g);
         t_combine = clk.lap();
-        if (DIAG_REPLAY) replay_fast_wg<SPLIT>(T, &fl, wgi, fb, refcodes, rowcodes, bnd, g);
+        if (DIAG_REPLAY) replay_fast_wg<SPLIT, WT>(T, &fl, wgi, fb, refcodes, rowcodes, bnd, g);
         t_replay = clk.lap();
     }
     if (lane == 0 && live) {
@@ -1566,8 +1577,8 @@
 #pragma unroll
         for (int i = 0; i < RW; ++i) X[i] = BIAS2 + drift2(i);
         const int R = rt.last_row & TASK_ROW;
-        const int nv0 = has0 ? min(W, fu.ref0_len - c0 * W) : 0;
-        const int nv1 = has1 ? min(W, fu.ref1_len - c1 * W) : 0;
+        const int nv0 = has0 ? min(g.wt, fu.ref0_len - c0 * g.wt) : 0;
+        const int nv1 = has1 ? min(g.wt, fu.ref1_len - c1 * g.wt) : 0;
         {
             const uint2* kr2 = reinterpret_cast<const uint2*>(kr);
             uint2 first[KCACHE];
@@ -1664,9 +1675,9 @@
 }
 
 __device__ __forceinline__ bool col_in(const ReplayTask* tasks, const uint64_t* masks, uint32_t tb, uint32_t te,
-                                       int k, int h, int col )
-{
-    const int c = (col - 1) / W, bit = (col - 1) % W;
+                                       int k, int h, int col , int wt)
+{
+    const int c = (col - 1) / wt, bit = (col - 1) % wt;
     for (uint32_t q = tb; q < te; ++q)
         if ((h ? tasks[q].chunk1 : tasks[q].chunk0) == c)
             return (masks[((uint64_t)tasks[q].mask_begin + k) * 2 + h] >> bit) & 1ull;
@@ -1687,7 +1698,7 @@
                                              const dsa_fusion* __restrict__ fusions, const KeptRow* __restrict__ kept,
                                              const ReplayTask* __restrict__ tasks, const uint64_t* __restrict__ masks,
                                              const int64_t* __restrict__ rec_offset, dsa_record* __restrict__ out, uint64_t out_cap,
-                                             int64_t pair_base)
+                                             int64_t pair_base, int wt)
 {
     const int tid = threadIdx.x;
     int64_t n = 0;
@@ -1749,7 +1760,7 @@
             }
         }
         const bool both = st.tiles0 != 0 && st.tiles1 != 0;
-        const int base1 = __builtin_ctz(st.tiles0 | 0x10000u) * W + 1, base2 = __builtin_ctz(st.tiles1 | 0x10000u) * W + 1;
+        const int base1 = __builtin_ctz(st.tiles0 | 0x10000u) * wt + 1, base2 = __builtin_ctz(st.tiles1 | 0x10000u) * wt + 1;
         auto lo64 = [](const uint4& v) -> uint64_t { return ((uint64_t)v.y << 32) | v.x; };
         auto hi64 = [](const uint4& v) -> uint64_t { return ((uint64_t)v.w << 32) | v.z; };
 #pragma unroll
@@ -1801,7 +1812,7 @@
                             const int b2 = __builtin_ctzll(r2);
                             bool dup = false;
                             for (int k2 = 0; k2 < k && !dup; ++k2) dup = ((mask_of(k2, t1, 0) >> b1) & 1ull) && ((mask_of(k2, t2, 1) >> b2) & 1ull);
-                            if (!dup) put(c0 * W + b1 + 1, c1 * W + b2 + 1, kr);
+                            if (!dup) put(c0 * wt + b1 + 1, c1 * wt + b2 + 1, kr);
                         }
                     }
                 }
@@ -1815,17 +1826,17 @@
                 if (tasks[q1].chunk0 == NO_CHUNK) continue;
                 uint64_t m1 = masks[((uint64_t)tasks[q1].mask_begin + k) * 2];
                 while (m1) {
-                    const int i1 = tasks[q1].chunk0 * W + __builtin_ctzll(m1) + 1;
+                    const int i1 = tasks[q1].chunk0 * wt + __builtin_ctzll(m1) + 1;
                     m1 &= m1 - 1;
                     for (uint32_t q2 = tb; q2 < te; ++q2) {
                         if (tasks[q2].chunk1 == NO_CHUNK) continue;
                         uint64_t m2 = masks[((uint64_t)tasks[q2].mask_begin + k) * 2 + 1];
                         while (m2) {
-                            const int i2 = tasks[q2].chunk1 * W + __builtin_ctzll(m2) + 1;
+                            const int i2 = tasks[q2].chunk1 * wt + __builtin_ctzll(m2) + 1;
                             m2 &= m2 - 1;
                             bool dup = false;
                             for (int k2 = 0; k2 < k && !dup; ++k2)
-                                dup = col_in(tasks, masks, tb, te, k2, 0, i1) && col_in(tasks, masks, tb, te, k2, 1, i2);
+                                dup = col_in(tasks, masks, tb, te, k2, 0, i1, wt) && col_in(tasks, masks, tb, te, k2, 1, i2, wt);
                             if (!dup) put(i1, i2, kr);
                         }
                     }
@@ -1841,7 +1852,7 @@
                                                   uint32_t tiles0, uint32_t tiles1, int first0, int first1, const dsa_pair* __restrict__ pairs,
                                                   const dsa_fusion* __restrict__ fusions, const KeptRow* __restrict__ kept,
                                                   const uint64_t* __restrict__ masks, const int64_t* __restrict__ rec_offset,
-                                                  dsa_record* __restrict__ out, uint64_t out_cap, int64_t pair_base)
+                                                  dsa_record* __restrict__ out, uint64_t out_cap, int64_t pair_base, int wt)
 {
     const int lane = threadIdx.x & 63, wbase = threadIdx.x & ~63;
     auto slot_m = [&](int e) -> uint4& { return lds->mask[e >> 6][wbase + (e & 63)]; };
@@ -1885,7 +1896,7 @@
                         const int b2 = __builtin_ctzll(r2);
                         bool dup = false;
                         for (int k2 = 0; k2 < k && !dup; ++k2) dup = ((mask_of(k2, t1, 0) >> b1) & 1ull) && ((mask_of(k2, t2, 1) >> b2) & 1ull);
-                        if (!dup) fn(c0 * W + b1 + 1, c1 * W + b2 + 1);
+                        if (!dup) fn(c0 * wt + b1 + 1, c1 * wt + b2 + 1);
                     }
                 }
             }
@@ -1938,7 +1949,7 @@
                                                       const dsa_pair* __restrict__ pairs, const dsa_fusion* __restrict__ fusions,
                                                       const KeptRow* __restrict__ kept, const uint64_t* __restrict__ masks,
                                                       const int64_t* __restrict__ rec_offset, dsa_record* __restrict__ out, uint64_t out_cap,
-                                                      int64_t pair_base)
+                                                      int64_t pair_base, int wt)
 {
     int64_t mine = 0;
     uint64_t todo = __builtin_amdgcn_ballot_w64(heavy);
@@ -1951,7 +1962,7 @@
         const int tl = __shfl((int)st.tiles0 | ((int)st.tiles1 << 16), src, 64);
         const int firsts = __shfl((int)st.first0 | ((int)st.first1 << 8), src, 64);
         const int64_t n = emit_pair_wave<WRITE, SLOTS>(lds, sp, so, mb, kb, packed & 0xFFFF, (packed >> 16) & 0xFF, (uint32_t)tl & 0xFFFFu,
-                                                        (uint32_t)tl >> 16, firsts & 0xFF, (firsts >> 8) & 0xFF, pairs, fusions, kept, masks, rec_offset, out, out_cap, pair_base);
+                                                        (uint32_t)tl >> 16, firsts & 0xFF, (firsts >> 8) & 0xFF, pairs, fusions, kept, masks, rec_offset, out, out_cap, pair_base, wt);
         if ((int)(threadIdx.x & 63) == src) mine = n;
     }
     return mine;
@@ -1974,7 +1985,7 @@
         o = g.orig ? g.orig[p] : p;
     }
     const bool mine = p < g.n_pairs && (st.flags & STATE_COUNTED) && st.n_kept != 0;
-    if (mine) emit_pair<true, EMIT_SLOTS_COUNTED>(&lds, p, o, st, pairs, fusions, kept, tasks, masks, rec_offset, out, out_cap, pair_base);
+    if (mine) emit_pair<true, EMIT_SLOTS_COUNTED>(&lds, p, o, st, pairs, fusions, kept, tasks, masks, rec_offset, out, out_cap, pair_base, g.wt);
 }
 
 template <bool WRITE>
@@ -2002,8 +2013,8 @@
         const bool heavy = mine && emit_is_heavy<EMIT_SLOTS_LISTED>(st);
         DiagClock clk;
         int64_t n = 0;
-        if (mine && !heavy) n = emit_pair<WRITE, EMIT_SLOTS_LISTED>(&lds, p, o, st, pairs, fusions, kept, tasks, masks, rec_offset, out, out_cap, pair_base);
-        const int64_t nh = emit_heavy_of_wave<WRITE, EMIT_SLOTS_LISTED>(&lds, heavy, p, o, st, pairs, fusions, kept, masks, rec_offset, out, out_cap, pair_base);
+        if (mine && !heavy) n = emit_pair<WRITE, EMIT_SLOTS_LISTED>(&lds, p, o, st, pairs, fusions, kept, tasks, masks, rec_offset, out, out_cap, pair_base, g.wt);
+        const int64_t nh = emit_heavy_of_wave<WRITE, EMIT_SLOTS_LISTED>(&lds, heavy, p, o, st, pairs, fusions, kept, masks, rec_offset, out, out_cap, pair_base, g.wt);
         if (!WRITE && mine) rec_count[o] = heavy ? nh : n;
         if (!WRITE && mine)
             DSA_STAT_MAX(g, DS_SLOWEST_LISTED, (clk.lap() << 24) | ((unsigned long long)st.n_kept << 8) | st.n_tasks);
diff --git a/defuse_amd/csrc/dsa_tile.hpp b/defuse_amd/csrc/dsa_tile.hpp
--- /dev/null
+++ b/defuse_amd/csrc/dsa_tile.hpp
@@ -0,0 +1,34 @@
+#pragma once
+
+namespace dsa {
+
+constexpr int TILE_W = 64;
+constexpr int TILE_WIDTHS[] = {64, 60, 56};
+constexpr int N_TILE_WIDTHS = sizeof(TILE_WIDTHS) / sizeof(TILE_WIDTHS[0]);
+
+constexpr int tile_count_class(int tiles) { return tiles <= 8 ? 0 : tiles <= 16 ? 1 : tiles <= 64 ? 2 : tiles <= 255 ? 3 : 4; }
+constexpr int tiles_of(int len, int wt) { return (len + wt - 1) / wt; }
+
+constexpr int pick_tile_width(int max_window)
+{
+    if (max_window <= 0) return TILE_W;
+    int best = TILE_W, best_cols = tiles_of(max_window, TILE_W) * TILE_W;
+    for (int k = 0; k < N_TILE_WIDTHS; ++k) {
+        const int wt = TILE_WIDTHS[k], cols = tiles_of(max_window, wt) * wt;
+        if (cols < best_cols) { best = wt; best_cols = cols; }
+    }
+    if (tile_count_class(tiles_of(max_window, best)) != tile_count_class(tiles_of(max_window, TILE_W))) return TILE_W;
+    return best;
+}
+constexpr bool is_tile_width(int wt)
+{
+    for (int k = 0; k < N_TILE_WIDTHS; ++k)
+        if (TILE_WIDTHS[k] == wt) return true;
+    return false;
+}
+
+static_assert(pick_tile_width(389) == 56 && pick_tile_width(390) == 56 && pick_tile_width(392) == 56, "seven tiles of 56");
+static_assert(pick_tile_width(590) == 60 && pick_tile_width(448) == 64 && pick_tile_width(450) == 60, "");
+static_assert(pick_tile_width(16320) == 64 && tiles_of(15300, pick_tile_width(15300)) <= 255, "tile indices fit a byte");
+
+}
diff --git a/defuse_amd/dsa.py b/defuse_amd/dsa.py
--- a/defuse_amd/dsa.py
+++ b/defuse_amd/dsa.py
@@ -14,7 +14,7 @@
                                              "ref_second", "read_first", "read_second", "score", "pair_idx")])
 assert FUSION_DTYPE.itemsize == 20 and PAIR_DTYPE.itemsize == 20 and RECORD_DTYPE.itemsize == 40
 
-EXPORTS = ["dsa_create", "dsa_destroy", "dsa_get_limits", "dsa_last_error", "dsa_version", "dsa_build_flags", "dsa_device_count", "dsa_pick_device", "dsa_pick_device_among", "dsa_set_plan_options", "dsa_set_scratch_budget", "dsa_share_scratch", "dsa_align_batch",
+EXPORTS = ["dsa_create", "dsa_destroy", "dsa_get_limits", "dsa_tile_cols_for", "dsa_tile_cols_in_use", "dsa_last_error", "dsa_version", "dsa_build_flags", "dsa_device_count", "dsa_pick_device", "dsa_pick_device_among", "dsa_set_plan_options", "dsa_set_scratch_budget", "dsa_share_scratch", "dsa_align_batch",
            "dsa_upload", "dsa_plan", "dsa_run", "dsa_download", "dsa_copy_records_device", "dsa_get_timing", "dsa_get_kernel_counts", "dsa_set_stream", "dsa_synchronize",
            "dsa_stream_create", "dsa_stream_destroy", "dsa_stream_submit", "dsa_stream_collect", "dsa_stream_recollect", "dsa_stream_last_error",
            "dsa_host_alloc", "dsa_host_free", "dsa_host_register", "dsa_host_unregister"]
@@ -62,6 +62,8 @@
         lib.dsa_destroy.argtypes = [vp]
         lib.dsa_destroy.restype = None
         lib.dsa_get_limits.argtypes = [vp, ctypes.POINTER(Limits)]
+        lib.dsa_tile_cols_for.argtypes = [i32]
+        lib.dsa_tile_cols_in_use.argtypes = [vp]
         lib.dsa_last_error.argtypes = [vp]
         lib.dsa_last_error.restype = ctypes.c_char_p
         lib.dsa_version.restype = ctypes.c_char_p
@@ -99,6 +101,10 @@
     return _lib
 
 
+def tile_cols_for(max_window):
+    return int(load_library().dsa_tile_cols_for(int(max_window)))
+
+
 def _check_arrays(ref_bytes, fusions, read_bytes, pairs):
     ref_bytes = np.ascontiguousarray(ref_bytes, dtype=np.uint8)
     read_bytes = np.ascontiguousarray(read_bytes, dtype=np.uint8)
@@ -136,6 +142,9 @@
         lim = Limits()
         self.lib.dsa_get_limits(self.h, ctypes.byref(lim))
         return lim
+
+    def tile_cols_in_use(self):
+        return int(self.lib.dsa_tile_cols_in_use(self.h))
 
     def set_plan_options(self, flags):
         rc = self.lib.dsa_set_plan_options(self.h, int(flags))
diff --git a/include/defuse_dsa.h b/include/defuse_dsa.h
--- a/include/defuse_dsa.h
+++ b/include/defuse_dsa.h
@@ -80,6 +80,8 @@
 void dsa_destroy(dsa_ctx* ctx);
 int  dsa_get_limits(const dsa_ctx* ctx, dsa_limits* out);
 const char* dsa_last_error(const dsa_ctx* ctx);
+int  dsa_tile_cols_for(int32_t max_window);
+int  dsa_tile_cols_in_use(const dsa_ctx* ctx);
 const char* dsa_version(void);
 const char* dsa_build_flags(void);
 int dsa_device_count(void);
```

Result: faster. 305.2 million, median of 6 (+6.6%).
